# cucibala/FaceRecognizeOnnx

Hardware: AMD Instinct MI355X
Metric: faces/sec end-to-end (detect+align+embed), batch=128 640x640 (higher is better)
Workload: dtype f32; 1 GPU; C-headline: 128 frames 640x640 per GPU, SCRFD det_500m + decode + NMS, first 1 face(s)/frame aligned to 112x112, IResNet-50 (w600k_r50) embed, L2-norm; frames_per_gpu=128, faces_per_frame=1, weights=synthetic seeded (det seed 100, rec seed 200), input_residency=HBM-resident before the timed region, gallery_rows=0, topk=0, parallelism=frame-sharded x1, no data-path collective

## Files before the change

facerecognizeonnx_amd/_lib.py:

```python
from __future__ import annotations

import ctypes as C
import os
import subprocess

import numpy as np

_HERE = os.path.dirname(os.path.abspath(__file__))
LIB_PATH = os.path.join(_HERE, "libfacehip.so")
CSRC = os.path.join(_HERE, "csrc")

FACE_DTYPE = np.dtype([("x", "<i4"), ("y", "<i4"), ("w", "<i4"), ("h", "<i4"),
                       ("score", "<f4"), ("lm", "<f4", (10,))])
assert FACE_DTYPE.itemsize == 60


class FhFace(C.Structure):
    _fields_ = [("x", C.c_int32), ("y", C.c_int32), ("w", C.c_int32), ("h", C.c_int32),
                ("score", C.c_float), ("lm", C.c_float * 10)]


def build(force: bool = False) -> str:
    srcs = [os.path.join(CSRC, f) for f in os.listdir(CSRC)] + [os.path.join(_HERE, "..", "include", "facehip.h")]
    stale = (not os.path.exists(LIB_PATH)) or any(os.path.getmtime(s) > os.path.getmtime(LIB_PATH) for s in srcs)
    if force or stale:
        subprocess.check_call(["make", "-C", CSRC, "-j8", "-s"])
    return LIB_PATH


def csrc_fingerprint() -> str:
    import hashlib
    h = hashlib.sha256()
    host_only = {"image_io.cpp", "onnx_reader.cpp", "onnx_reader.h", "comm.cpp"}
    for f in sorted(os.listdir(CSRC)):
        if f.endswith((".hip", ".cpp", ".h")) and f not in host_only:
            h.update(f.encode()); h.update(open(os.path.join(CSRC, f), "rb").read())
    return h.hexdigest()[:16]


_vp, _i, _f, _ll, _d = C.c_void_p, C.c_int, C.c_float, C.c_longlong, C.c_double
_ip = C.POINTER(C.c_int)

PROTOTYPES = {
    "fh_version": (C.c_char_p, []),
    "fh_last_error": (C.c_char_p, []),
    "fh_init": (_i, [_i]),
    "fh_plan_describe": (_i, [C.c_char_p, _i, _i, C.c_char_p, _i]),
    "fh_onnx_dump": (_i, [C.c_char_p, C.c_char_p, _i]),
    "fh_det_create": (_vp, [C.c_char_p]),
    "fh_det_destroy": (None, [_vp]),
    "fh_det_input_size": (_i, [_vp, _ip, _ip]),
    "fh_det_num_anchors": (_i, [_vp]),
    "fh_det_macs_per_frame": (_d, [_vp]),
    "fh_det_act_bytes_per_frame": (_d, [_vp]),
    "fh_det_detect": (_i, [_vp, _vp, _i, _i, _i, _f, _f, _vp, _i]),
    "fh_det_detect_batch_dev": (_i, [_vp, _vp, _i, _i, _i, _i, _ll, _f, _f, _vp, _i, _vp, _vp]),
    "fh_det_run_network_dev": (_i, [_vp, _vp, _i, _i, _i, _i, _ll, _vp]),
    "fh_det_num_outputs": (_i, [_vp]),
    "fh_det_output_dev": (_vp, [_vp, _i, _ip, _ip]),
    "fh_det_input_dev": (_vp, [_vp]),
    "fh_det_postprocess_dev": (_i, [_vp, _i, _f, _f, _vp, _i, _vp, _vp]),
    "fh_postprocess_rows_dev": (_i, [_vp, _i, _i, _i, _f, _f, _f, _vp, _i, _vp, _vp]),
    "fh_rec_create": (_vp, [C.c_char_p]),
    "fh_rec_destroy": (None, [_vp]),
    "fh_rec_input_size": (_i, [_vp, _ip, _ip]),
    "fh_rec_feature_dim": (_i, [_vp]),
    "fh_rec_macs_per_face": (_d, [_vp]),
    "fh_rec_act_bytes_per_face": (_d, [_vp]),
    "fh_rec_set_chunk": (_i, [_vp, _i]),
    "fh_rec_extract": (_i, [_vp, _vp, _i, _i, _i, _vp, _vp, _i]),
    "fh_rec_extract_simple": (_i, [_vp, _vp, _i, _i, _i, _vp, _i]),
    "fh_compare": (_f, [_vp, _i, _vp, _i]),
    "fh_rec_embed_aligned_dev": (_i, [_vp, _vp, _i, _vp, _vp, _vp]),
    "fh_rec_align_dev": (_i, [_vp, _vp, _i, _i, _i, _ll, _vp, _vp, _i, _vp, _vp, _vp]),
    "fh_rec_input_dev": (_vp, [_vp]),
    "fh_rec_embed_faces_dev": (_i, [_vp, _vp, _i, _i, _i, _ll, _vp, _vp, _i, _vp, _vp, _vp]),
    "fh_pipeline_run_dev": (_i, [_vp, _vp, _vp, _i, _i, _i, _i, _ll, _f, _f, _i, _vp, _vp, _vp, _vp]),
    "fh_pipeline_submit_dev": (_i, [_vp, _vp, _vp, _i, _i, _i, _i, _ll, _f, _f, _i, _vp, _vp, _vp, _vp, _vp, _vp]),
    "fh_stream_create": (_vp, [_vp, _vp, _i, _i, _i, _i]),
    "fh_stream_destroy": (None, [_vp]),
    "fh_stream_submit": (_i, [_vp, _vp, _i, _f, _f]),
    "fh_stream_collect": (_i, [_vp, _vp, _vp, _vp, _i]),
    "fh_gallery_create": (_vp, [_i]),
    "fh_gallery_destroy": (None, [_vp]),
    "fh_gallery_upload": (_i, [_vp, _vp, _ll, _i, _ll]),
    "fh_gallery_enroll": (_ll, [_vp, _vp, _ll, _i]),
    "fh_gallery_size": (_ll, [_vp]),
    "fh_gallery_label_dev": (_i, [_vp, _vp, _i, _f, _vp, _vp, _vp]),
    "fh_gallery_topk_dev": (_i, [_vp, _vp, _i, _i, _vp, _vp, _vp]),
    "fh_gallery_set_scan": (_i, [_vp, _i]),
    "fh_gallery_get_scan": (_i, [_vp]),
    "fh_gallery_scan_stats": (_i, [_vp, C.POINTER(_ll), C.POINTER(_ll)]),
    "fh_topk_merge_dev": (_i, [_vp, _vp, _i, _i, _i, _vp, _vp, _vp]),
    "fh_comm_unique_id": (_i, [_vp]),
    "fh_comm_create": (_vp, [_i, _i, _vp, _i]),
    "fh_comm_destroy": (None, [_vp]),
    "fh_comm_rank": (_i, [_vp]),
    "fh_comm_world": (_i, [_vp]),
    "fh_comm_allgather_f32_dev": (_i, [_vp, _vp, _vp, _ll, _vp]),
    "fh_gallery_topk_sharded_dev": (_i, [_vp, _vp, _vp, _i, _i, _vp, _vp, _vp]),
    "fh_timing_enable": (_i, [_i]),
    "fh_timing_num_tags": (_i, []),
    "fh_timing_collect": (_i, [_vp, _vp, _vp, _vp, _i]),
    "fh_timing_collect_ops": (_i, [_vp, _vp, _vp, _i]),
    "fh_det_set_conv_cfg": (_i, [_vp, _i, _i]),
    "fh_rec_set_conv_cfg": (_i, [_vp, _i, _i]),
    "fh_memcpy_d2h": (_i, [_vp, _vp, C.c_size_t]),
    "fh_det_sync": (_i, [_vp, _vp]),
    "fh_rec_sync": (_i, [_vp, _vp]),
    "fh_imread": (_i, [C.c_char_p, C.POINTER(_vp), C.POINTER(_i), C.POINTER(_i)]),
    "fh_image_decode": (_i, [_vp, C.c_size_t, C.POINTER(_vp), C.POINTER(_i), C.POINTER(_i)]),
    "fh_image_free": (None, [_vp]),
    "fh_det_set_winograd": (_i, [_vp, _i]),
    "fh_rec_set_winograd": (_i, [_vp, _i]),
    "fh_rec_set_wino_fusion": (_i, [_vp, _i]),
    "fh_rec_set_shortcut_fold": (_i, [_vp, _i]),
    "fh_rec_set_precision": (_i, [_vp, _i, C.POINTER(C.c_float)]),
    "fh_rec_get_precision": (_i, [_vp]),
    "fh_det_set_cus": (_i, [_vp, _i]),
    "fh_rec_set_cus": (_i, [_vp, _i]),
    "fh_debug_streamk": (_i, [_i, _i]),
    "fh_debug_wino_slots": (_i, [_i]),
    "fh_debug_topk_merge_strided_dev": (_i, [_vp, _vp, _i, _i, _i, _ll, _vp, _vp, _vp]),
    "fh_set_graph_replay": (_i, [_i]),
    "fh_det_workspace_dev": (_vp, [_vp]),
    "fh_det_graph_stats": (_i, [_vp, _vp]),
    "fh_rec_graph_stats": (_i, [_vp, _vp]),
    "fh_det_set_fused_stem": (_i, [_vp, _i]),
    "fh_rec_set_fused_stem": (_i, [_vp, _i]),
    "fh_det_set_fused_front": (_i, [_vp, _i]),
    "fh_det_set_halo_conv": (_i, [_vp, _i]),
    "fh_resize_u8c3_dev": (_i, [_vp, _i, _i, _i, _vp, _i, _i, _i, _vp]),
    "fh_conv_forward_dev": (_i, [_vp, _vp, _vp, _vp, _i, _i, _i, _i, _i, _i, _i, _i, _i, _vp]),
    "fh_conv_winograd_dev": (_i, [_vp, _vp, _vp, _vp, _i, _i, _i, _i, _i, _vp]),
    "fh_debug_wino2_clock_mhz": (_d, []),
    "fh_conv_wino2_dev": (_i, [_vp, _vp, _vp, _vp, _vp, _vp, _i, _i, _i, _i, _i, _i, _i, _vp]),
    "fh_conv_wino2_ex_dev": (_i, [_vp, _vp, _vp, _vp, _vp, _vp, _vp, _vp, _vp, _i, _vp, _vp, _vp, _i, _i, _i, _i, _i, _i, _i, _vp]),
    "fh_conv_wt_rows": (_i, [_i]),
    "fh_conv_pack_weights": (_i, [_vp, _i, _i, _i, _vp]),
    "fh_conv_kpad": (_i, [_i]),
}

_LIB = None


def lib() -> C.CDLL:
    global _LIB
    if _LIB is None:
        path = build()
        path = os.environ.get("FACEHIP_LIB") or path
        try:
            import torch
        except ImportError:
            pass
        L = C.CDLL(path)
        for name, (res, args) in PROTOTYPES.items():
            fn = getattr(L, name)
            fn.restype = res
            fn.argtypes = args
        _LIB = L
    return _LIB


def last_error() -> str:
    return lib().fh_last_error().decode(errors="replace")


class FaceHipError(RuntimeError):
    pass


def check(rc: int, what: str) -> int:
    if rc < 0:
        raise FaceHipError(f"{what} failed ({rc}): {last_error()}")
    return rc
```

facerecognizeonnx_amd/csrc/api.cpp:

```cpp
#include <algorithm>
#include <cstdio>
#include <cstring>
#include <memory>
#include <string>
#include <vector>

#include "../../include/facehip.h"
#include "engine.h"

static_assert(sizeof(fh_face) == 60 && sizeof(fh::FaceRec) == 60, "FaceBox mirror must stay 60 bytes");

namespace {
thread_local std::string g_err;

struct CallOwners { const fh::Net* net[2] = {nullptr, nullptr}; bool shared = false; };
thread_local CallOwners t_owners;
struct Owns {
    explicit Owns(const fh::Net* a, const fh::Net* b = nullptr) { t_owners.net[0] = a; t_owners.net[1] = b; t_owners.shared = !a && !b; }
    ~Owns() { t_owners = CallOwners{}; }
    Owns(const Owns&) = delete;
    Owns& operator=(const Owns&) = delete;
};
template <class F>
int guarded(F&& f) {
    try {
        const int rc = f();
        for (const fh::Net* n : t_owners.net)
            if (n && fh::conv_take_error(g_err, n->error_record())) return FH_ERR_DEVICE;
        if (t_owners.shared && fh::conv_take_error(g_err, fh::conv_error_words())) return FH_ERR_DEVICE;
        return rc;
    } catch (const std::exception& e) {
        g_err = e.what();
        const bool dev = g_err.rfind("HIP error", 0) == 0;
        return dev ? FH_ERR_DEVICE : (g_err.rfind("onnx", 0) == 0 || g_err.rfind("plan", 0) == 0) ? FH_ERR_MODEL : FH_ERR_STATE;
    } catch (...) {
        g_err = "unknown exception";
        return FH_ERR_STATE;
    }
}
int arg_error(const char* msg) { g_err = msg; return FH_ERR_ARG; }
size_t host_image_bytes(int rows, int cols, int step) { return (size_t)(rows - 1) * step + (size_t)cols * 3; }
hipStream_t S(void* s) { return reinterpret_cast<hipStream_t>(s); }
}

namespace fh {
void set_error(const std::string& msg) { g_err = msg; }
}

struct PinnedBuf {
    void* p = nullptr; size_t bytes = 0;
    bool ensure(size_t n) {
        if (n <= bytes) return false;
        if (p) (void)hipHostFree(p);
        p = nullptr; bytes = 0;
        FH_HIP(hipHostMalloc(&p, n, hipHostMallocDefault));
        bytes = n;
        return true;
    }
    ~PinnedBuf() { if (p) (void)hipHostFree(p); }
};
bool g_graph_replay = [] { const char* e = getenv("FACEHIP_GRAPH"); return !e || atoi(e) != 0; }();
struct GraphCall {
    hipGraph_t g = nullptr; hipGraphExec_t x = nullptr;
    std::vector<long long> key;
    int seen = 0;
    size_t nodes = 0;
    long replays = 0;
    void reset() {
        if (x) (void)hipGraphExecDestroy(x);
        if (g) (void)hipGraphDestroy(g);
        x = nullptr; g = nullptr; seen = 0; nodes = 0;
    }
    ~GraphCall() { reset(); }
    template <class F>
    void run(const std::vector<long long>& k, hipStream_t s, F&& body) {
        const bool allow = g_graph_replay && !fh::KernelTimer::get().enabled && !getenv("FACEHIP_DEBUG_SYNC");
        if (!allow) { reset(); key.clear(); body(s); return; }
        if (k != key) { reset(); key = k; }
        if (x) { FH_HIP(hipGraphLaunch(x, s)); ++replays; return; }
        if (seen++ == 0) { body(s); return; }
        FH_HIP(hipStreamBeginCapture(s, hipStreamCaptureModeThreadLocal));
        try {
            body(s);
        } catch (...) {
            hipGraph_t dead = nullptr;
            (void)hipStreamEndCapture(s, &dead);
            if (dead) (void)hipGraphDestroy(dead);
            seen = 0;
            throw;
        }
        FH_HIP(hipStreamEndCapture(s, &g));
        FH_HIP(hipGraphInstantiate(&x, g, nullptr, nullptr, 0));
        (void)hipGraphGetNodes(g, nullptr, &nodes);
        FH_HIP(hipGraphLaunch(x, s));
        ++replays;
    }
};
struct CallStream {
    hipStream_t s = nullptr;
    hipStream_t get() { if (!s) FH_HIP(hipStreamCreateWithFlags(&s, hipStreamNonBlocking)); return s; }
    ~CallStream() { if (s) (void)hipStreamDestroy(s); }
};
static void graph_env_key(std::vector<long long>& key, const fh::Net& net) {
    key.push_back((long long)fh::layout_epoch());
    key.push_back(net.config_word());
    key.push_back((long long)fh::conv_error_generation() << 32 | fh::conv_debug_generation());
}
constexpr int kGraphFaces = 256;

struct fh_det {
    explicit fh_det(const char* p) : det(p) {}
    fh::Detector det;
    fh::DevBuf img, out, cnt;
    PinnedBuf h_img, h_res;
    GraphCall gcall;
    CallStream cs;
    fh::DevBuf p_det, p_cnt, p_total;
    hipEvent_t ev_sel = nullptr;
    int* h_total = nullptr;
    ~fh_det() { if (ev_sel) (void)hipEventDestroy(ev_sel); if (h_total) (void)hipHostFree(h_total); }
};
struct fh_rec {
    explicit fh_rec(const char* p) : rec(p) {}
    fh::Recognizer rec;
    fh::DevBuf img, face, emb;
    PinnedBuf h_img, h_io;
    GraphCall gcall, gcall_simple;
    CallStream cs;
};
struct fh_gallery {
    explicit fh_gallery(int dim) : g(dim) {}
    fh::Gallery g;
};

extern "C" {

const char* fh_version(void) { return "facehip 0.1 (gfx950)"; }
const char* fh_last_error(void) { return g_err.c_str(); }

int fh_init(int device) {
    return guarded([&] {
        int n = 0;
        FH_HIP(hipGetDeviceCount(&n));
        if (device < 0 || device >= n) throw std::runtime_error("HIP error: no such device");
        FH_HIP(hipSetDevice(device));
        return n;
    });
}

int fh_plan_describe(const char* onnx_path, int default_h, int default_w, char* buf, int cap) {
    if (!onnx_path || !buf || cap <= 0) return arg_error("fh_plan_describe: null argument");
    return guarded([&] {
        fh::OnnxModel m = fh::load_onnx(onnx_path);
        int H = default_h, W = default_w;
        const auto& shp = m.inputs[0].shape;
        if (shp.size() == 4) { if (shp[2] > 0) H = (int)shp[2]; if (shp[3] > 0) W = (int)shp[3]; }
        fh::Plan p = fh::build_plan(m, H, W);
        std::string s = p.describe();
        snprintf(buf, (size_t)cap, "%s", s.c_str());
        return (int)s.size();
    });
}

int fh_onnx_dump(const char* onnx_path, char* buf, int cap) {
    if (!onnx_path || !buf || cap <= 0) return arg_error("fh_onnx_dump: null argument");
    return guarded([&] {
        const fh::OnnxModel m = fh::load_onnx(onnx_path);
        std::string s;
        char tmp[256];
        auto dims = [&](const std::vector<int64_t>& d) { std::string o; for (size_t i = 0; i < d.size(); ++i) { o += (i ? "," : ""); o += std::to_string(d[i]); } return o; };
        for (const auto& v : m.inputs) s += "input " + v.name + " [" + dims(v.shape) + "]\n";
        for (const auto& v : m.outputs) s += "output " + v.name + " [" + dims(v.shape) + "]\n";
        for (const auto& kv : m.inits) {
            const fh::OnnxTensor& t = kv.second;
            double sum = 0, first = 0, last = 0;
            size_t n = 0;
            if (!t.f.empty()) { n = t.f.size(); for (float x : t.f) sum += x; first = t.f.front(); last = t.f.back(); }
            else if (!t.i.empty()) { n = t.i.size(); for (int64_t x : t.i) sum += (double)x; first = (double)t.i.front(); last = (double)t.i.back(); }
            snprintf(tmp, sizeof tmp, " n=%zu sum=%.9g first=%.9g last=%.9g\n", n, sum, first, last);
            s += "init " + kv.first + " dtype=" + std::to_string(t.dtype) + " [" + dims(t.dims) + "]" + tmp;
        }
        for (const auto& nd : m.nodes) {
            s += "node " + nd.op + " in=";
            for (size_t i = 0; i < nd.inputs.size(); ++i) s += (i ? "," : "") + nd.inputs[i];
            s += " out=";
            for (size_t i = 0; i < nd.outputs.size(); ++i) s += (i ? "," : "") + nd.outputs[i];
            for (const auto& av : nd.attrs) {
                const fh::OnnxAttr& a = av.second;
                s += " " + av.first + "=";
                if (!a.ints.empty()) s += "ints:" + dims(a.ints);
                else if (!a.floats.empty()) { s += "floats:"; for (size_t i = 0; i < a.floats.size(); ++i) { snprintf(tmp, sizeof tmp, "%s%.9g", i ? "," : "", a.floats[i]); s += tmp; } }
                else if (!a.s.empty()) s += "s:" + a.s;
                else if (!a.t.dims.empty() || !a.t.f.empty() || !a.t.i.empty()) s += "t:[" + dims(a.t.dims) + "]";
                else if (a.f != 0.f) { snprintf(tmp, sizeof tmp, "f:%.9g", a.f); s += tmp; }
                else s += "i:" + std::to_string(a.i);
            }
            s += "\n";
        }
        snprintf(buf, (size_t)cap, "%s", s.c_str());
        return (int)std::min<size_t>(s.size(), (size_t)cap - 1);
    });
}

fh_det* fh_det_create(const char* onnx_path) {
    if (!onnx_path) { g_err = "fh_det_create: null path"; return nullptr; }
    fh_det* h = nullptr;
    int rc = guarded([&] { h = new fh_det(onnx_path); return 0; });
    return rc == 0 ? h : nullptr;
}
void fh_det_destroy(fh_det* d) { delete d; }
int fh_det_input_size(const fh_det* d, int* w, int* h) {
    if (!d) return arg_error("null handle");
    if (w) *w = const_cast<fh_det*>(d)->det.net().in_w();
    if (h) *h = const_cast<fh_det*>(d)->det.net().in_h();
    return FH_OK;
}
int fh_det_num_anchors(const fh_det* d) { return d ? d->det.num_anchors() : arg_error("null handle"); }
double fh_det_macs_per_frame(const fh_det* d) { return d ? const_cast<fh_det*>(d)->det.net().plan().macs : 0.0; }
double fh_det_act_bytes_per_frame(const fh_det* d) { return d ? const_cast<fh_det*>(d)->det.net().plan().act_bytes : 0.0; }

int fh_det_detect_batch_dev(fh_det* d, const uint8_t* frames, int n, int rows, int cols, int step, long long stride,
                            float score_thr, float nms_thr, fh_face* out, int max_pf, int* counts, void* stream) {
    if (!d || !frames || !out || !counts) return arg_error("fh_det_detect_batch_dev: null argument");
    if (n <= 0 || rows <= 0 || cols <= 0 || step < cols * 3 || max_pf <= 0) return arg_error("fh_det_detect_batch_dev: bad size");
    Owns owns(&d->det.net());
    return guarded([&] {
        d->det.detect_dev(frames, n, rows, cols, step, (long)stride, score_thr, nms_thr, reinterpret_cast<fh::FaceRec*>(out), max_pf,
                          counts, S(stream));
        return n;
    });
}

int fh_det_detect(fh_det* d, const uint8_t* bgr, int rows, int cols, int step, float score_thr, float nms_thr, fh_face* out,
                  int max_out) {
    if (!d) return arg_error("Model not loaded!");
    if (!bgr || rows <= 0 || cols <= 0) return 0;
    if (!out || max_out <= 0 || step < cols * 3) return arg_error("fh_det_detect: bad output buffer / step");
    Owns owns(&d->det.net());
    return guarded([&] {
        const size_t bytes = (size_t)rows * step, used = host_image_bytes(rows, cols, step);
        const int in_graph = max_out < kGraphFaces ? max_out : kGraphFaces;
        d->img.ensure(bytes);
        d->out.ensure((size_t)max_out * sizeof(fh_face));
        d->cnt.ensure(sizeof(int));
        const bool m1 = d->h_img.ensure(bytes), m2 = d->h_res.ensure(64 + (size_t)kGraphFaces * sizeof(fh_face));
        const bool moved = m1 || m2;
        if (moved) d->gcall.reset();
        memcpy(d->h_img.p, bgr, used);
        hipStream_t s = d->cs.get();
        int* const h_cnt = static_cast<int*>(d->h_res.p);
        fh_face* const h_faces = reinterpret_cast<fh_face*>(static_cast<char*>(d->h_res.p) + 64);
        long long kthr, knms;
        { float f = score_thr; int v; memcpy(&v, &f, 4); kthr = v; f = nms_thr; memcpy(&v, &f, 4); knms = v; }
        std::vector<long long> key{rows, cols, step, kthr, knms, max_out, (long long)(size_t)d->img.p, (long long)(size_t)d->out.p};
        graph_env_key(key, d->det.net());
        try {
            d->gcall.run(key, s, [&](hipStream_t st) {
                FH_HIP(hipMemcpyAsync(d->img.p, d->h_img.p, used, hipMemcpyHostToDevice, st));
                d->det.detect_dev(d->img.as<uint8_t>(), 1, rows, cols, step, (long)bytes, score_thr, nms_thr, d->out.as<fh::FaceRec>(),
                                  max_out, d->cnt.as<int>(), st);
                FH_HIP(hipMemcpyAsync(h_cnt, d->cnt.p, sizeof(int), hipMemcpyDeviceToHost, st));
                FH_HIP(hipMemcpyAsync(h_faces, d->out.p, (size_t)in_graph * sizeof(fh_face), hipMemcpyDeviceToHost, st));
            });
        } catch (const std::runtime_error& e) {
            if (std::string(e.what()) == "Invalid resize dimensions") return 0;
            throw;
        }
        FH_HIP(hipStreamSynchronize(s));
        int c = *h_cnt;
        c = c < max_out ? c : max_out;
        const int first = c < in_graph ? c : in_graph;
        if (first > 0) memcpy(out, h_faces, (size_t)first * sizeof(fh_face));
        if (c > first)
            FH_HIP(hipMemcpy(out + first, d->out.as<fh_face>() + first, (size_t)(c - first) * sizeof(fh_face), hipMemcpyDeviceToHost));
        return c;
    });
}

int fh_det_sync(fh_det* d, void* stream) {
    if (!d) return arg_error("fh_det_sync: null handle");
    Owns owns(&d->det.net());
    return guarded([&] { FH_HIP(hipStreamSynchronize(S(stream))); return (int)FH_OK; });
}
int fh_det_run_network_dev(fh_det* d, const uint8_t* frames, int n, int rows, int cols, int step, long long stride, void* stream) {
    if (!d || !frames || n <= 0) return arg_error("fh_det_run_network_dev: bad argument");
    Owns owns(&d->det.net());
    return guarded([&] { d->det.run_network_dev(frames, n, rows, cols, step, (long)stride, S(stream)); return n; });
}
int fh_det_num_outputs(const fh_det* d) { return d ? (int)const_cast<fh_det*>(d)->det.net().plan().outputs.size() : arg_error("null handle"); }
const float* fh_det_output_dev(fh_det* d, int index, int* rows, int* cols) {
    if (!d || index < 0 || index >= (int)d->det.net().plan().outputs.size()) { g_err = "bad output index"; return nullptr; }
    const auto& o = d->det.net().plan().outputs[index];
    if (rows) *rows = o.rows;
    if (cols) *cols = o.cols;
    return d->det.net().capacity() > 0 ? d->det.net().output(index) : nullptr;
}
const float* fh_det_input_dev(fh_det* d) { return d && d->det.net().capacity() > 0 ? d->det.net().input() : nullptr; }
int fh_det_postprocess_dev(fh_det* d, int n, float score_thr, float nms_thr, fh_face* out, int max_pf, int* counts, void* stream) {
    if (!d || !out || !counts || n <= 0) return arg_error("fh_det_postprocess_dev: bad argument");
    Owns owns(&d->det.net());
    return guarded([&] { d->det.postprocess_dev(n, score_thr, nms_thr, reinterpret_cast<fh::FaceRec*>(out), max_pf, counts, S(stream)); return n; });
}

int fh_postprocess_rows_dev(const float* rows, int n, int rows_per_frame, int feat, float scale, float score_thr, float nms_thr,
                            fh_face* out, int max_pf, int* counts, void* stream) {
    if (!rows || !out || !counts) return arg_error("fh_postprocess_rows_dev: null argument");
    if (n <= 0 || rows_per_frame <= 0 || max_pf <= 0 || !(scale > 0.f)) return arg_error("fh_postprocess_rows_dev: bad size");
    if ((long)n * rows_per_frame >= (1L << 31) / 16) return arg_error("fh_postprocess_rows_dev: too many rows");
    return guarded([&] {
        hipStream_t s = S(stream);
        if (feat < 15) {
            FH_HIP(hipMemsetAsync(counts, 0, (size_t)n * sizeof(int), s));
            return n;
        }
        struct Scratch { fh::DevBuf cand, keys, ws, count; hipEvent_t done = nullptr; hipStream_t last = nullptr; bool used = false; };
        thread_local Scratch* scp = new Scratch();
        Scratch& sc = *scp;
        if (!sc.done) FH_HIP(hipEventCreateWithFlags(&sc.done, hipEventDisableTiming));
        if (sc.used && sc.last != s) FH_HIP(hipStreamWaitEvent(s, sc.done, 0));
        fh::DevBuf &cand = sc.cand, &keys = sc.keys, &ws = sc.ws, &count = sc.count;
        int cap = 1;
        while (cap < rows_per_frame) cap <<= 1;
        cand.ensure((size_t)n * cap * sizeof(fh::FaceRec));
        keys.ensure((size_t)n * cap * sizeof(unsigned long long));
        ws.ensure((size_t)n * cap * sizeof(int));
        count.ensure((size_t)n * sizeof(int));
        FH_HIP(hipMemsetAsync(count.p, 0, (size_t)n * sizeof(int), s));
        fh::launch_rows_threshold(rows, n, rows_per_frame, feat, scale, score_thr, cand.as<fh::FaceRec>(), keys.as<unsigned long long>(),
                                  count.as<int>(), cap, s);
        fh::launch_sort_nms(cand.as<fh::FaceRec>(), keys.as<unsigned long long>(), count.as<int>(), cap, n, nms_thr,
                            reinterpret_cast<fh::FaceRec*>(out), counts, max_pf, ws.as<int>(), s);
        FH_HIP(hipGetLastError());
        FH_HIP(hipEventRecord(sc.done, s));
        sc.last = s; sc.used = true;
        return n;
    });
}

fh_rec* fh_rec_create(const char* onnx_path) {
    if (!onnx_path) { g_err = "fh_rec_create: null path"; return nullptr; }
    fh_rec* h = nullptr;
    int rc = guarded([&] { h = new fh_rec(onnx_path); return 0; });
    return rc == 0 ? h : nullptr;
}
void fh_rec_destroy(fh_rec* r) { delete r; }
int fh_rec_input_size(const fh_rec* r, int* w, int* h) {
    if (!r) return arg_error("null handle");
    if (w) *w = const_cast<fh_rec*>(r)->rec.net().in_w();
    if (h) *h = const_cast<fh_rec*>(r)->rec.net().in_h();
    return FH_OK;
}
int fh_rec_feature_dim(const fh_rec* r) { return r ? r->rec.dim() : arg_error("null handle"); }
double fh_rec_macs_per_face(const fh_rec* r) { return r ? const_cast<fh_rec*>(r)->rec.net().plan().macs : 0.0; }
double fh_rec_act_bytes_per_face(const fh_rec* r) { return r ? const_cast<fh_rec*>(r)->rec.net().plan().act_bytes : 0.0; }
int fh_rec_set_chunk(fh_rec* r, int n) {
    if (!r || n <= 0) return arg_error("fh_rec_set_chunk: bad argument");
    size_t biggest = 1;
    for (const auto& t : r->rec.net().plan().tensors) biggest = std::max(biggest, t.elems());
    const long limit = (long)(((1UL << 31) - 1) / biggest);
    if (n > limit) return arg_error("fh_rec_set_chunk: chunk too large for the 32-bit tensor offsets of one pass");
    r->rec.max_chunk = n;
    return FH_OK;
}
const float* fh_rec_input_dev(fh_rec* r) { return r && r->rec.net().capacity() > 0 ? r->rec.net().input() : nullptr; }

int fh_rec_embed_aligned_dev(fh_rec* r, const uint8_t* crops, int n, float* out, float* raw, void* stream) {
    if (!r || !crops || !out || n <= 0) return arg_error("fh_rec_embed_aligned_dev: bad argument");
    Owns owns(&r->rec.net());
    return guarded([&] { r->rec.embed_aligned_dev(crops, n, out, S(stream), raw); return n; });
}
int fh_rec_sync(fh_rec* r, void* stream) {
    if (!r) return arg_error("fh_rec_sync: null handle");
    Owns owns(&r->rec.net());
    return guarded([&] { FH_HIP(hipStreamSynchronize(S(stream))); return (int)FH_OK; });
}
int fh_rec_align_dev(fh_rec* r, const uint8_t* frames, int rows, int cols, int step, long long stride, const fh_face* faces,
                     const int* frame_of, int n, uint8_t* crops, int* ok, void* stream) {
    if (!r || !frames || !faces || !crops || !ok || n <= 0 || rows <= 0 || cols <= 0) return arg_error("fh_rec_align_dev: bad argument");
    Owns owns(&r->rec.net());
    return guarded([&] {
        r->rec.align_dev(frames, rows, cols, step, (long)stride, reinterpret_cast<const fh::FaceRec*>(faces), frame_of, n, crops, ok, S(stream));
        return n;
    });
}
int fh_rec_embed_faces_dev(fh_rec* r, const uint8_t* frames, int rows, int cols, int step, long long stride, const fh_face* faces,
                           const int* frame_of, int n, float* out, int* ok, void* stream) {
    if (!r || !frames || !faces || !out || n <= 0 || rows <= 0 || cols <= 0) return arg_error("fh_rec_embed_faces_dev: bad argument");
    Owns owns(&r->rec.net());
    return guarded([&] {
        r->rec.embed_faces_dev(frames, rows, cols, step, (long)stride, reinterpret_cast<const fh::FaceRec*>(faces), frame_of, n, out, ok, S(stream));
        return n;
    });
}

int fh_rec_extract(fh_rec* r, const uint8_t* bgr, int rows, int cols, int step, const fh_face* face, float* out, int out_cap) {
    if (!r) return arg_error("Model not loaded!");
    if (!bgr || rows <= 0 || cols <= 0) return 0;
    if (!face || !out || step < cols * 3) return arg_error("fh_rec_extract: bad argument");
    if (out_cap < r->rec.dim()) return arg_error("fh_rec_extract: output buffer too small");
    Owns owns(&r->rec.net());
    return guarded([&] {
        const size_t bytes = (size_t)rows * step, used = host_image_bytes(rows, cols, step);
        const size_t dimb = (size_t)r->rec.dim() * sizeof(float);
        r->img.ensure(bytes);
        r->face.ensure(sizeof(fh_face) + sizeof(int));
        r->emb.ensure(dimb);
        const bool m1 = r->h_img.ensure(bytes), m2 = r->h_io.ensure(128 + dimb);
        const bool moved = m1 || m2;
        if (moved) { r->gcall.reset(); r->gcall_simple.reset(); }
// ... 44 lines not shown
        });
        FH_HIP(hipStreamSynchronize(s));
        memcpy(out, io + 128, dimb);
        return r->rec.dim();
    });
}

float fh_compare(const float* f1, int n1, const float* f2, int n2) {
    if (n1 != n2 || n1 <= 0 || !f1 || !f2) return 0.0f;
    float dot = 0.0f;
    for (int i = 0; i < n1; ++i) dot += f1[i] * f2[i];
    return (dot + 1.0f) / 2.0f;
}

namespace {
int detect_select_count(fh_det* d, const uint8_t* frames, int n, int rows, int cols, int step, long stride, float score_thr, float nms_thr,
                        int F, fh_face* faces, int* frame_of, int* d_total, hipStream_t sd) {
    d->p_det.ensure((size_t)n * F * sizeof(fh_face));
    d->p_cnt.ensure((size_t)n * sizeof(int));
    d->p_total.ensure(sizeof(int));
    if (!d->ev_sel) FH_HIP(hipEventCreateWithFlags(&d->ev_sel, hipEventDisableTiming));
    if (!d->h_total) FH_HIP(hipHostMalloc(reinterpret_cast<void**>(&d->h_total), sizeof(int), hipHostMallocDefault));
    int* dt = d_total ? d_total : d->p_total.as<int>();
    d->det.detect_dev(frames, n, rows, cols, step, stride, score_thr, nms_thr, d->p_det.as<fh::FaceRec>(), F, d->p_cnt.as<int>(), sd);
    fh::launch_select_faces(d->p_det.as<fh::FaceRec>(), d->p_cnt.as<int>(), n, F, F, reinterpret_cast<fh::FaceRec*>(faces), frame_of, dt, sd);
    FH_HIP(hipMemcpyAsync(d->h_total, dt, sizeof(int), hipMemcpyDeviceToHost, sd));
    FH_HIP(hipEventRecord(d->ev_sel, sd));
    FH_HIP(hipEventSynchronize(d->ev_sel));
    return *d->h_total;
}
}

int fh_pipeline_run_dev(fh_det* d, fh_rec* r, const uint8_t* frames, int n, int rows, int cols, int step, long long stride,
                        float score_thr, float nms_thr, int F, fh_face* faces, int* frame_of, float* emb, void* stream) {
    if (!d || !r || !frames || !faces || !frame_of || !emb) return arg_error("fh_pipeline_run_dev: null argument");
    if (n <= 0 || n > 4096 || rows <= 0 || cols <= 0 || F <= 0) return arg_error("fh_pipeline_run_dev: bad size");
    Owns owns(&d->det.net(), &r->rec.net());
    return guarded([&] {
        hipStream_t s = S(stream);
        const int total = detect_select_count(d, frames, n, rows, cols, step, (long)stride, score_thr, nms_thr, F, faces, frame_of, nullptr, s);
        r->rec.embed_faces_dev(frames, rows, cols, step, (long)stride, reinterpret_cast<const fh::FaceRec*>(faces), frame_of, total, emb, nullptr, s);
        return total;
    });
}

int fh_pipeline_submit_dev(fh_det* d, fh_rec* r, const uint8_t* frames, int n, int rows, int cols, int step, long long stride,
                           float score_thr, float nms_thr, int F, fh_face* faces, int* frame_of, float* emb, int* d_total,
                           void* stream_det, void* stream_rec) {
    if (!d || !r || !frames || !faces || !frame_of || !emb || !d_total) return arg_error("fh_pipeline_submit_dev: null argument");
    if (n <= 0 || n > 4096 || rows <= 0 || cols <= 0 || F <= 0) return arg_error("fh_pipeline_submit_dev: bad size");
    Owns owns(&d->det.net(), &r->rec.net());
    return guarded([&] {
        hipStream_t sd = S(stream_det), sr = S(stream_rec);
        const int total = detect_select_count(d, frames, n, rows, cols, step, (long)stride, score_thr, nms_thr, F, faces, frame_of, d_total, sd);
        if (sd != sr) FH_HIP(hipStreamWaitEvent(sr, d->ev_sel, 0));
        r->rec.embed_faces_dev(frames, rows, cols, step, (long)stride, reinterpret_cast<const fh::FaceRec*>(faces), frame_of, total, emb, nullptr, sr);
        return total;
    });
}

struct fh_stream {
    static constexpr int kSlots = 2;
    fh_det* det; fh_rec* rec;
    int n, rows, cols, F, dim;
    size_t frame_bytes;
    hipStream_t copy_s = nullptr, comp_s = nullptr;
    struct Slot {
        fh::DevBuf frames, faces, frame_of, emb;
        hipEvent_t uploaded = nullptr, done = nullptr;
        int total = -1;
        int frames_in = 0;
    } slot[kSlots];
    long submitted = 0, collected = 0;
    fh_stream(fh_det* d, fh_rec* r, int n_, int rows_, int cols_, int F_) : det(d), rec(r), n(n_), rows(rows_), cols(cols_), F(F_) {
        dim = r->rec.dim();
        frame_bytes = (size_t)rows * cols * 3;
        FH_HIP(hipStreamCreateWithFlags(&copy_s, hipStreamNonBlocking));
        FH_HIP(hipStreamCreateWithFlags(&comp_s, hipStreamNonBlocking));
        for (auto& sl : slot) {
            sl.frames.ensure((size_t)n * frame_bytes);
            sl.faces.ensure((size_t)n * F * sizeof(fh_face));
            sl.frame_of.ensure((size_t)n * F * sizeof(int));
            sl.emb.ensure((size_t)n * F * dim * sizeof(float));
            FH_HIP(hipEventCreateWithFlags(&sl.uploaded, hipEventDisableTiming));
            FH_HIP(hipEventCreateWithFlags(&sl.done, hipEventDisableTiming));
        }
    }
    ~fh_stream() {
        (void)hipDeviceSynchronize();
        for (auto& sl : slot) { if (sl.uploaded) (void)hipEventDestroy(sl.uploaded); if (sl.done) (void)hipEventDestroy(sl.done); }
        if (copy_s) (void)hipStreamDestroy(copy_s);
        if (comp_s) (void)hipStreamDestroy(comp_s);
    }
};

fh_stream* fh_stream_create(fh_det* d, fh_rec* r, int frames_per_batch, int rows, int cols, int faces_per_frame) {
    if (!d || !r || frames_per_batch <= 0 || frames_per_batch > 4096 || rows <= 0 || cols <= 0 || faces_per_frame <= 0) {
        g_err = "fh_stream_create: bad argument";
        return nullptr;
    }
    fh_stream* h = nullptr;
    const int rc = guarded([&] { h = new fh_stream(d, r, frames_per_batch, rows, cols, faces_per_frame); return 0; });
    return rc == 0 ? h : nullptr;
}
void fh_stream_destroy(fh_stream* s) { delete s; }

int fh_stream_submit(fh_stream* st, const uint8_t* host_frames, int n_frames, float score_thr, float nms_thr) {
    if (!st || !host_frames) return arg_error("fh_stream_submit: null argument");
    if (n_frames <= 0 || n_frames > st->n) return arg_error("fh_stream_submit: batch larger than the stream was created for");
    if (st->submitted - st->collected >= fh_stream::kSlots) { g_err = "fh_stream_submit: ring full, collect a batch first"; return FH_ERR_STATE; }
    Owns owns(&st->det->det.net(), &st->rec->rec.net());
    return guarded([&] {
        fh_stream::Slot& sl = st->slot[st->submitted % fh_stream::kSlots];
        FH_HIP(hipMemcpyAsync(sl.frames.p, host_frames, (size_t)n_frames * st->frame_bytes, hipMemcpyHostToDevice, st->copy_s));
        FH_HIP(hipEventRecord(sl.uploaded, st->copy_s));
        FH_HIP(hipStreamWaitEvent(st->comp_s, sl.uploaded, 0));
        const int step = st->cols * 3;
        const int total = detect_select_count(st->det, sl.frames.as<uint8_t>(), n_frames, st->rows, st->cols, step, (long)st->frame_bytes, score_thr, nms_thr,
                                              st->F, sl.faces.as<fh_face>(), sl.frame_of.as<int>(), nullptr, st->comp_s);
        st->rec->rec.embed_faces_dev(sl.frames.as<uint8_t>(), st->rows, st->cols, step, (long)st->frame_bytes, sl.faces.as<fh::FaceRec>(),
                                     sl.frame_of.as<int>(), total, sl.emb.as<float>(), nullptr, st->comp_s);
        FH_HIP(hipEventRecord(sl.done, st->comp_s));
        sl.total = total; sl.frames_in = n_frames;
        ++st->submitted;
        return total;
    });
}

int fh_stream_collect(fh_stream* st, fh_face* faces, int* frame_of, float* emb, int cap) {
    if (!st) return arg_error("fh_stream_collect: null handle");
    if (st->collected >= st->submitted) { g_err = "fh_stream_collect: nothing in flight"; return FH_ERR_STATE; }
    Owns owns(&st->det->det.net(), &st->rec->rec.net());
    return guarded([&] {
        fh_stream::Slot& sl = st->slot[st->collected % fh_stream::kSlots];
        FH_HIP(hipEventSynchronize(sl.done));
        const int m = sl.total < cap ? sl.total : cap;
        if (m > 0) {
            if (faces) FH_HIP(hipMemcpy(faces, sl.faces.p, (size_t)m * sizeof(fh_face), hipMemcpyDeviceToHost));
            if (frame_of) FH_HIP(hipMemcpy(frame_of, sl.frame_of.p, (size_t)m * sizeof(int), hipMemcpyDeviceToHost));
            if (emb) FH_HIP(hipMemcpy(emb, sl.emb.p, (size_t)m * st->dim * sizeof(float), hipMemcpyDeviceToHost));
        }
        const int total = sl.total;
        sl.total = -1;
        ++st->collected;
        return total;
    });
}

fh_gallery* fh_gallery_create(int dim) {
    if (dim <= 0) { g_err = "fh_gallery_create: bad dim"; return nullptr; }
    return new fh_gallery(dim);
}
void fh_gallery_destroy(fh_gallery* g) { delete g; }
int fh_gallery_upload(fh_gallery* g, const float* rows, long long n, int on_device, long long index_base) {
    if (!g || !rows || n <= 0) return arg_error("fh_gallery_upload: bad argument");
    return guarded([&] { g->g.upload(rows, (long)n, on_device != 0, (long)index_base); return 0; });
}
long long fh_gallery_enroll(fh_gallery* g, const float* rows, long long n, int on_device) {
    if (!g || !rows || n <= 0) return arg_error("fh_gallery_enroll: bad argument");
    long long first = -1;
    const int rc = guarded([&] { first = g->g.enroll(rows, (long)n, on_device != 0); return 0; });
    return rc < 0 ? rc : first;
}
long long fh_gallery_size(fh_gallery* g) { return g ? (long long)g->g.size() : (long long)arg_error("fh_gallery_size: null handle"); }
int fh_gallery_label_dev(fh_gallery* g, const float* q, int nq, float threshold, int* labels, float* scores, void* stream) {
    if (!g || !q || !labels || !scores) return arg_error("fh_gallery_label_dev: null argument");
    return guarded([&] { g->g.label_dev(q, nq, threshold, labels, scores, S(stream)); return nq; });
}
int fh_gallery_topk_dev(fh_gallery* g, const float* q, int nq, int k, float* scores, int* indices, void* stream) {
    if (!g || !q || !scores || !indices) return arg_error("fh_gallery_topk_dev: null argument");
    return guarded([&] { g->g.topk_dev(q, nq, k, scores, indices, S(stream)); return nq; });
}

int fh_gallery_set_scan(fh_gallery* g, int mode) {
    if (!g) return arg_error("fh_gallery_set_scan: null handle");
    if (mode != FH_GAL_SCAN_FP32 && mode != FH_GAL_SCAN_F16_RERANK) return arg_error("fh_gallery_set_scan: unknown mode");
    return guarded([&] { g->g.set_scan(mode); return 0; });
}
int fh_gallery_get_scan(const fh_gallery* g) { return g ? g->g.scan() : arg_error("fh_gallery_get_scan: null handle"); }
int fh_gallery_scan_stats(fh_gallery* g, long long* certified, long long* fallback) {
    if (!g) return arg_error("fh_gallery_scan_stats: null handle");
    return guarded([&] { g->g.scan_stats(certified, fallback); return 0; });
}

int fh_topk_merge_dev(const float* ps, const int* pi, int nparts, int nq, int k, float* scores, int* indices, void* stream) {
    if (!ps || !pi || !scores || !indices) return arg_error("fh_topk_merge_dev: null argument");
    if (nparts <= 0 || nq <= 0 || k <= 0 || k > 16 || (long)nparts * k > 65536) return arg_error("fh_topk_merge_dev: bad size");
    return guarded([&] {
        fh::launch_topk_merge(ps, pi, nparts, nq, k, scores, indices, S(stream));
        FH_HIP(hipGetLastError());
        return nq;
    });
}

int fh_debug_topk_merge_strided_dev(const float* ps, const int* pi, int nparts, int nq, int k, long long part_stride, float* scores, int* indices,
                                    void* stream) {
    if (!ps || !pi || !scores || !indices) return arg_error("fh_debug_topk_merge_strided_dev: null argument");
    if (nparts <= 0 || nq <= 0 || k <= 0 || k > 16 || (long)nparts * k > 65536 || part_stride < (long long)nq * k)
        return arg_error("fh_debug_topk_merge_strided_dev: bad size");
    return guarded([&] {
        fh::launch_topk_merge_strided(ps, pi, nparts, nq, k, (long)part_stride, scores, indices, S(stream));
        FH_HIP(hipGetLastError());
        return nq;
    });
}

int fh_timing_enable(int on) { fh::KernelTimer::get().enabled = on != 0; return FH_OK; }
int fh_timing_num_tags(void) { return fh::KernelTimer::kTags; }
int fh_timing_collect(double* ms, double* flops, double* bytes, long long* launches, int n) {
    if (!ms || !flops || !bytes || !launches || n < fh::KernelTimer::kTags) return arg_error("fh_timing_collect: need fh_timing_num_tags()-entry arrays");
    return guarded([&] { fh::KernelTimer::get().collect(ms, flops, bytes, launches); return fh::KernelTimer::kTags; });
}
int fh_timing_collect_ops(double* ms, double* flops, int* tag, int cap) {
    if (!ms || !flops || !tag || cap <= 0) return arg_error("fh_timing_collect_ops: bad argument");
    return guarded([&] { return fh::KernelTimer::get().collect_ops(ms, flops, tag, cap); });
}
int fh_det_set_conv_cfg(fh_det* d, int cfg, int stream_k) {
    if (!d) return arg_error("null handle");
    d->det.net().force_cfg = cfg; d->det.net().sk_enable = stream_k != 0;
    return FH_OK;
}
int fh_det_set_winograd(fh_det* d, int on) { if (!d) return arg_error("null handle"); d->det.net().winograd = on != 0; return FH_OK; }
int fh_rec_set_winograd(fh_rec* r, int on) { if (!r) return arg_error("null handle"); r->rec.net().winograd = on != 0; return FH_OK; }
int fh_rec_set_wino_fusion(fh_rec* r, int on) { if (!r) return arg_error("null handle"); r->rec.net().fuse_wino = on != 0; return FH_OK; }
int fh_rec_set_precision(fh_rec* r, int mode, float* worst_out) {
    if (!r || (mode != FH_PREC_FP32 && mode != FH_PREC_BF16X2)) return arg_error("fh_rec_set_precision: bad argument");
    if (worst_out) *worst_out = 0.f;
    Owns owns(&r->rec.net());
    if (mode == FH_PREC_FP32) return guarded([&] { r->rec.net().set_bf16x2(false, nullptr); return (int)FH_OK; });
    return guarded([&] {
        fh::Net& net = r->rec.net();
        const int n = 64, dim = r->rec.dim();
        const size_t crop = (size_t)net.in_h() * net.in_w() * 3;
        std::vector<uint8_t> h((size_t)n * crop);
        uint32_t st = 0x9E3779B9u;
        for (int i = 0; i < n; ++i) {
            const int amp = 16 + 3 * i;
            for (size_t e = 0; e < crop; ++e) {
                st = st * 1664525u + 1013904223u;
                const int px = (int)(e / 3) % net.in_w(), py = (int)(e / 3) / net.in_w();
                const int v = 128 + ((px * (i + 1) + py * (n - i)) % 97 - 48) + (int)((st >> 24) % (2 * amp + 1)) - amp;
                h[(size_t)i * crop + e] = (uint8_t)std::min(255, std::max(0, v));
            }
        }
        fh::DevBuf dc, de;
        dc.ensure(h.size()); de.ensure((size_t)2 * n * dim * sizeof(float));
        FH_HIP(hipMemcpy(dc.p, h.data(), h.size(), hipMemcpyHostToDevice));
        const bool was = net.bf16x2();
        net.set_bf16x2(false, nullptr);
        r->rec.embed_aligned_dev(dc.as<uint8_t>(), n, de.as<float>(), nullptr);
        const int layers = net.set_bf16x2(true, nullptr);
        if (layers == 0) { net.set_bf16x2(was, nullptr); throw std::runtime_error("fh_rec_set_precision: this model has no layer with a split-bf16 form"); }
        struct Rollback { fh::Net& n; bool armed = true; ~Rollback() { if (armed) { try { n.set_bf16x2(false, nullptr); } catch (...) {} } } } rollback{net};
        r->rec.embed_aligned_dev(dc.as<uint8_t>(), n, de.as<float>() + (size_t)n * dim, nullptr);
        std::vector<float> e((size_t)2 * n * dim);
        FH_HIP(hipDeviceSynchronize());
        FH_HIP(hipMemcpy(e.data(), de.p, e.size() * sizeof(float), hipMemcpyDeviceToHost));
        double worst = 0;
        for (int i = 0; i < n; ++i) {
            double dot = 0, na = 0, nb = 0;
            for (int c = 0; c < dim; ++c) {
                const double a = e[(size_t)i * dim + c], b = e[(size_t)(n + i) * dim + c];
                dot += a * b; na += a * a; nb += b * b;
            }
            const double err = (na > 0 && nb > 0) ? 1.0 - dot / std::sqrt(na * nb) : 1.0;
            worst = std::max(worst, std::isfinite(err) ? err : 1.0);
        }
        if (worst_out) *worst_out = (float)worst;
        double gate = 1e-3;
        if (const char* g = getenv("FACEHIP_PRECISION_GATE")) gate = std::min(gate, atof(g));
        if (!(worst < gate))
            throw std::runtime_error("fh_rec_set_precision: split-bf16 embeddings differ from fp32 by 1 - cos = " + std::to_string(worst) +
                                 " (gate " + std::to_string(gate) + "): staying fp32");
        rollback.armed = false;
        return layers;
    });
}
int fh_rec_get_precision(fh_rec* r) { return r && r->rec.net().bf16x2() ? FH_PREC_BF16X2 : FH_PREC_FP32; }
int fh_rec_set_shortcut_fold(fh_rec* r, int on) { if (!r) return arg_error("null handle"); r->rec.net().fold_shortcut = on != 0; return FH_OK; }
int fh_det_set_halo_conv(fh_det* d, int on) { if (!d) return arg_error("null handle"); d->det.net().halo_conv = on != 0; return FH_OK; }
int fh_det_set_cus(fh_det* d, int cus) { if (!d || cus < 0) return arg_error("bad argument"); d->det.net().cus = cus; return FH_OK; }
int fh_rec_set_cus(fh_rec* r, int cus) { if (!r || cus < 0) return arg_error("bad argument"); r->rec.net().cus = cus; return FH_OK; }
int fh_det_set_fused_stem(fh_det* d, int on) { if (!d) return arg_error("null handle"); d->det.net().fuse_stem = on != 0; return FH_OK; }
int fh_det_set_fused_front(fh_det* d, int on) { if (!d) return arg_error("null handle"); d->det.net().fuse_front = on != 0; return FH_OK; }
int fh_rec_set_fused_stem(fh_rec* r, int on) { if (!r) return arg_error("null handle"); r->rec.net().fuse_stem = on != 0; return FH_OK; }
int fh_rec_set_conv_cfg(fh_rec* r, int cfg, int stream_k) {
    if (!r) return arg_error("null handle");
    r->rec.net().force_cfg = cfg; r->rec.net().sk_enable = stream_k != 0;
    return FH_OK;
}

int fh_memcpy_d2h(void* dst, const void* src, size_t bytes) {
    if (!dst || !src) return arg_error("fh_memcpy_d2h: null argument");
    return guarded([&] { FH_HIP(hipDeviceSynchronize()); FH_HIP(hipMemcpy(dst, src, bytes, hipMemcpyDeviceToHost)); return 0; });
}
int fh_resize_u8c3_dev(const uint8_t* src, int sh, int sw, int sstep, uint8_t* dst, int dh, int dw, int dstep, void* stream) {
    if (!src || !dst || sh <= 0 || sw <= 0 || dh <= 0 || dw <= 0) return arg_error("fh_resize_u8c3_dev: bad argument");
    return guarded([&] {
        fh::launch_resize_u8c3(src, (long)sh * sstep, sh, sw, sstep, dst, (long)dh * dstep, dh, dw, dstep, 1, S(stream));
        FH_HIP(hipGetLastError());
        return 0;
    });
}
int fh_conv_winograd_dev(const float* d_in, const float* w_ohwi, const float* d_bias, float* d_out, int batch, int h, int w, int cin,
                         int cout, void* stream) {
    if (!d_in || !w_ohwi || !d_out || cin % 32 || cout % 4) return arg_error("fh_conv_winograd_dev: bad argument");
    Owns owns(nullptr);
    return guarded([&] {
        const int rows = fh::conv_wt_rows(cout);
        std::vector<float> u36((size_t)36 * rows * cin, 0.f), uf((size_t)cout * cin);
        std::vector<double> uall((size_t)cout * cin * 36);
        for (int co = 0; co < cout; ++co)
            for (int ci = 0; ci < cin; ++ci) {
                double g[9];
                for (int t = 0; t < 9; ++t) g[t] = w_ohwi[((size_t)co * 9 + t) * cin + ci];
                fh::wino_filter_transform(g, &uall[((size_t)co * cin + ci) * 36]);
            }
        for (int f = 0; f < 36; ++f) {
            for (size_t e = 0; e < uf.size(); ++e) uf[e] = (float)uall[e * 36 + f];
            fh::conv_pack_weights(uf.data(), cout, cin, 1, u36.data() + (size_t)f * rows * cin);
        }
        const size_t tiles = (size_t)batch * ((h + 3) / 4) * ((w + 3) / 4);
        fh::DevBuf dU, dV, dM;
        dU.ensure(u36.size() * sizeof(float));
        dV.ensure((36 * (size_t)fh::wino_rows((long)tiles) + 100 * 128) * cin * sizeof(float));
        dM.ensure((36 * (size_t)fh::wino_rows((long)tiles) + 100 * 128) * cout * sizeof(float));
        FH_HIP(hipMemcpy(dU.p, u36.data(), u36.size() * sizeof(float), hipMemcpyHostToDevice));
        static fh::DevBuf slabs;
        static unsigned slabs_gen = 0;
        if (!slabs.p) { slabs.ensure(fh::conv_slab_floats() * sizeof(float)); fh::conv_workspace_init(slabs.as<float>()); slabs_gen = fh::conv_error_generation(); }
        if (slabs_gen != fh::conv_error_generation()) { fh::conv_workspace_reset_async(slabs.as<float>(), S(stream)); slabs_gen = fh::conv_error_generation(); }
        fh::ConvArgs a{};
        a.in = d_in; a.bias = d_bias; a.out1 = d_out; a.slabs = slabs.as<float>(); a.sk_enable = 1;
        a.B = batch; a.H = h; a.W = w; a.Ho = h; a.Wo = w; a.Cin = cin; a.Cout = cout; a.ks = 3; a.stride = 1; a.pad = 1;
        a.act = (int)fh::Act::NONE; a.res_mode = (int)fh::ResMode::NONE;
        fh::launch_conv_winograd(a, dU.as<float>(), dV.as<float>(), dM.as<float>(), 2, nullptr, nullptr, S(stream));
        FH_HIP(hipStreamSynchronize(S(stream)));
        return 0;
    });
}
int fh_conv_wino2_ex_dev(const float* d_in, const float* w_ohwi, const float* d_bias, const float* d_slope, const float* d_res, float* d_out,
                         float* d_out2, const float* d_s2, const float* d_t2, int n_outs, float* const* d_outs, const int* oc0, const int* oact,
                         int batch, int h, int w, int cin, int cout, int act, int bias_cls, void* stream) {
    if (!d_in || !w_ohwi || batch <= 0 || h <= 0 || w <= 0 || cin != 64 || cout <= 0) return arg_error("fh_conv_wino2_dev: bad argument (cin = 64, positive sizes)");
    if (n_outs < 0 || n_outs > 3 || (n_outs > 0 && (!d_outs || !oc0 || !oact))) return arg_error("fh_conv_wino2_dev: bad merged-output description");
    if (n_outs == 0 && ((!d_out && !d_out2) || cout % 64)) return arg_error("fh_conv_wino2_dev: plain layers need an output and cout % 64 == 0");
    if (d_out2 && (!d_s2 || !d_t2)) return arg_error("fh_conv_wino2_dev: a second output needs its scale and shift");
    Owns owns(nullptr);
    return guarded([&] {
        fh::ConvArgs a{};
        a.in = d_in; a.bias = d_bias; a.slope = d_slope; a.res = d_res; a.out1 = d_out; a.out2 = d_out2; a.s2 = d_s2; a.t2 = d_t2;
        a.B = batch; a.H = h; a.W = w; a.Ho = h; a.Wo = w; a.Cin = cin; a.Cout = cout; a.ks = 3; a.stride = 1; a.pad = 1;
        a.act = act; a.bias_cls = bias_cls; a.res_mode = d_res ? (int)fh::ResMode::SAME : (int)fh::ResMode::NONE;
        a.n_outs = n_outs;
        for (int g = 0; g < n_outs; ++g) { a.outs[g] = d_outs[g]; a.oact[g] = oact[g]; a.oc0[g] = oc0[g]; }
        if (n_outs > 0) a.oc0[n_outs] = oc0[n_outs];
        if (!fh::wino2_ok(a)) throw std::runtime_error("fh_conv_wino2_dev: layer shape not supported by the fused F(2x2) kernel");
        std::vector<float> u(fh::wino2_weight_floats(cin, cout));
        fh::wino2_pack_weights(w_ohwi, cout, cin, u.data());
        fh::DevBuf dU;
        dU.ensure(u.size() * sizeof(float));
        FH_HIP(hipMemcpy(dU.p, u.data(), u.size() * sizeof(float), hipMemcpyHostToDevice));
        a.wt = dU.as<float>();
        fh::launch_wino2(a, S(stream));
        FH_HIP(hipGetLastError());
        FH_HIP(hipStreamSynchronize(S(stream)));
        return 0;
    });
}
int fh_conv_wino2_dev(const float* d_in, const float* w_ohwi, const float* d_bias, const float* d_slope, const float* d_res, float* d_out,
                      int batch, int h, int w, int cin, int cout, int act, int bias_cls, void* stream) {
    return fh_conv_wino2_ex_dev(d_in, w_ohwi, d_bias, d_slope, d_res, d_out, nullptr, nullptr, nullptr, 0, nullptr, nullptr, nullptr, batch, h, w,
                                cin, cout, act, bias_cls, stream);
}
double fh_debug_wino2_clock_mhz(void) { return fh::wino2_debug_clock_mhz(); }
int fh_conv_wt_rows(int cout) { return fh::conv_wt_rows(cout); }
int fh_conv_pack_weights(const float* w_ohwi, int cout, int cin, int ksize, float* dst_packed) {
    if (!w_ohwi || !dst_packed || cout <= 0 || cin <= 0) return arg_error("fh_conv_pack_weights: bad argument");
    memset(dst_packed, 0, (size_t)fh::conv_wt_rows(cout) * fh::conv_kpad(ksize * ksize * cin) * sizeof(float));
    fh::conv_pack_weights(w_ohwi, cout, cin, ksize, dst_packed);
    return 0;
}
int fh_conv_kpad(int ktot) { return fh::conv_kpad(ktot); }
const float* fh_det_workspace_dev(fh_det* d) { return d ? d->det.net().workspace() : nullptr; }
int fh_set_graph_replay(int on) { g_graph_replay = on != 0; return FH_OK; }
int fh_det_graph_stats(fh_det* d, long long* replays) {
    if (!d) return arg_error("null handle");
    if (replays) *replays = d->gcall.replays;
    return (int)d->gcall.nodes;
}
int fh_rec_graph_stats(fh_rec* r, long long* replays) {
    if (!r) return arg_error("null handle");
    if (replays) *replays = r->gcall.replays + r->gcall_simple.replays;
    return (int)(r->gcall.nodes ? r->gcall.nodes : r->gcall_simple.nodes);
}
int fh_debug_wino_slots(int slots) { fh::wino_debug_slots(slots); return 0; }
int fh_debug_streamk(int drop_publish, int timeout_ms) { fh::conv_debug_streamk(drop_publish, timeout_ms); return 0; }
int fh_conv_forward_dev(const float* in, const float* wt, const float* bias, float* out, int batch, int h, int w, int cin, int cout,
                        int ks, int stride, int kpad, int cfg, void* stream) {
    if (!in || !wt || !out || batch <= 0 || (ks != 1 && ks != 3) || cin % 4) return arg_error("fh_conv_forward_dev: bad argument");
    Owns owns(nullptr);
    return guarded([&] {
        fh::ConvArgs a{};
        const int pad = ks / 2;
        a.in = in; a.wt = wt; a.bias = bias; a.out1 = out;
        a.B = batch; a.H = h; a.W = w; a.Cin = cin; a.Cout = cout; a.ks = ks; a.stride = stride; a.pad = pad;
        a.Ho = (h + 2 * pad - ks) / stride + 1; a.Wo = (w + 2 * pad - ks) / stride + 1;
        a.Kpad = kpad;
        static fh::DevBuf slabs;
        static unsigned slabs_gen = 0;
        if (!slabs.p) { slabs.ensure(fh::conv_slab_floats() * sizeof(float)); fh::conv_workspace_init(slabs.as<float>()); slabs_gen = fh::conv_error_generation(); }
        if (slabs_gen != fh::conv_error_generation()) { fh::conv_workspace_reset_async(slabs.as<float>(), S(stream)); slabs_gen = fh::conv_error_generation(); }
        a.slabs = slabs.as<float>(); a.sk_enable = 1;
        fh::launch_conv(a, cfg, S(stream));
        FH_HIP(hipGetLastError());
        return 0;
    });
}

}

namespace fh {
Gallery& gallery_of(fh_gallery* g) { return g->g; }
}
```

facerecognizeonnx_amd/csrc/engine.cpp:

```cpp
#include "engine.h"

#include <atomic>
#include <cstdio>
#include <cstdlib>
#include <algorithm>
#include <cmath>
#include <cstring>

namespace fh {

void hip_check(hipError_t e, const char* what) {
    if (e != hipSuccess) throw std::runtime_error(std::string("HIP error: ") + hipGetErrorString(e) + " in " + what);
}

static std::atomic<unsigned long long> g_layout_epoch{1};
unsigned long long layout_epoch() { return g_layout_epoch.load(std::memory_order_relaxed); }

DevBuf::~DevBuf() {
    if (p) { (void)hipFree(p); g_layout_epoch.fetch_add(1, std::memory_order_relaxed); }
}
void DevBuf::ensure(size_t n) {
    if (n <= bytes) return;
    g_layout_epoch.fetch_add(1, std::memory_order_relaxed);
    if (p) { FH_HIP(hipDeviceSynchronize()); FH_HIP(hipFree(p)); p = nullptr; bytes = 0; }
    FH_HIP(hipMalloc(&p, n));
    bytes = n;
}

KernelTimer& KernelTimer::get() { static KernelTimer t; return t; }
hipEvent_t KernelTimer::take() {
    if (!pool_.empty()) { hipEvent_t e = pool_.back(); pool_.pop_back(); return e; }
    hipEvent_t e; FH_HIP(hipEventCreate(&e)); return e;
}
void KernelTimer::begin(hipStream_t s) {
    if (!enabled) return;
    cur_ = take();
    FH_HIP(hipEventRecord(cur_, s));
}
void KernelTimer::end(hipStream_t s, int tag, double flops, double bytes) {
    if (!enabled || !cur_) return;
    hipEvent_t b = take();
    FH_HIP(hipEventRecord(b, s));
    recs_.push_back(Rec{cur_, b, tag, flops, bytes});
    cur_ = nullptr;
}
void KernelTimer::collect(double* ms, double* flops, double* bytes, long long* launches) {
    for (int i = 0; i < kTags; ++i) { ms[i] = 0; flops[i] = 0; bytes[i] = 0; launches[i] = 0; }
    for (auto& r : recs_) {
        FH_HIP(hipEventSynchronize(r.b));
        float t = 0.f;
        FH_HIP(hipEventElapsedTime(&t, r.a, r.b));
        ms[r.tag] += t; flops[r.tag] += r.flops; bytes[r.tag] += r.bytes; launches[r.tag] += 1;
        pool_.push_back(r.a); pool_.push_back(r.b);
    }
    recs_.clear();
}

int KernelTimer::collect_ops(double* ms, double* flops, int* tag, int cap) {
    int n = 0;
    for (auto& r : recs_) {
        FH_HIP(hipEventSynchronize(r.b));
        float t = 0.f;
        FH_HIP(hipEventElapsedTime(&t, r.a, r.b));
        if (n < cap) { ms[n] = t; flops[n] = r.flops; tag[n] = r.tag; ++n; }
        pool_.push_back(r.a); pool_.push_back(r.b);
    }
    recs_.clear();
    return n;
}

static bool debug_sync() {
    static int v = -1;
    if (v < 0) { const char* e = getenv("FACEHIP_DEBUG_SYNC"); v = e ? atoi(e) : 0; }
    return v != 0;
}


static constexpr int kWinoMinCin = 128;
static constexpr long kWinoMinTiles = 256;
static long wino2_min_blocks() {
    static long v = -1;
    if (v < 0) {
        const char* e = getenv("FACEHIP_WINO2");
        const char* m = getenv("FACEHIP_WINO2_MIN");
        v = e && atoi(e) == 0 ? (1L << 60) : m ? atol(m) : 64;
    }
    return v;
}

Net::Net(const std::string& onnx_path, int default_h, int default_w) {
    OnnxModel m = load_onnx(onnx_path);
    int H = default_h, W = default_w;
    const auto& shp = m.inputs[0].shape;
    if (shp.size() == 4) {
        if (shp[2] > 0) H = (int)shp[2];
        if (shp[3] > 0) W = (int)shp[3];
    }
    plan_ = build_plan(m, H, W);

    std::vector<float> host;
    auto push = [&](const float* src, size_t n) {
        size_t off = (host.size() + 63) / 64 * 64;
        host.resize(off + n, 0.f);
        if (n) memcpy(host.data() + off, src, n * sizeof(float));
        return off;
    };
    dev_.resize(plan_.ops.size());
    for (size_t i = 0; i < plan_.ops.size(); ++i) {
        POp& c = plan_.ops[i];
        if (c.bn_src < 0 || c.kind != OpKind::CONV || c.ks != 3 || c.stride != 1 || c.pad != 1 || c.H < 2 || c.W < 2) continue;
        const bool wino_ok = c.Cin >= kWinoMinCin && c.Cin % 32 == 0 && c.Cout % 4 == 0 && c.outs.empty() && c.res_mode != ResMode::UP2X;
        const POp& pr = plan_.ops[c.bn_src];
        if (wino_ok || !c.outs.empty() || (int)pr.s2.size() < c.Cin || pr.out < 0) continue;
        std::vector<float> b9((size_t)9 * c.Cout);
        for (int co = 0; co < c.Cout; ++co) {
            double tap_shift[9];
            for (int t = 0; t < 9; ++t) {
                double acc = 0;
                for (int ci = 0; ci < c.Cin; ++ci) acc += (double)c.weight[((size_t)co * 9 + t) * c.Cin + ci] * pr.t2[ci];
                tap_shift[t] = acc;
            }
            for (int ry = 0; ry < 3; ++ry)
                for (int rx = 0; rx < 3; ++rx) {
                    double b = c.bias[co];
                    for (int ky = 0; ky < 3; ++ky)
                        for (int kx = 0; kx < 3; ++kx) {
                            const bool in_y = !(ry == 0 && ky == 0) && !(ry == 2 && ky == 2);
                            const bool in_x = !(rx == 0 && kx == 0) && !(rx == 2 && kx == 2);
                            if (in_y && in_x) b += tap_shift[ky * 3 + kx];
                        }
                    b9[(size_t)(ry * 3 + rx) * c.Cout + co] = (float)b;
                }
            for (int t = 0; t < 9; ++t)
                for (int ci = 0; ci < c.Cin; ++ci) c.weight[((size_t)co * 9 + t) * c.Cin + ci] *= pr.s2[ci];
        }
        c.bias = b9;
        dev_[i].bn_fold_src = c.bn_src;
        dev_[c.bn_src].bn_fold_dst = true;
    }
    for (size_t i = 0; i < plan_.ops.size(); ++i) {
        const POp& op = plan_.ops[i];
        DevOp& d = dev_[i];
        if (op.kind == OpKind::DWPW) {
            d.dww = push(op.dw_weight.data(), op.dw_weight.size());
            d.dwb = push(op.dw_bias.data(), op.dw_bias.size());
        }
        if (op.kind == OpKind::CONV || op.kind == OpKind::GEMM || op.kind == OpKind::DWPW) {
            const int Ktot = op.ks * op.ks * op.Cin;
            d.Kpad = conv_kpad(Ktot);
            const int rows = conv_wt_rows(op.Cout);
            std::vector<float> packed((size_t)rows * d.Kpad, 0.f);
            conv_pack_weights(op.weight.data(), op.Cout, op.Cin, op.ks, packed.data());
            d.wt = push(packed.data(), packed.size());
            if (op.kind == OpKind::CONV) {
                ConvArgs probe{};
                probe.ks = op.ks; probe.stride = op.stride; probe.pad = op.pad; probe.Cin = op.Cin; probe.Cout = op.Cout; probe.act = (int)op.act;
                probe.res_mode = (int)op.res_mode; probe.H = op.H; probe.W = op.W;
                float dummy = 0.f;
                probe.out2 = op.out2 >= 0 ? &dummy : nullptr;
                probe.bias_cls = dev_[i].bn_fold_src >= 0 ? 1 : 0;
                if (conv_halo_ok(probe) && op.Ho * op.Wo >= 400) {
                    std::vector<float> wf(conv_halo_wfrag_floats(op.Cin, op.Cout));
                    conv_halo_pack_weights(op.weight.data(), op.Cout, op.Cin, wf.data());
                    d.wfrag = push(wf.data(), wf.size());
                    d.halo = true;
                }
            }
            if (op.kind == OpKind::CONV && op.Cin < kWinoMinCin) {
                ConvArgs probe{};
                probe.ks = op.ks; probe.stride = op.stride; probe.pad = op.pad; probe.Cin = op.Cin; probe.Cout = op.Cout; probe.act = (int)op.act;
                probe.res_mode = (int)op.res_mode; probe.H = op.H; probe.W = op.W; probe.Ho = op.Ho; probe.Wo = op.Wo;
                probe.n_outs = (int)op.outs.size(); probe.bias_cls = dev_[i].bn_fold_src >= 0 ? 1 : 0;
                float dummy2 = 0.f;
                probe.out2 = op.out2 >= 0 ? &dummy2 : nullptr;
                if (wino2_ok(probe)) {
                    std::vector<float> u(wino2_weight_floats(op.Cin, op.Cout));
                    wino2_pack_weights(op.weight.data(), op.Cout, op.Cin, u.data());
                    d.w2 = push(u.data(), u.size());
                    d.w2ok = true;
                }
            }
            if (op.kind == OpKind::CONV && op.ks == 3 && op.stride == 1 && op.pad == 1 && op.Cin >= kWinoMinCin && op.Cin % 32 == 0 &&
                op.Cout % 4 == 0 && op.outs.empty() && op.res_mode != ResMode::UP2X) {
                std::vector<float> u36((size_t)36 * rows * op.Cin, 0.f), uf((size_t)op.Cout * op.Cin);
                std::vector<double> uall((size_t)op.Cout * op.Cin * 36);
                for (int co = 0; co < op.Cout; ++co)
                    for (int ci = 0; ci < op.Cin; ++ci) {
                        double g[9];
                        for (int t = 0; t < 9; ++t) g[t] = op.weight[((size_t)co * 9 + t) * op.Cin + ci];
                        wino_filter_transform(g, &uall[((size_t)co * op.Cin + ci) * 36]);
                    }
                for (int f = 0; f < 36; ++f) {
                    for (size_t e = 0; e < uf.size(); ++e) uf[e] = (float)uall[e * 36 + f];
                    conv_pack_weights(uf.data(), op.Cout, op.Cin, 1, u36.data() + (size_t)f * rows * op.Cin);
                }
                d.w36 = push(u36.data(), u36.size());
                d.w36n = u36.size();
                d.wino = true;
                d.bf2 = wino_gemm_ok_bf16x2(op.Cin, op.Cout);
                const size_t tiles = (size_t)((op.H + 3) / 4) * ((op.W + 3) / 4);
                wino_elems_ = std::max(wino_elems_, 36 * tiles * (size_t)std::max(op.Cin, op.Cout));
                wino_maxc_ = std::max(wino_maxc_, (size_t)std::max(op.Cin, op.Cout));
            }
        } else if (op.kind == OpKind::DWCONV || op.kind == OpKind::DWGLOBAL || op.kind == OpKind::GCONV) {
            d.wt = push(op.weight.data(), op.weight.size());
        }
        if (!op.bias.empty()) d.bias = push(op.bias.data(), op.bias.size());
        if (!op.slope.empty()) { d.slope = push(op.slope.data(), op.slope.size()); d.has_slope = true; }
        if (!op.s2.empty()) { d.s2 = push(op.s2.data(), op.s2.size()); d.t2 = push(op.t2.data(), op.t2.size()); d.has_aff = true; }
    }
    for (size_t i = 0; i < plan_.ops.size(); ++i) {
        const POp& c = plan_.ops[i];
        if (c.sc_src < 0 || dev_[i].bn_fold_src >= 0 || c.bias.size() != (size_t)c.Cout) continue;
        if (dev_[i].wino || dev_[i].halo) continue;
        const POp& x = plan_.ops[c.sc_src];
        const int K9 = 9 * c.Cin, K = K9 + x.Cin, rows = conv_wt_rows(c.Cout);
        std::vector<float> w((size_t)rows * K, 0.f), b((size_t)c.Cout);
        for (int co = 0; co < c.Cout; ++co) {
            std::copy_n(&c.weight[(size_t)co * K9], K9, &w[(size_t)co * K]);
            std::copy_n(&x.weight[(size_t)co * x.Cin], x.Cin, &w[(size_t)co * K + K9]);
            b[co] = c.bias[co] + (x.bias.empty() ? 0.f : x.bias[co]);
        }
        dev_[i].wt_sc = push(w.data(), w.size());
        dev_[i].bias_sc = push(b.data(), b.size());
        dev_[i].Kpad_sc = K;
        dev_[i].sc_src = c.sc_src;
        dev_[c.sc_src].sc_dst = true;
    }
    for (size_t i = 0; i < plan_.ops.size(); ++i) {
        const int prod = plan_.ops[i].bn_src;
        if (!dev_[i].wino || prod <= 0 || !dev_[prod].has_aff) continue;
        dev_[i].aff_src = prod; dev_[prod].aff_dst = (int)i;
    }
    for (size_t i = 0; i + 1 < plan_.ops.size(); ++i) {
        const POp& a = plan_.ops[i];
        const POp& b = plan_.ops[i + 1];
        if (!dev_[i].wino || !dev_[i + 1].wino || a.H != b.H || a.W != b.W || a.Cout != b.Cin || !wino_can_fuse(a.H, a.W, a.Cout, false)) continue;
        int feed = -1;
        if (dev_[i + 1].aff_src == (int)i) feed = 1;
        else if (a.out >= 0 && b.in == a.out) feed = 0;
        else if (a.out2 >= 0 && b.in == a.out2) feed = 1;
        if (feed < 0) continue;
        int other_uses = 0;
        if (a.out >= 0) {
            for (const POp& o : plan_.ops)
                for (int x : {o.in, o.in2, o.res}) if (x == a.out) ++other_uses;
            for (const auto& o : plan_.outputs) if (o.tensor == a.out) ++other_uses;
            if (b.in == a.out) --other_uses;
        }
        const bool writes_out2 = a.out2 >= 0 && dev_[i + 1].aff_src != (int)i;
        if (!wino_can_fuse(a.H, a.W, a.Cout, other_uses > 0 || a.res >= 0 || writes_out2)) continue;
        dev_[i].fuse_next = true; dev_[i].fuse_feed_aff = feed == 1; dev_[i].fuse_keep_out1 = other_uses > 0;
    }
    {
        const POp& op = plan_.ops[0];
        stem_ok_ = op.kind == OpKind::CONV && op.in == plan_.input && op.ks == 3 && op.Cin == 4 && op.res < 0 && op.outs.empty() &&
                   op.Cout % 4 == 0 && op.Cout <= 64 && (op.stride == 1 || op.stride == 2);
        if (stem_ok_) {
            std::vector<float> w27((size_t)27 * op.Cout);
            for (int co = 0; co < op.Cout; ++co)
                for (int t = 0; t < 9; ++t)
                    for (int ci = 0; ci < 3; ++ci) w27[(size_t)(t * 3 + ci) * op.Cout + co] = op.weight[((size_t)co * 9 + t) * 4 + ci];
            dev_[0].w27 = push(w27.data(), w27.size());
            std::vector<float> wf((size_t)27 * op.Cout), bf((size_t)op.Cout);
            for (int co = 0; co < op.Cout; ++co) {
                double sum = 0;
                for (int t = 0; t < 9; ++t)
                    for (int j = 0; j < 3; ++j) {
                        const float w = op.weight[((size_t)co * 9 + t) * 4 + (2 - j)];
                        wf[(size_t)(t * 3 + j) * op.Cout + co] = w / 128.0f;
                        sum += w;
                    }
                bf[co] = (float)((double)op.bias[co] - 127.5 / 128.0 * sum);
            }
            dev_[0].wf = push(wf.data(), wf.size());
            dev_[0].bf = push(bf.data(), bf.size());
            if (op.Cout % 16 == 0) {
                std::vector<unsigned> fr((size_t)(op.Cout / 16) * 3 * 64 * 4, 0u);
                stem_pack_wfrag(wf.data(), op.Cout, fr.data());
                std::vector<float> asf(fr.size());
                memcpy(asf.data(), fr.data(), fr.size() * 4);
                dev_[0].wfr = push(asf.data(), asf.size());
            }
        }
    }
    if (stem_ok_ && plan_.ops.size() > 1) {
        const POp& st = plan_.ops[0];
        const POp& nx = plan_.ops[1];
        int uses = 0;
        for (const auto& o : plan_.ops) for (int x : {o.in, o.in2, o.res}) if (x == st.out) ++uses;
        for (const auto& o : plan_.outputs) if (o.tensor == st.out) ++uses;
        front_ok_ = st.Cout == 16 && st.out >= 0 && st.out2 < 0 && (st.act == Act::NONE || st.act == Act::RELU) && nx.kind == OpKind::DWPW &&
                    nx.in == st.out && uses == 1 && front_fused_ok(nx.Cin, nx.Cout, nx.dw_stride);
    }
    params_.ensure(std::max<size_t>(host.size(), 64) * sizeof(float));
    FH_HIP(hipMemcpy(params_.p, host.data(), host.size() * sizeof(float), hipMemcpyHostToDevice));
    for (auto& op : plan_.ops) { std::vector<float>().swap(op.weight); }
}

Net::SkRecord::~SkRecord() {
    if (!p) return;
    int cur = -1;
    (void)hipGetDevice(&cur);
    if (device >= 0 && device != cur) (void)hipSetDevice(device);
    (void)hipDeviceSynchronize();
    if (device >= 0 && device != cur && cur >= 0) (void)hipSetDevice(cur);
    conv_error_record_release(p);
}

void Net::reserve(int max_batch) {
    if (max_batch <= cap_) return;
    cap_ = max_batch;
    arena_.ensure(plan_.arena_elems * (size_t)cap_ * sizeof(float));
    if (partial_.bytes < conv_slab_floats() * sizeof(float)) {
        partial_.ensure(conv_slab_floats() * sizeof(float));
        conv_workspace_init(partial_.as<float>());
        if (!sk_rec_.p) { sk_rec_.p = conv_error_record_new(); (void)hipGetDevice(&sk_rec_.device); }
        if (!sk_rec_.p) throw std::runtime_error("HIP error: cannot allocate the stream-K watchdog record");
        sk_gen_ = conv_error_generation();
    }
    if (wino_elems_) {
        const size_t pad = 36 * 256 * wino_maxc_;
        wino_v_.ensure((wino_elems_ * (size_t)cap_ + pad) * sizeof(float));
        wino_m_.ensure((wino_elems_ * (size_t)cap_ + pad) * sizeof(float));
    }
    FH_HIP(hipMemset(arena_.p, 0, arena_.bytes));
}

void Net::run_u8(const uint8_t* src, long img_stride, int srcH, int srcW, int step, int batch, hipStream_t s) {
    if (batch <= 0) return;
    if (batch > cap_) throw std::runtime_error("Net::run_u8: batch exceeds reserved capacity");
    if (stem_ok_ && fuse_stem && front_ok_ && fuse_front && srcW >= 2) {
        const POp& st = plan_.ops[0];
        const POp& op = plan_.ops[1];
        const DevOp& d0 = dev_[0];
        const DevOp& d = dev_[1];
        const float* P = params_.as<float>();
        ConvArgs a{};
        a.wt = P + d.wt; a.bias = P + d.bias;
        a.out1 = tensor_ptr(op.out);
        a.dw_w = P + d.dww; a.dw_b = P + d.dwb; a.dw_act = (int)op.dw_act; a.dw_stride = op.dw_stride;
        a.B = batch; a.H = op.H; a.W = op.W; a.Cin = op.Cin; a.Ho = op.Ho; a.Wo = op.Wo; a.Cout = op.Cout;
        a.ks = 1; a.stride = 1; a.pad = 0; a.Kpad = d.Kpad; a.act = (int)op.act;
        a.u8_src = src; a.u8_img_stride = img_stride; a.u8_step = step; a.u8_srcH = srcH; a.u8_srcW = srcW; a.u8_inH = plan_.inH; a.u8_inW = plan_.inW;
        a.slabs = partial_.as<float>();
        a.u8_stride = st.stride; a.stem_act = (int)st.act; a.stem_wf = P + d0.wf; a.stem_bf = P + d0.bf;
        a.stem_wfrag = reinterpret_cast<const unsigned*>(P + d0.wfr);
        a.cus = cus;
        a.t_flops = 2.0 * (st.macs + op.macs) * batch;
        a.t_bytes = ((double)srcH * srcW * 3 + (double)op.Ho * op.Wo * op.Cout * 4) * batch;
        launch_dwpw(a, s);
        run(batch, s, 2);
        return;
    }
    if (stem_ok_ && fuse_stem) {
        const POp& op = plan_.ops[0];
        const DevOp& d = dev_[0];
        const float* P = params_.as<float>();
        KernelTimer& timer = KernelTimer::get();
        timer.begin(s);
        launch_stem_conv_u8(src, img_stride, srcH, srcW, step, batch, plan_.inH, plan_.inW, op.stride, op.Cout, P + d.w27, P + d.bias, P + d.wf,
                            P + d.bf, d.has_slope ? P + d.slope : nullptr, (int)op.act, op.out >= 0 ? tensor_ptr(op.out) : nullptr,
                            op.out2 >= 0 && !d.bn_fold_dst ? tensor_ptr(op.out2) : nullptr, d.has_aff ? P + d.s2 : nullptr,
                            d.has_aff ? P + d.t2 : nullptr, s, d.wfr ? reinterpret_cast<const unsigned*>(P + d.wfr) : nullptr);
        timer.end(s, 5, 2.0 * op.macs * batch, op.bytes * batch);
        run(batch, s, 1);
        return;
    }
    launch_det_preprocess(src, img_stride, srcH, srcW, step, batch, plan_.inH, plan_.inW, srcH, srcW, input(), s);
    run(batch, s, 0);
}

int Net::set_bf16x2(bool on, hipStream_t s) {
    int layers = 0;
    size_t total = 0;
    for (auto& d : dev_) if (d.wino && d.bf2) { d.w36p = total; total += d.w36n; ++layers; }
    if (on && layers > 0 && w36_bf_.bytes < total * sizeof(float)) {
        w36_bf_.ensure(total * sizeof(float));
        for (const auto& d : dev_)
            if (d.wino && d.bf2) launch_pack_bf16x2(params_.as<float>() + d.w36, w36_bf_.as<float>() + d.w36p, (long)d.w36n, s);
        FH_HIP(hipStreamSynchronize(s));
    }
    bf16x2_ = on && layers > 0;
    return on ? layers : 0;
}

void Net::run(int batch, hipStream_t s, int first_op) {
    if (batch <= 0) return;
    if ((sk_gen_ != conv_error_generation() || conv_error_pending(sk_rec_.p)) && partial_.p) {
        conv_workspace_reset_async(partial_.as<float>(), s);
        sk_gen_ = conv_error_generation();
    }
    if (batch > cap_) throw std::runtime_error("Net::run: batch exceeds reserved capacity");
    const float* P = params_.as<float>();
    KernelTimer& timer = KernelTimer::get();
    bool v_ready = false;
    for (size_t i = (size_t)first_op; i < plan_.ops.size(); ++i) {
        const POp& op = plan_.ops[i];
        const DevOp& d = dev_[i];
        int tag = 5;
        const bool dense = op.kind == OpKind::CONV || op.kind == OpKind::GEMM || op.kind == OpKind::DWPW;
        if (!dense) timer.begin(s);
        switch (op.kind) {
            case OpKind::CONV:
            case OpKind::GEMM: {
                if (d.sc_dst && fold_shortcut && force_cfg < 0) break;
                ConvArgs a{};
                a.in = tensor_ptr(op.in);
                a.wt = P + d.wt;
                a.bias = P + d.bias;
                a.slope = d.has_slope ? P + d.slope : nullptr;
                a.res = op.res >= 0 ? tensor_ptr(op.res) : nullptr;
                a.out1 = op.out >= 0 ? tensor_ptr(op.out) : nullptr;
                a.out2 = op.out2 >= 0 ? tensor_ptr(op.out2) : nullptr;
                if (d.bn_fold_dst) a.out2 = nullptr;
                if (d.bn_fold_src >= 0) { a.in = tensor_ptr(plan_.ops[d.bn_fold_src].out); a.bias_cls = 1; }
                if (d.aff_dst >= 0 && winograd) {
                    const POp& c = plan_.ops[d.aff_dst];
                    if ((long)batch * ((c.H + 3) / 4) * ((c.W + 3) / 4) >= kWinoMinTiles) a.out2 = nullptr;
                }
                a.s2 = d.has_aff ? P + d.s2 : nullptr;
                a.t2 = d.has_aff ? P + d.t2 : nullptr;
                a.slabs = partial_.as<float>();
                a.sk_err = sk_rec_.p;
                a.sk_enable = sk_enable ? 1 : 0;
                a.cus = cus;
                a.no_pw = force_cfg >= 0 ? 1 : 0;
                a.B = batch; a.H = op.H; a.W = op.W; a.Cin = op.Cin; a.Ho = op.Ho; a.Wo = op.Wo; a.Cout = op.Cout;
                a.ks = op.ks; a.stride = op.stride; a.pad = op.pad; a.Kpad = d.Kpad;
                a.act = (int)op.act; a.res_mode = (int)op.res_mode;
                a.n_outs = (int)op.outs.size();
                for (int g = 0; g < a.n_outs && g < 3; ++g) { a.outs[g] = tensor_ptr(op.outs[g]); a.oact[g] = op.out_act[g]; a.oc0[g] = op.out_c0[g]; }
                if (a.n_outs > 0) a.oc0[a.n_outs] = op.out_c0[a.n_outs];
                const long M = (long)batch * op.Ho * op.Wo;
                int cfg = force_cfg >= 0 ? force_cfg : conv_pick_cfg(M, op.Cout);
                if (force_cfg < 0 && cfg == 0 && ((M + 127) / 128) * ((op.Cout + 127) / 128) < 128) cfg = 3;
                a.t_flops = 2.0 * op.macs * batch; a.t_bytes = op.bytes * batch;
                if (d.sc_src >= 0 && fold_shortcut && force_cfg < 0) {
                    const POp& x = plan_.ops[d.sc_src];
                    a.wt = P + d.wt_sc; a.bias = P + d.bias_sc; a.Kpad = d.Kpad_sc;
                    a.res = nullptr; a.res_mode = (int)ResMode::NONE;
                    a.sc_in = tensor_ptr(x.in); a.sc_H = x.H; a.sc_W = x.W; a.sc_C = x.Cin; a.sc_stride = x.stride;
                    a.t_flops += 2.0 * x.macs * batch;
                }
                if (d.halo && halo_conv && force_cfg < 0) {
                    launch_conv_halo(a, P + d.wfrag, s);
                    tag = 9;
                    break;
                }
                if (d.w2ok && winograd && force_cfg < 0 && d.sc_src < 0 && wino2_blocks(a) >= wino2_min_blocks()) {
                    a.wt = P + d.w2;
                    launch_wino2(a, s);
                    break;
                }
                const bool use_wino = d.wino && winograd && (long)batch * ((op.H + 3) / 4) * ((op.W + 3) / 4) >= kWinoMinTiles;
                if (use_wino) {
                    const int wcfg = force_cfg >= 0 ? force_cfg : 2;
                    const bool bf2 = bf16x2_ && d.bf2 && force_cfg < 0;
                    WinoPlanes pl;
                    const bool mix = wcfg == 2 && wino_mix_layout(batch, op.H, op.W, op.Cin, op.Cout, &pl);
                    if (!v_ready) {
                        const float* in_s = nullptr; const float* in_t = nullptr;
                        if (d.aff_src >= 0) {
                            a.in = tensor_ptr(plan_.ops[d.aff_src].out);
                            in_s = P + dev_[d.aff_src].s2; in_t = P + dev_[d.aff_src].t2;
                        }
                        if (mix) launch_wino_mix(a, pl, nullptr, wino_v_.as<float>(), 0, in_s, in_t, bf2, s);
                        else launch_wino_input(a, wino_v_.as<float>(), in_s, in_t, bf2, s);
                    }
                    launch_wino_gemm(a, bf2 ? w36_bf_.as<float>() + d.w36p : P + d.w36, wino_v_.as<float>(), wino_m_.as<float>(), wcfg, bf2, s,
                                     mix ? &pl : nullptr);
                    v_ready = false;
                    if (d.fuse_next && fuse_wino && i + 1 < plan_.ops.size()) {
                        const POp& nx = plan_.ops[i + 1];
                        const bool next_wino = dev_[i + 1].wino && (long)batch * ((nx.H + 3) / 4) * ((nx.W + 3) / 4) >= kWinoMinTiles;
                        const bool next_mix = next_wino && wcfg == 2 && wino_mix_layout(batch, nx.H, nx.W, nx.Cin, nx.Cout, nullptr);
                        if (next_wino && mix == next_mix) {
                            ConvArgs e = a;
                            if (!d.fuse_keep_out1) e.out1 = nullptr;
                            const bool pack_next = bf16x2_ && dev_[i + 1].bf2 && force_cfg < 0;
                            if (mix) launch_wino_mix(e, pl, wino_m_.as<float>(), wino_v_.as<float>(), d.fuse_feed_aff ? 1 : 0, nullptr, nullptr, pack_next, s);
                            else launch_wino_fused(e, wino_m_.as<float>(), wino_v_.as<float>(), d.fuse_feed_aff ? 1 : 0, pack_next, s);
                            v_ready = true;
                        }
                    }
                    if (!v_ready) {
                        if (mix) launch_wino_mix(a, pl, wino_m_.as<float>(), nullptr, 0, nullptr, nullptr, false, s);
                        else launch_wino_output(a, wino_m_.as<float>(), s);
                    }
                    tag = 7;
                    break;
                }
                launch_conv(a, cfg, s);
                tag = cfg;
                break;
            }
            case OpKind::DWPW: {
                ConvArgs a{};
                a.in = tensor_ptr(op.in);
                a.wt = P + d.wt; a.bias = P + d.bias;
                a.out1 = tensor_ptr(op.out);
                a.dw_w = P + d.dww; a.dw_b = P + d.dwb; a.dw_act = (int)op.dw_act; a.dw_stride = op.dw_stride;
                a.B = batch; a.H = op.H; a.W = op.W; a.Cin = op.Cin; a.Ho = op.Ho; a.Wo = op.Wo; a.Cout = op.Cout;
                a.ks = 1; a.stride = 1; a.pad = 0; a.Kpad = d.Kpad; a.act = (int)op.act;
                a.t_flops = 2.0 * op.macs * batch; a.t_bytes = op.bytes * batch;
                a.slabs = partial_.as<float>();
                launch_dwpw(a, s);
                break;
            }
            case OpKind::DWCONV:
                launch_dwconv3x3(tensor_ptr(op.in), P + d.wt, P + d.bias, tensor_ptr(op.out), batch, op.H, op.W, op.Cin, op.stride,
                                 (int)op.act, d.has_slope ? P + d.slope : nullptr, s);
                tag = 4;
                break;
            case OpKind::DWGLOBAL:
                launch_dwglobal(tensor_ptr(op.in), P + d.wt, P + d.bias, tensor_ptr(op.out), batch, op.ks * op.ks, op.Cin, (int)op.act,
                                d.has_slope ? P + d.slope : nullptr, s);
                break;
            case OpKind::GCONV:
                launch_gconv3x3(tensor_ptr(op.in), P + d.wt, P + d.bias, tensor_ptr(op.out), batch, op.H, op.W, op.Cin,
                                (int)(op.weight_group), op.stride, (int)op.act, d.has_slope ? P + d.slope : nullptr, s);
                tag = 4;
                break;
            case OpKind::AFFINE:
                launch_affine(tensor_ptr(op.in), P + d.s2, P + d.t2, tensor_ptr(op.out), (long)batch * op.H * op.W, op.Cin, s);
                break;
            case OpKind::ACT:
                launch_act(tensor_ptr(op.in), d.has_slope ? P + d.slope : nullptr, tensor_ptr(op.out), (long)batch * op.H * op.W,
                           op.Cin, (int)op.act, s);
                break;
            case OpKind::ADD:
                launch_add(tensor_ptr(op.in), tensor_ptr(op.in2), tensor_ptr(op.out), (long)batch * op.H * op.W * op.Cin, s);
                break;
            case OpKind::UPSAMPLE:
                launch_upsample2x(tensor_ptr(op.in), tensor_ptr(op.out), batch, op.H, op.W, op.Cin, s);
                break;
        }
        if (!dense) timer.end(s, tag, 2.0 * op.macs * batch, op.bytes * batch);
        if (debug_sync()) {
            fprintf(stderr, "[facehip] op %zu %s batch %d done-launch\n", i, op.name.c_str(), batch); fflush(stderr);
            const hipError_t e1 = hipGetLastError(), e2 = hipStreamSynchronize(s);
            if (e1 != hipSuccess || e2 != hipSuccess)
                throw std::runtime_error("HIP error after op " + std::to_string(i) + " (" + op.name + "): " + hipGetErrorString(e1 != hipSuccess ? e1 : e2));
        }
    }
    FH_HIP(hipGetLastError());
}

Detector::Detector(const std::string& onnx_path) : net_(onnx_path, 640, 640) {
    const auto& outs = net_.plan().outputs;
    const int H = net_.in_h(), W = net_.in_w();
    if (outs.size() == 9) {
        static const int cols[9] = {1, 1, 1, 4, 4, 4, 10, 10, 10};
        static const int strides[3] = {8, 16, 32};
        bool ok = true;
        for (int i = 0; i < 9; ++i) {
            const int s = strides[i % 3];
            ok = ok && outs[i].cols == cols[i] && outs[i].rows == (H / s) * (W / s) * 2;
        }
        if (ok) anchors_ = ((H / 8) * (W / 8) + (H / 16) * (W / 16) + (H / 32) * (W / 32)) * 2;
    } else if (outs.size() >= 1 && outs[0].cols >= 15) {
        predecoded_ = true;
        anchors_ = outs[0].rows;
        feat_ = outs[0].cols;
    }
    cap_ = 1;
    while (cap_ < std::max(anchors_, 1)) cap_ <<= 1;
}

void Detector::reserve(int n, int rows, int cols) {
    (void)rows; (void)cols;
    net_.reserve(n);
    if (n > nb_) {
        nb_ = n;
        cand_.ensure((size_t)n * cap_ * sizeof(FaceRec));
        keys_.ensure((size_t)n * cap_ * sizeof(unsigned long long));
        ws_.ensure((size_t)n * cap_ * sizeof(int));
        count_.ensure((size_t)n * sizeof(int));
    }
}

void Detector::run_network_dev(const uint8_t* frames, int n, int rows, int cols, int step, long stride, hipStream_t s) {
    reserve(n, rows, cols);
    const int inW = net_.in_w(), inH = net_.in_h();
    const float scaleW = (float)inW / (float)cols, scaleH = (float)inH / (float)rows;
    scale_ = std::min(scaleW, scaleH);
    const int newW = (int)((float)cols * scale_), newH = (int)((float)rows * scale_);
    if (newW <= 0 || newH <= 0) throw std::runtime_error("Invalid resize dimensions");
    const uint8_t* src = frames;
    long sstride = stride;
    int sstep = step;
    if (newW != cols || newH != rows) {
        resized_.ensure((size_t)n * newH * newW * 3);
        launch_resize_u8c3(frames, stride, rows, cols, step, resized_.as<uint8_t>(), (long)newH * newW * 3, newH, newW, newW * 3, n, s);
        src = resized_.as<uint8_t>(); sstride = (long)newH * newW * 3; sstep = newW * 3;
    }
    net_.run_u8(src, sstride, newH, newW, sstep, n, s);
}

void Detector::postprocess_dev(int n, float score_thr, float nms_thr, FaceRec* out, int max_out, int* counts, hipStream_t s) {
    if (anchors_ <= 0) { FH_HIP(hipMemsetAsync(counts, 0, (size_t)n * sizeof(int), s)); return; }
    FH_HIP(hipMemsetAsync(count_.p, 0, (size_t)n * sizeof(int), s));
    if (predecoded_) {
        launch_rows_threshold(net_.output(0), n, anchors_, feat_, scale_, score_thr, cand_.as<FaceRec>(),
                              keys_.as<unsigned long long>(), count_.as<int>(), cap_, s);
    } else {
        DecodeArgs a{};
        for (int i = 0; i < 3; ++i) { a.score[i] = net_.output(i); a.bbox[i] = net_.output(3 + i); a.kps[i] = net_.output(6 + i); }
        a.inH = net_.in_h(); a.inW = net_.in_w(); a.B = n; a.scale = scale_; a.thr = score_thr;
        a.cand = cand_.as<FaceRec>(); a.keys = keys_.as<unsigned long long>(); a.count = count_.as<int>(); a.cap = cap_;
        launch_scrfd_decode(a, s);
    }
    launch_sort_nms(cand_.as<FaceRec>(), keys_.as<unsigned long long>(), count_.as<int>(), cap_, n, nms_thr, out, counts, max_out,
                    ws_.as<int>(), s);
    FH_HIP(hipGetLastError());
}

void Detector::detect_dev(const uint8_t* frames, int n, int rows, int cols, int step, long stride, float score_thr, float nms_thr,
                          FaceRec* out, int max_out, int* counts, hipStream_t s) {
    if (n <= 0) return;
    run_network_dev(frames, n, rows, cols, step, stride, s);
    postprocess_dev(n, score_thr, nms_thr, out, max_out, counts, s);
}

Recognizer::Recognizer(const std::string& onnx_path) : net_(onnx_path, 112, 112) {
    const auto& o = net_.plan().outputs.at(0);
    dim_ = o.rows * o.cols;
}

void Recognizer::embed_aligned_dev(const uint8_t* crops, int n, float* out, hipStream_t s, float* raw_out) {
    const int H = net_.in_h(), W = net_.in_w();
    net_.reserve(std::min(n, max_chunk));
    for (int off = 0; off < n; off += max_chunk) {
        const int c = std::min(max_chunk, n - off);
        net_.run_u8(crops + (size_t)off * H * W * 3, (long)H * W * 3, H, W, W * 3, c, s);
        if (raw_out) FH_HIP(hipMemcpyAsync(raw_out + (size_t)off * dim_, net_.output(0), (size_t)c * dim_ * sizeof(float), hipMemcpyDeviceToDevice, s));
        launch_l2_normalize(net_.output(0), out + (size_t)off * dim_, c, dim_, s);
    }
    FH_HIP(hipGetLastError());
}

void Recognizer::align_dev(const uint8_t* frames, int rows, int cols, int step, long stride, const FaceRec* faces,
                           const int* frame_of, int n, uint8_t* crops, int* ok, hipStream_t s) {
    launch_align(frames, stride, rows, cols, step, faces, frame_of, n, net_.in_h(), net_.in_w(), crops, ok, s);
    FH_HIP(hipGetLastError());
}

void Recognizer::embed_faces_dev(const uint8_t* frames, int rows, int cols, int step, long stride, const FaceRec* faces,
                                 const int* frame_of, int n, float* out, int* ok, hipStream_t s) {
    if (n <= 0) return;
    const size_t crop = (size_t)net_.in_h() * net_.in_w() * 3;
    crops_.ensure((size_t)n * crop);
    ok_.ensure((size_t)n * sizeof(int));
    int* okp = ok ? ok : ok_.as<int>();
    align_dev(frames, rows, cols, step, stride, faces, frame_of, n, crops_.as<uint8_t>(), okp, s);
    embed_aligned_dev(crops_.as<uint8_t>(), n, out, s);
}

void Recognizer::resize_embed_dev(const uint8_t* frames, int n, int rows, int cols, int step, long stride, float* out, hipStream_t s) {
    const int H = net_.in_h(), W = net_.in_w();
    crops_.ensure((size_t)n * H * W * 3);
    launch_resize_u8c3(frames, stride, rows, cols, step, crops_.as<uint8_t>(), (long)H * W * 3, H, W, W * 3, n, s);
    embed_aligned_dev(crops_.as<uint8_t>(), n, out, s);
}

void Gallery::upload(const float* rows, long n, bool device_src, long index_base) {
    if (dim_ % 64) throw std::runtime_error("gallery: dim must be a multiple of 64");
    rows_.ensure((size_t)n * dim_ * sizeof(float));
    FH_HIP(hipMemcpy(rows_.p, rows, (size_t)n * dim_ * sizeof(float), device_src ? hipMemcpyDeviceToDevice : hipMemcpyHostToDevice));
    n_ = n; base_ = index_base;
    if (scan_ == 1) {
        rows16_.ensure((size_t)n * dim_ * sizeof(uint16_t));
        convert16(0, n);
    }
}

void Gallery::convert16(long first, long n) {
    gstat_.ensure(4 * sizeof(unsigned));
    if (first == 0) FH_HIP(hipMemset(gstat_.p, 0, 4 * sizeof(unsigned)));
    launch_gallery16_convert(rows_.as<float>() + (size_t)first * dim_, rows16_.as<uint16_t>() + (size_t)first * dim_, n, dim_,
                             gstat_.as<unsigned>(), nullptr);
    FH_HIP(hipGetLastError());
    unsigned h[4];
    FH_HIP(hipMemcpy(h, gstat_.p, sizeof(h), hipMemcpyDeviceToHost));
    for (int i = 0; i < 3; ++i) memcpy(&gbound_[i], &h[i], sizeof(float));
    f16_bad_ = h[3] != 0;
}

void Gallery::set_scan(int mode) {
    if (mode != 0 && mode != 1) throw std::invalid_argument("gallery: unknown scan mode");
    if (mode == 0) {
        DevBuf none;
        std::swap(none.p, rows16_.p);
        std::swap(none.bytes, rows16_.bytes);
        scan_ = 0;
        return;
    }
    if (scan_ != 1) {
        ctr_.ensure(2 * sizeof(unsigned long long));
        FH_HIP(hipMemset(ctr_.p, 0, 2 * sizeof(unsigned long long)));
        if (n_ > 0) {
            rows16_.ensure((size_t)n_ * dim_ * sizeof(uint16_t));
            convert16(0, n_);
        }
        scan_ = 1;
    }
}

void Gallery::scan_stats(long long* certified, long long* fallback) {
    unsigned long long h[2] = {0, 0};
    FH_HIP(hipDeviceSynchronize());
    if (ctr_.p) {
        FH_HIP(hipMemcpy(h, ctr_.p, sizeof(h), hipMemcpyDeviceToHost));
        FH_HIP(hipMemset(ctr_.p, 0, sizeof(h)));
    }
    if (certified) *certified = (long long)h[0];
    if (fallback) *fallback = (long long)h[1] + host_fallback_;
    host_fallback_ = 0;
}

long Gallery::enroll(const float* rows, long n, bool device_src) {
    if (dim_ % 64) throw std::runtime_error("gallery: dim must be a multiple of 64");
    const size_t row_bytes = (size_t)dim_ * sizeof(float);
    const size_t need = (size_t)(n_ + n) * row_bytes;
    if (need > rows_.bytes) {
        DevBuf bigger;
        bigger.ensure(std::max(need, rows_.bytes * 2));
        if (n_ > 0) FH_HIP(hipMemcpy(bigger.p, rows_.p, (size_t)n_ * row_bytes, hipMemcpyDeviceToDevice));
        std::swap(bigger.p, rows_.p);
        std::swap(bigger.bytes, rows_.bytes);
    }
    FH_HIP(hipMemcpy(static_cast<char*>(rows_.p) + (size_t)n_ * row_bytes, rows, (size_t)n * row_bytes,
                     device_src ? hipMemcpyDeviceToDevice : hipMemcpyHostToDevice));
    if (scan_ == 1) {
        const size_t row16 = (size_t)dim_ * sizeof(uint16_t), cap16 = rows_.bytes / row_bytes * row16;
        if (cap16 > rows16_.bytes) {
            DevBuf bigger;
            bigger.ensure(cap16);
            if (n_ > 0) FH_HIP(hipMemcpy(bigger.p, rows16_.p, (size_t)n_ * row16, hipMemcpyDeviceToDevice));
            std::swap(bigger.p, rows16_.p);
            std::swap(bigger.bytes, rows16_.bytes);
        }
        convert16(n_, n);
    }
    const long first = base_ + n_;
    n_ += n;
    return first;
}

void Gallery::label_dev(const float* q, int Q, float thr, int* out_label, float* out_score, hipStream_t s) {
    best_i_.ensure((size_t)std::max(Q, 1) * sizeof(int));
    topk_dev(q, Q, 1, out_score, best_i_.as<int>(), s);
    launch_label(out_score, best_i_.as<int>(), Q, thr, out_label, s);
}

void Gallery::topk_dev(const float* q, int Q, int k, float* out_score, int* out_idx, hipStream_t s) {
    if (Q <= 0 || Q > 256 || k <= 0 || k > 16) throw std::runtime_error("gallery: need 0 < Q <= 256 and 0 < k <= 16");
    if (dim_ % 64) throw std::runtime_error("gallery: dim must be a multiple of 64");
    if (scan_ == 1) {
        if (!f16_bad_ && n_ > 0 && dim_ % 128 == 0) {
            topk_f16(q, Q, k, out_score, out_idx, s);
            return;
        }
// ... 52 lines not shown
```

facerecognizeonnx_amd/csrc/kernels.h:

```cpp
#pragma once
#include <hip/hip_runtime.h>

#include <cstdint>
#include <string>

#include <vector>

namespace fh {

void hip_check(hipError_t e, const char* what);
#define FH_HIP(x) ::fh::hip_check((x), #x)

#if defined(__HIPCC__)
__device__ __forceinline__ void wave_lds_order() {
#if defined(__HIP_DEVICE_COMPILE__)
    __builtin_amdgcn_fence(__ATOMIC_ACQ_REL, "wavefront");
    __builtin_amdgcn_wave_barrier();
#endif
}
#endif

struct KernelTimer {
    static constexpr int kTags = 13;
    bool enabled = false;
    void begin(hipStream_t s);
    void end(hipStream_t s, int tag, double flops, double bytes);
    void collect(double* ms, double* flops, double* bytes, long long* launches);
    int collect_ops(double* ms, double* flops, int* tag, int cap);
    static KernelTimer& get();

  private:
    struct Rec { hipEvent_t a, b; int tag; double flops, bytes; };
    std::vector<Rec> recs_;
    std::vector<hipEvent_t> pool_;
    hipEvent_t cur_ = nullptr;
    hipEvent_t take();
};


struct ConvArgs {
    const float* in;
    const float* wt;
    const float* bias;
    const float* slope;
    const float* res;
    float* out1;
    float* out2;
    const float* s2;
    const float* t2;
    float* slabs;
    const float* zeros;
    int B, H, W, Cin, Ho, Wo, Cout;
    int ks, stride, pad;
    int Kpad;
    int bias_cls;
    const float* sc_in;
    int sc_H, sc_W, sc_C, sc_stride;
    int act;
    int res_mode;
    const float* dw_w;
    const float* dw_b;
    int dw_act;
    int dw_stride;
    const uint8_t* u8_src;
    long u8_img_stride;
    int u8_step, u8_srcH, u8_srcW, u8_inH, u8_inW, u8_stride, stem_act;
    const float* stem_wf;
    const float* stem_bf;
    const unsigned* stem_wfrag;
    int no_prio;
    int no_pw;
    int n_outs;
    float* outs[3];
    int oc0[4];
    int oact[3];
    int sk_enable;
    int cus;
    int wt_group_rows;
    long wt_gs;
    double t_flops, t_bytes;
    int sk_full, sk_units, sk_q, sk_helpers, sk_rem, sk_owner_chunks, sk_maxp;
    unsigned* sk_err;
    int ep_direct;
    unsigned sk_timeout;
    int sk_test_drop;
    int tile0;
};

void launch_conv(const ConvArgs& a, int cfg, hipStream_t s);
int conv_pick_cfg(long M, int Cout);
void conv_workspace_init(float* ws);
void conv_workspace_reset_async(float* ws, hipStream_t s);
unsigned* conv_error_words();
unsigned* conv_error_record_new();
void conv_error_record_release(unsigned* r);
bool conv_take_error(std::string& msg, unsigned* rec);
bool conv_error_pending(const unsigned* rec);
unsigned conv_error_generation();
void conv_debug_streamk(int drop_publish, int timeout_ms);
unsigned conv_debug_generation();
size_t wino2_weight_floats(int Cin, int Cout);
void wino2_pack_weights(const float* w_ohwi, int Cout, int Cin, float* dst);
bool wino2_ok(const ConvArgs& a);
void launch_wino2(const ConvArgs& a, hipStream_t s);
long wino2_blocks(const ConvArgs& a);
double wino2_debug_clock_mhz();
const float* conv_zero_line();
int conv_num_cus();
bool conv_halo_ok(const ConvArgs& a);
size_t conv_halo_wfrag_floats(int Cin, int Cout);
void conv_halo_pack_weights(const float* w_ohwi, int Cout, int Cin, float* dst);
void launch_conv_halo(const ConvArgs& a, const float* wfrag, hipStream_t s);
void stem_pack_wfrag(const float* wf, int Cout, unsigned* out);
bool front_fused_ok(int Cin, int Cout, int dw_stride);
void launch_dwpw(const ConvArgs& a, hipStream_t s);
void launch_conv_winograd(const ConvArgs& a, const float* wt36, float* V, float* M, int cfg, const float* in_scale, const float* in_shift,
                          hipStream_t s);
struct WinoPlanes;
void launch_wino_input(const ConvArgs& a, float* V, const float* in_scale, const float* in_shift, bool pack, hipStream_t s);
void launch_wino_gemm(const ConvArgs& a, const float* wt36, const float* V, float* M, int cfg, bool bf16x2, hipStream_t s,
                      const WinoPlanes* mix = nullptr);
bool wino_gemm_ok_bf16x2(int Cin, int Cout);
void launch_wino_output(const ConvArgs& a, const float* M, hipStream_t s);
bool wino_can_fuse(int H, int W, int C, bool touches_memory);
void launch_wino_fused(const ConvArgs& a, const float* M, float* Vnext, int feed_aff, bool pack_next, hipStream_t s);
void launch_pack_bf16x2(const float* in, float* out, long n, hipStream_t s);
struct WinoPlanes {
    int e[4];
    int t[4];
    int nfc[4];
    int f2[4];
    int n[4];
    int rows[4];
    int base[4];
    int total_tiles;
    int planes;
};
bool wino_mix_layout(int B, int H, int W, int Cin, int Cout, WinoPlanes* out);
void launch_wino_mix(const ConvArgs& a, const WinoPlanes& pl, const float* M, float* Vnext, int feed_aff, const float* in_scale,
                     const float* in_shift, bool pack_next, hipStream_t s);
void wino_filter_transform(const double g[9], double u[36]);
void wino_debug_slots(int slots);
long wino_rows(long tiles);
int conv_wt_rows(int Cout);
size_t conv_slab_floats();
void conv_pack_weights(const float* w, int Cout, int Cin, int ks, float* dst);
inline int conv_kpad(int Ktot) { return (Ktot + 31) / 32 * 32; }

void launch_dwconv3x3(const float* in, const float* w9c, const float* bias, float* out, int B, int H, int W,
                      int C, int stride, int act, const float* slope, hipStream_t s);
void launch_dwglobal(const float* in, const float* w, const float* bias, float* out, int B, int taps, int C, int act, const float* slope,
                     hipStream_t s);
void launch_gconv3x3(const float* in, const float* w, const float* bias, float* out, int B, int H, int W, int C, int G, int stride, int act,
                     const float* slope, hipStream_t s);
void launch_affine(const float* in, const float* sc, const float* sh, float* out, long pixels, int C, hipStream_t s);
void launch_act(const float* in, const float* slope, float* out, long pixels, int C, int act, hipStream_t s);
void launch_add(const float* a, const float* b, float* out, long n, hipStream_t s);
void launch_upsample2x(const float* in, float* out, int B, int H, int W, int C, hipStream_t s);

struct FaceRec {
    int32_t x, y, w, h;
    float score;
    float lm[10];
};

void launch_det_preprocess(const uint8_t* frames, long img_stride, int rows, int cols, int step, int B,
                           int inH, int inW, int newH, int newW, float* out, hipStream_t s);
void launch_rec_preprocess(const uint8_t* crops, int n, int H, int W, float* out, hipStream_t s);
void launch_stem_conv_u8(const uint8_t* src, long img_stride, int srcH, int srcW, int step, int B, int inH, int inW, int stride,
                         int Cout, const float* w27, const float* bias, const float* wf, const float* biasf, const float* slope, int act,
                         float* out1, float* out2, const float* s2, const float* t2, hipStream_t s, const unsigned* wfrag = nullptr);

struct DecodeArgs {
    const float* score[3];
    const float* bbox[3];
    const float* kps[3];
    int inH, inW, B;
    float scale, thr;
    FaceRec* cand;
    unsigned long long* keys;
    int* count;
    int cap;
};
void launch_scrfd_decode(const DecodeArgs& a, hipStream_t s);
void launch_rows_threshold(const float* rows, int B, int n, int feat, float scale, float thr, FaceRec* cand,
                           unsigned long long* keys, int* count, int cap, hipStream_t s);
void launch_sort_nms(const FaceRec* cand, unsigned long long* keys, const int* count, int cap, int B, float nms_thr,
                     FaceRec* out, int* out_count, int max_out, int* order_ws, hipStream_t s);

void launch_align(const uint8_t* frames, long img_stride, int rows, int cols, int step, const FaceRec* faces,
                  const int* frame_of, int n, int outH, int outW, uint8_t* crops, int* ok, hipStream_t s);
void launch_resize_u8c3(const uint8_t* src, long src_stride, int sh, int sw, int sstep, uint8_t* dst, long dst_stride,
                        int dh, int dw, int dstep, int n, hipStream_t s);

void launch_l2_normalize(const float* in, float* out, int n, int dim, hipStream_t s);

int gallery_parts(long G, int Q, int* tiles_per_part);
void launch_gallery_topk(const float* gal, long G, int dim, const float* qpacked, int Q, int k, long idx_base, float* part_score, int* part_idx,
                         float* seed_score, int* seed_idx, hipStream_t s,
                         const int* qcount = nullptr);
void launch_label(const float* best_score, const int* best_idx, int n, float thr, int* labels, hipStream_t s);
void launch_topk_merge(const float* part_score, const int* part_idx, int nparts, int Q, int k, float* out_score,
                       int* out_idx, hipStream_t s, const int* qcount = nullptr);
void launch_topk_merge_strided(const float* part_score, const int* part_idx, int nparts, int Q, int k, long part_stride, float* out_score,
                               int* out_idx, hipStream_t s, const int* qcount = nullptr);

constexpr int GAL16_KC = 32;
void launch_gallery16_convert(const float* rows, uint16_t* rows16, long n, int dim, unsigned* stats, hipStream_t s);
int gallery16_parts(long G, int Q, int* tiles_per_part);
void launch_gallery16_candidates(const uint16_t* rows16, long G, int dim, const float* q, uint16_t* q16, int Q, long idx_base, float* part_score,
                                 int* part_idx, float* seed_score, int* seed_idx, float* cand_score, int* cand_idx, hipStream_t s);
void launch_gallery16_rescore(const float* rows, long G, int dim, const float* q, int Q, int k, long idx_base, const float* cand_score,
                              const int* cand_idx, float gn, float ghn, float dn, float* out_score, int* out_idx, int* fb_count, int* fb_idx,
                              unsigned long long* counters, hipStream_t s);
void launch_gallery16_gather(const float* q, int Q, int dim, const int* fb_count, const int* fb_idx, float* qpacked, hipStream_t s);
void launch_gallery16_scatter(const float* fb_score, const int* fb_idx_out, int Q, int k, const int* fb_count, const int* fb_idx, float* out_score,
                              int* out_idx, hipStream_t s);

void launch_select_faces(const FaceRec* det, const int* counts, int n, int per_frame, int F, FaceRec* faces, int* frame_of,
                         int* total, hipStream_t s);

}
```

facerecognizeonnx_amd/csrc/winograd.hip:

```cpp
#include <hip/hip_runtime.h>

#include <algorithm>
#include <cstdlib>
#include <stdexcept>

#include "kernels.h"
#include "plan.h"

namespace fh {

typedef float v4f __attribute__((ext_vector_type(4)));
typedef float v16f __attribute__((ext_vector_type(16)));
typedef float v2f __attribute__((ext_vector_type(2)));
typedef unsigned v4u __attribute__((ext_vector_type(4)));
typedef __bf16 bf16x2 __attribute__((ext_vector_type(2)));
typedef __bf16 bf16x8 __attribute__((ext_vector_type(8)));

__device__ __forceinline__ v4f wino_pack_bf16x2(const v4f x) {
    v4u out;
#pragma unroll
    for (int p = 0; p < 2; ++p) {
        const v2f a = {x[2 * p], x[2 * p + 1]};
        const unsigned hb = __builtin_bit_cast(unsigned, __builtin_convertvector(a, bf16x2));
        const v2f r = {a[0] - __builtin_bit_cast(float, hb << 16), a[1] - __builtin_bit_cast(float, hb & 0xffff0000u)};
        const unsigned mb = __builtin_bit_cast(unsigned, __builtin_convertvector(r, bf16x2));
        out[2 * p] = (hb & 0xffffu) | (mb << 16);
        out[2 * p + 1] = (hb >> 16) | (mb & 0xffff0000u);
    }
    return __builtin_bit_cast(v4f, out);
}

__global__ __launch_bounds__(256) void pack_bf16x2_kernel(const float* __restrict__ in, float* __restrict__ out, long n4) {
    for (long i = (long)blockIdx.x * blockDim.x + threadIdx.x; i < n4; i += (long)gridDim.x * blockDim.x)
        *reinterpret_cast<v4f*>(out + 4 * i) = wino_pack_bf16x2(*reinterpret_cast<const v4f*>(in + 4 * i));
}
void launch_pack_bf16x2(const float* in, float* out, long n, hipStream_t s) {
    const long n4 = n / 4;
    if (n4 > 0) hipLaunchKernelGGL(pack_bf16x2_kernel, dim3((unsigned)std::min<long>((n4 + 255) / 256, 256 * 64)), dim3(256), 0, s, in, out, n4);
}

__device__ __forceinline__ void wino_bt(const v4f (&d)[6], v4f (&t)[6]) {
    t[0] = 4.f * d[0] - 5.f * d[2] + d[4];
    t[1] = -4.f * d[1] - 4.f * d[2] + d[3] + d[4];
    t[2] = 4.f * d[1] - 4.f * d[2] - d[3] + d[4];
    t[3] = -2.f * d[1] - d[2] + 2.f * d[3] + d[4];
    t[4] = 2.f * d[1] - d[2] - 2.f * d[3] + d[4];
    t[5] = 4.f * d[1] - 5.f * d[3] + d[5];
}
__device__ __forceinline__ void wino_at(const v4f (&m)[6], v4f (&y)[4]) {
    y[0] = m[0] + m[1] + m[2] + m[3] + m[4];
    y[1] = m[1] - m[2] + 2.f * m[3] - 2.f * m[4];
    y[2] = m[1] + m[2] + 4.f * m[3] + 4.f * m[4];
    y[3] = m[1] - m[2] + 8.f * m[3] - 8.f * m[4] + m[5];
}

__global__ __launch_bounds__(256, 2) void wino_input_kernel(const float* __restrict__ in, float* __restrict__ V, int B, int H, int W,
                                                            int C, int TY, int TX, long NTp, const float* __restrict__ aff_s,
                                                            const float* __restrict__ aff_t, const int pack) {
    const int C4 = C >> 2;
    const int NT = B * TY * TX;
    const int total = NT * C4;
    for (int idx = blockIdx.x * blockDim.x + threadIdx.x; idx < total; idx += gridDim.x * blockDim.x) {
        const int c4 = idx % C4;
        const int tile = idx / C4;
        const int tx = tile % TX, ty = (tile / TX) % TY, b = tile / (TX * TY);
        const int iy0 = 4 * ty - 1, ix0 = 4 * tx - 1;
        const float* img = in + (size_t)b * H * W * C + c4 * 4;
        v4f as4 = {1.f, 1.f, 1.f, 1.f}, at4 = {0.f, 0.f, 0.f, 0.f};
        if (aff_s) { as4 = *reinterpret_cast<const v4f*>(aff_s + c4 * 4); at4 = *reinterpret_cast<const v4f*>(aff_t + c4 * 4); }
        v4f t[6][6];
#pragma unroll
        for (int c = 0; c < 6; ++c) {
            const int ix = ix0 + c;
            v4f d[6];
#pragma unroll
            for (int r = 0; r < 6; ++r) {
                const int iy = iy0 + r;
                const bool ok = (unsigned)iy < (unsigned)H && (unsigned)ix < (unsigned)W;
                const v4f raw = *reinterpret_cast<const v4f*>(img + (ok ? ((size_t)iy * W + ix) * C : (size_t)0));
                const float okf = ok ? 1.f : 0.f;
                d[r] = raw * (as4 * okf) + at4 * okf;
            }
            v4f tc[6];
            wino_bt(d, tc);
#pragma unroll
            for (int i = 0; i < 6; ++i) t[i][c] = tc[i];
        }
        float* dst = V + (size_t)tile * C + c4 * 4;
        const size_t fs = (size_t)NTp * C;
#pragma unroll
        for (int i = 0; i < 6; ++i) {
            v4f o[6];
            wino_bt(t[i], o);
#pragma unroll
            for (int j = 0; j < 6; ++j) *reinterpret_cast<v4f*>(dst + (size_t)(i * 6 + j) * fs) = pack ? wino_pack_bf16x2(o[j]) : o[j];
        }
    }
}

struct WinoOutArgs {
    const float* M; const float* bias; const float* slope; const float* res; float* out1; float* out2; const float* s2; const float* t2;
    int B, H, W, C, TY, TX, act;
    long NTp;
};

__global__ __launch_bounds__(256, 2) void wino_output_kernel(const WinoOutArgs p) {
    const int C = p.C, C4 = C >> 2;
    const int NT = p.B * p.TY * p.TX;
    const int total = NT * C4;
    const size_t fs = (size_t)p.NTp * C;
    for (int idx = blockIdx.x * blockDim.x + threadIdx.x; idx < total; idx += gridDim.x * blockDim.x) {
        const int c4 = idx % C4;
        const int tile = idx / C4;
        const int tx = tile % p.TX, ty = (tile / p.TX) % p.TY, b = tile / (p.TX * p.TY);
        const float* src = p.M + (size_t)tile * C + c4 * 4;
        v4f t[4][6];
#pragma unroll
        for (int j = 0; j < 6; ++j) {
            v4f m[6];
#pragma unroll
            for (int i = 0; i < 6; ++i) m[i] = *reinterpret_cast<const v4f*>(src + (size_t)(i * 6 + j) * fs);
            v4f y[4];
            wino_at(m, y);
#pragma unroll
            for (int r = 0; r < 4; ++r) t[r][j] = y[r];
        }
        const v4f b4 = p.bias ? *reinterpret_cast<const v4f*>(p.bias + c4 * 4) : v4f{0.f, 0.f, 0.f, 0.f};
        v4f sl = {0.f, 0.f, 0.f, 0.f}, s2 = sl, t2 = sl;
        if (p.act == (int)Act::PRELU) sl = *reinterpret_cast<const v4f*>(p.slope + c4 * 4);
        if (p.out2) { s2 = *reinterpret_cast<const v4f*>(p.s2 + c4 * 4); t2 = *reinterpret_cast<const v4f*>(p.t2 + c4 * 4); }
#pragma unroll
        for (int r = 0; r < 4; ++r) {
            const int oy = 4 * ty + r;
            if (oy >= p.H) continue;
            v4f y[4];
            wino_at(t[r], y);
            v4f rs[4];
            if (p.res) {
#pragma unroll
                for (int x = 0; x < 4; ++x)
                    rs[x] = *reinterpret_cast<const v4f*>(p.res + (((size_t)b * p.H + oy) * p.W + min(4 * tx + x, p.W - 1)) * C + c4 * 4);
            }
#pragma unroll
            for (int x = 0; x < 4; ++x) {
                const int ox = 4 * tx + x;
                if (ox >= p.W) continue;
                v4f v = y[x] + b4;
#pragma unroll
                for (int e = 0; e < 4; ++e) {
                    float u = v[e];
                    if (p.act == (int)Act::RELU) u = u > 0.f ? u : 0.f;
                    else if (p.act == (int)Act::PRELU) u = u >= 0.f ? u : u * sl[e];
                    else if (p.act == (int)Act::SIGMOID) u = 1.0f / (1.0f + expf(-u));
                    v[e] = u;
                }
                const size_t o = (((size_t)b * p.H + oy) * p.W + ox) * C + c4 * 4;
                if (p.res) v += rs[x];
                if (p.out1) *reinterpret_cast<v4f*>(p.out1 + o) = v;
                if (p.out2) *reinterpret_cast<v4f*>(p.out2 + o) = v * s2 + t2;
            }
        }
    }
}

struct WinoFuseArgs {
    WinoOutArgs o;
    float* V;
    int feed_aff;
    int csl4, pitch, img;
    int pack;
};

__global__ __launch_bounds__(256, 2) void wino_fused_kernel(const WinoFuseArgs a) {
    const WinoOutArgs& p = a.o;
    extern __shared__ v4f act[];
    const int C = p.C, TPI = p.TY * p.TX, IMG = a.img, HW = p.H * p.W, PITCH = a.pitch;
    const int tid = threadIdx.x, c4l = tid % a.csl4, slot = tid / a.csl4;
    const int cslices = C / (4 * a.csl4);
    const int cs = blockIdx.x % cslices, b0 = (blockIdx.x / cslices) * IMG;
    const int il = slot / TPI, tile = slot - il * TPI;
    const int ty = tile / p.TX, tx = tile - ty * p.TX;
    const int b = b0 + il;
    const bool live = il < IMG && b < p.B;
    const int c4 = cs * a.csl4 + c4l;
    const size_t fs = (size_t)p.NTp * C;
    const size_t tg = ((size_t)b * p.TY + ty) * p.TX + tx;
    if (live) {
        const float* src = p.M + tg * C + c4 * 4;
        v4f t[4][6];
#pragma unroll
        for (int j = 0; j < 6; ++j) {
            v4f m[6];
#pragma unroll
            for (int i = 0; i < 6; ++i) m[i] = *reinterpret_cast<const v4f*>(src + (size_t)(i * 6 + j) * fs);
            v4f y[4];
            wino_at(m, y);
#pragma unroll
            for (int r = 0; r < 4; ++r) t[r][j] = y[r];
        }
        const v4f b4 = p.bias ? *reinterpret_cast<const v4f*>(p.bias + c4 * 4) : v4f{0.f, 0.f, 0.f, 0.f};
        v4f rs[4][4];
        if (p.res) {
#pragma unroll
            for (int r = 0; r < 4; ++r)
#pragma unroll
                for (int x = 0; x < 4; ++x) {
                    const int oy = 4 * ty + r, ox = 4 * tx + x;
                    rs[r][x] = *reinterpret_cast<const v4f*>(p.res + (((size_t)b * p.H + min(oy, p.H - 1)) * p.W + min(ox, p.W - 1)) * C + c4 * 4);
                }
        }
        v4f sl = {0.f, 0.f, 0.f, 0.f}, s2 = {1.f, 1.f, 1.f, 1.f}, t2 = {0.f, 0.f, 0.f, 0.f};
        if (p.act == (int)Act::PRELU) sl = *reinterpret_cast<const v4f*>(p.slope + c4 * 4);
        if (p.s2) { s2 = *reinterpret_cast<const v4f*>(p.s2 + c4 * 4); t2 = *reinterpret_cast<const v4f*>(p.t2 + c4 * 4); }
#pragma unroll
        for (int r = 0; r < 4; ++r) {
            const int oy = 4 * ty + r;
            if (oy >= p.H) continue;
            v4f y[4];
            wino_at(t[r], y);
#pragma unroll
            for (int x = 0; x < 4; ++x) {
                const int ox = 4 * tx + x;
                if (ox >= p.W) continue;
                v4f v = y[x] + b4;
#pragma unroll
                for (int e = 0; e < 4; ++e) {
                    float u = v[e];
                    if (p.act == (int)Act::RELU) u = u > 0.f ? u : 0.f;
                    else if (p.act == (int)Act::PRELU) u = u >= 0.f ? u : u * sl[e];
                    else if (p.act == (int)Act::SIGMOID) u = 1.0f / (1.0f + expf(-u));
                    v[e] = u;
                }
                const size_t o = (((size_t)b * p.H + oy) * p.W + ox) * C + c4 * 4;
                if (p.res) v += rs[r][x];
                if (p.out1) *reinterpret_cast<v4f*>(p.out1 + o) = v;
                const v4f vb = v * s2 + t2;
                if (p.out2) *reinterpret_cast<v4f*>(p.out2 + o) = vb;
                act[(il * HW + oy * p.W + ox) * PITCH + c4l] = a.feed_aff ? vb : v;
            }
        }
    }
    __syncthreads();
    if (!live) return;
    const v4f* img = act + (size_t)il * HW * PITCH + c4l;
    const int iy0 = 4 * ty - 1, ix0 = 4 * tx - 1;
    v4f tt[6][6];
#pragma unroll
    for (int c = 0; c < 6; ++c) {
        const int ix = ix0 + c;
        v4f d[6];
#pragma unroll
        for (int r = 0; r < 6; ++r) {
            const int iy = iy0 + r;
            const bool ok = (unsigned)iy < (unsigned)p.H && (unsigned)ix < (unsigned)p.W;
            d[r] = ok ? img[(iy * p.W + ix) * PITCH] : v4f{0.f, 0.f, 0.f, 0.f};
        }
        v4f tc[6];
        wino_bt(d, tc);
#pragma unroll
        for (int i = 0; i < 6; ++i) tt[i][c] = tc[i];
    }
    float* dst = a.V + tg * C + c4 * 4;
#pragma unroll
    for (int i = 0; i < 6; ++i) {
        v4f o6[6];
        wino_bt(tt[i], o6);
#pragma unroll
        for (int j = 0; j < 6; ++j) *reinterpret_cast<v4f*>(dst + (size_t)(i * 6 + j) * fs) = a.pack ? wino_pack_bf16x2(o6[j]) : o6[j];
    }
}

constexpr int kSliceThreads = 448, kSliceTiles = kSliceThreads / 8;
__device__ __forceinline__ int wino_slice_slot(int x) { return (x & ~5) | ((x >> 2) & 1) | ((x & 1) << 2); }

__global__ __launch_bounds__(kSliceThreads) void wino_slice_kernel(const WinoFuseArgs a) {
    const WinoOutArgs& p = a.o;
    extern __shared__ v4f act[];
    const int C = p.C, TPI = p.TY * p.TX;
    const int tid = threadIdx.x, c4l = tid & 7, tile = tid >> 3;
    const int cslices = C >> 5;
    int blk = blockIdx.x;
    if ((p.B & 7) == 0) { const int x = blk & 7, j = blk >> 3; blk = ((j / cslices) * 8 + x) * cslices + j % cslices; }
    const int cs = blk % cslices, b = blk / cslices;
    const int ty = tile / p.TX, tx = tile - ty * p.TX;
    const bool live = tile < TPI;
    const int c4 = cs * 8 + c4l;
    const size_t fs = (size_t)p.NTp * C;
    const bool slice_nt = a.img == 2;
    const size_t tg = ((size_t)b * p.TY + ty) * p.TX + tx;
    if (live) {
        const float* src = p.M + tg * C + c4 * 4;
        v4f t[4][6];
#pragma unroll
        for (int j = 0; j < 6; ++j) {
            v4f m[6];
#pragma unroll
            for (int i = 0; i < 6; ++i) m[i] = slice_nt ? __builtin_nontemporal_load(reinterpret_cast<const v4f*>(src + (size_t)(i * 6 + j) * fs)) : *reinterpret_cast<const v4f*>(src + (size_t)(i * 6 + j) * fs);
            v4f y[4];
            wino_at(m, y);
#pragma unroll
            for (int r = 0; r < 4; ++r) t[r][j] = y[r];
        }
        const v4f b4 = p.bias ? *reinterpret_cast<const v4f*>(p.bias + c4 * 4) : v4f{0.f, 0.f, 0.f, 0.f};
        v4f rs[4][4];
        if (p.res) {
#pragma unroll
            for (int r = 0; r < 4; ++r)
#pragma unroll
                for (int x = 0; x < 4; ++x) {
                    const int oy = 4 * ty + r, ox = 4 * tx + x;
                    rs[r][x] = *reinterpret_cast<const v4f*>(p.res + (((size_t)b * p.H + min(oy, p.H - 1)) * p.W + min(ox, p.W - 1)) * C + c4 * 4);
                }
        }
        v4f sl = {0.f, 0.f, 0.f, 0.f}, s2 = {1.f, 1.f, 1.f, 1.f}, t2 = {0.f, 0.f, 0.f, 0.f};
        if (p.act == (int)Act::PRELU) sl = *reinterpret_cast<const v4f*>(p.slope + c4 * 4);
        if (p.s2) { s2 = *reinterpret_cast<const v4f*>(p.s2 + c4 * 4); t2 = *reinterpret_cast<const v4f*>(p.t2 + c4 * 4); }
#pragma unroll
        for (int r = 0; r < 4; ++r) {
            const int oy = 4 * ty + r;
            if (oy >= p.H) continue;
            v4f y[4];
            wino_at(t[r], y);
#pragma unroll
            for (int x = 0; x < 4; ++x) {
                const int ox = 4 * tx + x;
                if (ox >= p.W) continue;
                v4f v = y[x] + b4;
#pragma unroll
                for (int e = 0; e < 4; ++e) {
                    float u = v[e];
                    if (p.act == (int)Act::RELU) u = u > 0.f ? u : 0.f;
                    else if (p.act == (int)Act::PRELU) u = u >= 0.f ? u : u * sl[e];
                    else if (p.act == (int)Act::SIGMOID) u = 1.0f / (1.0f + expf(-u));
                    v[e] = u;
                }
                const size_t o = (((size_t)b * p.H + oy) * p.W + ox) * C + c4 * 4;
                if (p.res) v += rs[r][x];
                if (p.out1) *reinterpret_cast<v4f*>(p.out1 + o) = v;
                const v4f vb = v * s2 + t2;
                if (p.out2) *reinterpret_cast<v4f*>(p.out2 + o) = vb;
                act[(oy * 32 + wino_slice_slot(ox)) * 8 + c4l] = a.feed_aff ? vb : v;
            }
        }
    }
    __syncthreads();
    if (!live) return;
    const v4f* img = act + c4l;
    const int iy0 = 4 * ty - 1, ix0 = 4 * tx - 1;
    v4f tt[6][6];
#pragma unroll
    for (int c = 0; c < 6; ++c) {
        const int ix = ix0 + c;
        const int sx = wino_slice_slot(ix & 31);
        v4f d[6];
#pragma unroll
        for (int r = 0; r < 6; ++r) {
            const int iy = iy0 + r;
            const bool ok = (unsigned)iy < (unsigned)p.H && (unsigned)ix < (unsigned)p.W;
            d[r] = ok ? img[(iy * 32 + sx) * 8] : v4f{0.f, 0.f, 0.f, 0.f};
        }
        v4f tc[6];
        wino_bt(d, tc);
#pragma unroll
        for (int i = 0; i < 6; ++i) tt[i][c] = tc[i];
    }
    float* dst = a.V + tg * C + c4 * 4;
#pragma unroll
    for (int i = 0; i < 6; ++i) {
        v4f o6[6];
        wino_bt(tt[i], o6);
#pragma unroll
        for (int j = 0; j < 6; ++j) *reinterpret_cast<v4f*>(dst + (size_t)(i * 6 + j) * fs) = a.pack ? wino_pack_bf16x2(o6[j]) : o6[j];
    }
}

static int wino_slice_enabled() {
    static int v = -1;
    if (v < 0) { const char* e = getenv("FACEHIP_WINO_SLICE"); v = e ? atoi(e) : 1; }
    return v;
}
static bool wino_slice_shape(int H, int W, int C) {
    const int tpi = ((H + 3) / 4) * ((W + 3) / 4);
    return wino_slice_enabled() && C % 32 == 0 && tpi > 16 && tpi <= kSliceTiles && W <= 32 && (size_t)H * 32 * 8 * sizeof(v4f) <= 160 * 1024;
}

__device__ __forceinline__ void wino_dma16(const float* src, v4f* dst) {
#if defined(__HIP_DEVICE_COMPILE__)
    __builtin_amdgcn_global_load_lds(src, (__attribute__((address_space(3))) void*)dst, 16, 0, 0);
#else
    (void)src; (void)dst;
#endif
}

__device__ __forceinline__ int wino_plane_freq(const WinoPlanes& pl, const int tile_m) {
    const int c = tile_m >= pl.e[3] ? 3 : tile_m >= pl.e[2] ? 2 : tile_m >= pl.e[1] ? 1 : 0;
    const int pln = (tile_m - pl.e[c]) / pl.t[c];
    const int nfc = pl.nfc[c], f2 = pl.f2[c];
    int i = pln / nfc, j = pln - i * nfc;
    if ((f2 & 2) && i == 3) i = 5;
    if ((f2 & 1) && j == 3) j = 5;
    return 6 * i + j;
}

template <int TN>
__device__ __forceinline__ void wino_store_lines(const v16f (&acc)[TN], float* scratch, size_t scratch_bytes, float* __restrict__ M, int N,
                                                 int m0, int n0, int wid, int lane) {
    constexpr int JB = TN >= 2 ? 2 : 1, W = JB * 32;
    constexpr int PITCH = W + 4, RPI = 64 / (W / 4);
    static_assert(TN % JB == 0, "store scratch");
    (void)scratch_bytes;
    const int fr = lane & 31, fh2 = lane >> 5;
    float* const blk = scratch + wid * 32 * PITCH;
    const int rr = lane / (W / 4), cq = lane % (W / 4);
#pragma unroll
    for (int h = 0; h < TN / JB; ++h) {
        wave_lds_order();
#pragma unroll
        for (int jj = 0; jj < JB; ++jj)
#pragma unroll
            for (int g = 0; g < 4; ++g) {
                const int j = h * JB + jj;
                *reinterpret_cast<v4f*>(blk + fr * PITCH + jj * 32 + 8 * g + 4 * fh2) = v4f{acc[j][4 * g], acc[j][4 * g + 1], acc[j][4 * g + 2], acc[j][4 * g + 3]};
            }
        wave_lds_order();
        float* const obase = M + (size_t)(m0 + wid * 32 + rr) * N + n0 + h * W + 4 * cq;
#pragma unroll
        for (int i = 0; i < 32 / RPI; ++i)
            *reinterpret_cast<v4f*>(obase + (size_t)i * RPI * N) = *reinterpret_cast<const v4f*>(blk + (rr + i * RPI) * PITCH + 4 * cq);
    }
}

#ifdef FACEHIP_WINO_STAMP
__device__ unsigned long long g_wino_stamp[8 * 4096];
extern "C" __attribute__((visibility("default"))) int fh_debug_wino_stamps(unsigned long long* host, int n) {
    return hipMemcpyFromSymbol(host, HIP_SYMBOL(g_wino_stamp), sizeof(unsigned long long) * (size_t)(n < 8 * 4096 ? n : 8 * 4096)) == hipSuccess ? 0 : -1;
}
#define WINO_STAMP(i) if (tid == 0 && blockIdx.x < 4096) g_wino_stamp[blockIdx.x * 8 + (i)] = __builtin_amdgcn_s_memrealtime()
#else
#define WINO_STAMP(i)
#endif
template <int BN, int OCC, int ABL = 0>
__global__ __launch_bounds__(256, OCC) void wino_gemm_kernel(const float* __restrict__ V, const float* __restrict__ U, float* __restrict__ M,
                                                            const int K, const int N, const WinoPlanes pl, const long wt_gs,
                                                            const int tiles_n, const int chunks) {
    constexpr int BM = 128, TN = BN / 32, AL = BM / 32, BL = BN / 32;
    __shared__ v4f lds[2][(BM + BN) * 8];
    const int tid = threadIdx.x, lane = tid & 63;
    WINO_STAMP(0);
    const int wid = __builtin_amdgcn_readfirstlane(tid >> 6);
    const int fr = lane & 31, fh2 = lane >> 5, fsw = (fr >> 1) & 7;
    const int nb = gridDim.x, q = nb >> 3, r8 = nb & 7, x = blockIdx.x & 7;
    const int tile = x * q + min(x, r8) + (blockIdx.x >> 3);
    const int tile_n = tile % tiles_n, tile_m = tile / tiles_n;
    const int m0 = tile_m * BM, n0 = tile_n * BN;
    const float* Ug = U + (size_t)wino_plane_freq(pl, tile_m) * wt_gs;

    const int lrow = tid >> 3;
    const int lqs = (tid & 7) ^ ((lrow >> 1) & 7);
    const float* a_src = V + (size_t)(m0 + lrow) * K + lqs * 4;
    const float* b_src = Ug + (size_t)(n0 + lrow) * K + lqs * 4;
    const size_t row32 = (size_t)32 * K;
    v4f* const dstA = &lds[0][wid * 64];
    v4f* const dstB = &lds[0][BM * 8 + wid * 64];
    auto load_chunk = [&](int buf) {
        v4f* const dA = dstA + buf * ((BM + BN) * 8);
        v4f* const dB = dstB + buf * ((BM + BN) * 8);
#pragma unroll
        for (int i = 0; i < AL; ++i) wino_dma16(a_src + i * row32, dA + i * 32 * 8);
#pragma unroll
        for (int i = 0; i < BL; ++i) wino_dma16(b_src + i * row32, dB + i * 32 * 8);
        a_src += 32; b_src += 32;
    };
    v16f acc[TN];
#pragma unroll
    for (int j = 0; j < TN; ++j)
#pragma unroll
        for (int e = 0; e < 16; ++e) acc[j][e] = 0.f;
    load_chunk(0);
    __syncthreads();
    WINO_STAMP(1);
    v4f xk = v4f{0.f, 0.f, 0.f, 0.f}, wk[TN];
    if constexpr ((ABL & 2) != 0) {
        xk = lds[0][(wid * 32 + fr) * 8 + (fh2 ^ fsw)];
#pragma unroll
        for (int j = 0; j < TN; ++j) wk[j] = lds[0][BM * 8 + fr * 8 + j * 32 * 8 + (fh2 ^ fsw)];
    }
    for (int kc = 0; kc < chunks; ++kc) {
        const int buf = (ABL & 1) ? 0 : (kc & 1);
        if ((ABL & 1) == 0 && kc + 1 < chunks) load_chunk(buf ^ 1);
        const v4f* X = lds[buf] + (wid * 32 + fr) * 8;
        const v4f* Wt = lds[buf] + BM * 8 + fr * 8;
#pragma unroll
        for (int s = 0; s < 4; ++s) {
            const int col = (2 * s + fh2) ^ fsw;
            v4f xv;
            v4f w[TN];
            if constexpr ((ABL & 2) != 0) {
                xv = xk;
#pragma unroll
                for (int j = 0; j < TN; ++j) w[j] = wk[j];
#if defined(__HIP_DEVICE_COMPILE__)
                asm volatile("" : "+v"(xv));
#endif
            } else {
                xv = X[col];
#pragma unroll
                for (int j = 0; j < TN; ++j) w[j] = Wt[j * 32 * 8 + col];
            }
#pragma unroll
            for (int e = 0; e < 4; ++e)
#pragma unroll
                for (int j = 0; j < TN; ++j) acc[j] = __builtin_amdgcn_mfma_f32_32x32x2f32(w[j][e], xv[e], acc[j], 0, 0, 0);
        }
        if constexpr ((ABL & 4) == 0) __syncthreads();
    }
    WINO_STAMP(2);
    if constexpr ((ABL & 8) != 0) { if (acc[0][0] != 123.456f) return; }
    if constexpr ((ABL & 16) == 0) {
        static_assert(4 * 32 * ((TN >= 2 ? 64 : 32) + 4) * sizeof(float) <= sizeof(lds), "store scratch");
        wino_store_lines<TN>(acc, reinterpret_cast<float*>(&lds[0][0]), sizeof(lds), M, N, m0, n0, wid, lane);
        WINO_STAMP(3);
#ifdef FACEHIP_WINO_STAMP
        asm volatile("s_waitcnt vmcnt(0)" ::: "memory");
        WINO_STAMP(4);
        if (tid == 0 && blockIdx.x < 4096) { g_wino_stamp[blockIdx.x * 8 + 5] = (unsigned long long)tile; g_wino_stamp[blockIdx.x * 8 + 6] = __builtin_amdgcn_s_getreg((3 << 11) | 20); }
#endif
        return;
    }
    float* orow = M + (size_t)(m0 + wid * 32 + fr) * N + n0 + 4 * fh2;
#pragma unroll
    for (int j = 0; j < TN; ++j)
#pragma unroll
        for (int g = 0; g < 4; ++g)
            *reinterpret_cast<v4f*>(orow + j * 32 + 8 * g) = v4f{acc[j][4 * g], acc[j][4 * g + 1], acc[j][4 * g + 2], acc[j][4 * g + 3]};
}

template <int BN, int OCC>
__global__ __launch_bounds__(256, OCC) void wino_gemm_pers_kernel(const float* __restrict__ V, const float* __restrict__ U, float* __restrict__ M,
                                                                 const int K, const int N, const WinoPlanes pl, const long wt_gs,
                                                                 const int tiles_n, const int chunks, const int ntiles) {
    constexpr int BM = 128, TN = BN / 32, AL = BM / 32, BL = BN / 32;
    constexpr int BUF = (BM + BN) * 8;
    __shared__ v4f lds[2][BUF];
    const int tid = threadIdx.x, lane = tid & 63;
    const int wid = __builtin_amdgcn_readfirstlane(tid >> 6);
    const int fr = lane & 31, fh2 = lane >> 5, fsw = (fr >> 1) & 7;
    const int lrow = tid >> 3;
    const int lqs = (tid & 7) ^ ((lrow >> 1) & 7);
    const size_t row32 = (size_t)32 * K;
    const int q = ntiles >> 3, r8 = ntiles & 7;
    auto tile_of = [&](int vb) { const int x = vb & 7; return x * q + min(x, r8) + (vb >> 3); };
    const float* a_src; const float* b_src;
    auto point_at = [&](int tile) {
        const int tile_n = tile % tiles_n, tile_m = tile / tiles_n;
        const float* Ug = U + (size_t)wino_plane_freq(pl, tile_m) * wt_gs;
        a_src = V + (size_t)(tile_m * BM + lrow) * K + lqs * 4;
        b_src = Ug + (size_t)(tile_n * BN + lrow) * K + lqs * 4;
    };
    auto load_chunk = [&](int buf) {
        v4f* const dA = &lds[0][wid * 64] + buf * BUF;
        v4f* const dB = &lds[0][BM * 8 + wid * 64] + buf * BUF;
#pragma unroll
        for (int i = 0; i < AL; ++i) wino_dma16(a_src + i * row32, dA + i * 32 * 8);
#pragma unroll
        for (int i = 0; i < BL; ++i) wino_dma16(b_src + i * row32, dB + i * 32 * 8);
        a_src += 32; b_src += 32;
    };
    constexpr int JB = 1, W = JB * 32, PITCH = W + 4, RPI = 64 / (W / 4);
    static_assert(4 * 32 * PITCH * sizeof(float) <= BUF * sizeof(v4f), "store scratch must fit ONE tile buffer");
    constexpr int NSTORE = TN * (32 / RPI);
    int base = 0;
    int vb = blockIdx.x;
    point_at(tile_of(vb));
    load_chunk(0);
    __syncthreads();
    for (;;) {
        const int tile = tile_of(vb);
        const int m0 = (tile / tiles_n) * BM, n0 = (tile % tiles_n) * BN;
        v16f acc[TN];
#pragma unroll
        for (int j = 0; j < TN; ++j)
#pragma unroll
            for (int e = 0; e < 16; ++e) acc[j][e] = 0.f;
        for (int kc = 0; kc < chunks; ++kc) {
            const int buf = (base + kc) & 1;
            if (kc + 1 < chunks) load_chunk(buf ^ 1);
            const v4f* X = lds[buf] + (wid * 32 + fr) * 8;
            const v4f* Wt = lds[buf] + BM * 8 + fr * 8;
#pragma unroll
            for (int s4 = 0; s4 < 4; ++s4) {
                const int col = (2 * s4 + fh2) ^ fsw;
                const v4f xv = X[col];
                v4f w[TN];
#pragma unroll
                for (int j = 0; j < TN; ++j) w[j] = Wt[j * 32 * 8 + col];
#pragma unroll
                for (int e = 0; e < 4; ++e)
#pragma unroll
                    for (int j = 0; j < TN; ++j) acc[j] = __builtin_amdgcn_mfma_f32_32x32x2f32(w[j][e], xv[e], acc[j], 0, 0, 0);
            }
            __syncthreads();
        }
        const int last = (base + chunks - 1) & 1;
        const int nvb = vb + gridDim.x;
        const bool more = nvb < ntiles;
        if (more) {
            point_at(tile_of(nvb));
            load_chunk(last ^ 1);
#if defined(__HIP_DEVICE_COMPILE__)
            __builtin_amdgcn_sched_barrier(0);
#endif
        }
        {
            float* const blk = reinterpret_cast<float*>(&lds[last][0]) + wid * 32 * PITCH;
            const int rr = lane / (W / 4), cq = lane % (W / 4);
#pragma unroll
            for (int j = 0; j < TN; ++j) {
                wave_lds_order();
#pragma unroll
                for (int g = 0; g < 4; ++g)
                    *reinterpret_cast<v4f*>(blk + fr * PITCH + 8 * g + 4 * fh2) = v4f{acc[j][4 * g], acc[j][4 * g + 1], acc[j][4 * g + 2], acc[j][4 * g + 3]};
                wave_lds_order();
                float* const obase = M + (size_t)(m0 + wid * 32 + rr) * N + n0 + j * W + 4 * cq;
#pragma unroll
                for (int i = 0; i < 32 / RPI; ++i)
                    *reinterpret_cast<v4f*>(obase + (size_t)i * RPI * N) = *reinterpret_cast<const v4f*>(blk + (rr + i * RPI) * PITCH + 4 * cq);
            }
        }
        if (!more) break;
        vb = nvb; base = last ^ 1;
#if defined(__HIP_DEVICE_COMPILE__)
        asm volatile("s_waitcnt vmcnt(%0) lgkmcnt(0)" ::"n"(NSTORE) : "memory");
        __builtin_amdgcn_s_barrier();
        __builtin_amdgcn_sched_barrier(0);
#endif
    }
}

template <int BN, int OCC>
__global__ __launch_bounds__(256, OCC) void wino_gemm_bf16x2_kernel(const float* __restrict__ V, const float* __restrict__ U, float* __restrict__ M,
                                                                   const int K, const int N, const WinoPlanes pl, const long wt_gs,
                                                                   const int tiles_n, const int chunks) {
    constexpr int BM = 128, TN = BN / 32, AL = BM / 32, BL = BN / 32;
    __shared__ v4f lds[2][(BM + BN) * 8];
    const int tid = threadIdx.x, lane = tid & 63;
    const int wid = __builtin_amdgcn_readfirstlane(tid >> 6);
    const int fr = lane & 31, fh2 = lane >> 5, fsw = (fr >> 1) & 7;
    const int nb = gridDim.x, q = nb >> 3, r8 = nb & 7, x = blockIdx.x & 7;
    const int tile = x * q + min(x, r8) + (blockIdx.x >> 3);
    const int tile_n = tile % tiles_n, tile_m = tile / tiles_n;
    const int m0 = tile_m * BM, n0 = tile_n * BN;
    const float* Ug = U + (size_t)wino_plane_freq(pl, tile_m) * wt_gs;
    const int lrow = tid >> 3;
    const int lqs = (tid & 7) ^ ((lrow >> 1) & 7);
    const float* a_src = V + (size_t)(m0 + lrow) * K + lqs * 4;
    const float* b_src = Ug + (size_t)(n0 + lrow) * K + lqs * 4;
    const size_t row32 = (size_t)32 * K;
    v4f* const dstA = &lds[0][wid * 64];
    v4f* const dstB = &lds[0][BM * 8 + wid * 64];
    auto load_chunk = [&](int buf) {
        v4f* const dA = dstA + buf * ((BM + BN) * 8);
        v4f* const dB = dstB + buf * ((BM + BN) * 8);
#pragma unroll
        for (int i = 0; i < AL; ++i) wino_dma16(a_src + i * row32, dA + i * 32 * 8);
#pragma unroll
        for (int i = 0; i < BL; ++i) wino_dma16(b_src + i * row32, dB + i * 32 * 8);
        a_src += 32; b_src += 32;
    };
    auto split = [](const v4u lo4, const v4u hi4, bf16x8& h, bf16x8& m) {
        const v4u hh = {__builtin_amdgcn_perm(lo4[1], lo4[0], 0x05040100u), __builtin_amdgcn_perm(lo4[3], lo4[2], 0x05040100u),
                        __builtin_amdgcn_perm(hi4[1], hi4[0], 0x05040100u), __builtin_amdgcn_perm(hi4[3], hi4[2], 0x05040100u)};
        const v4u mm = {__builtin_amdgcn_perm(lo4[1], lo4[0], 0x07060302u), __builtin_amdgcn_perm(lo4[3], lo4[2], 0x07060302u),
                        __builtin_amdgcn_perm(hi4[1], hi4[0], 0x07060302u), __builtin_amdgcn_perm(hi4[3], hi4[2], 0x07060302u)};
        h = __builtin_bit_cast(bf16x8, hh); m = __builtin_bit_cast(bf16x8, mm);
    };
    v16f acc[TN];
#pragma unroll
    for (int j = 0; j < TN; ++j)
#pragma unroll
        for (int e = 0; e < 16; ++e) acc[j][e] = 0.f;
    load_chunk(0);
    __syncthreads();
    for (int kc = 0; kc < chunks; ++kc) {
        const int buf = kc & 1;
        if (kc + 1 < chunks) load_chunk(buf ^ 1);
        const v4u* X = reinterpret_cast<const v4u*>(lds[buf]) + (wid * 32 + fr) * 8;
        const v4u* Wt = reinterpret_cast<const v4u*>(lds[buf]) + BM * 8 + fr * 8;
#pragma unroll
        for (int ks = 0; ks < 2; ++ks) {
            const int c0 = (4 * ks + 2 * fh2) ^ fsw, c1 = (4 * ks + 2 * fh2 + 1) ^ fsw;
            bf16x8 xh, xm;
            split(X[c0], X[c1], xh, xm);
#pragma unroll
            for (int j = 0; j < TN; ++j) {
                bf16x8 wh, wm;
                split(Wt[j * 32 * 8 + c0], Wt[j * 32 * 8 + c1], wh, wm);
                acc[j] = __builtin_amdgcn_mfma_f32_32x32x16_bf16(wm, xh, acc[j], 0, 0, 0);
                acc[j] = __builtin_amdgcn_mfma_f32_32x32x16_bf16(wh, xm, acc[j], 0, 0, 0);
                acc[j] = __builtin_amdgcn_mfma_f32_32x32x16_bf16(wh, xh, acc[j], 0, 0, 0);
            }
        }
        __syncthreads();
    }
    static_assert(4 * 32 * ((TN >= 2 ? 64 : 32) + 4) * sizeof(float) <= sizeof(lds), "store scratch");
    wino_store_lines<TN>(acc, reinterpret_cast<float*>(&lds[0][0]), sizeof(lds), M, N, m0, n0, wid, lane);
}

long wino_rows(long tiles) { return (tiles + 255) / 256 * 256; }

static inline int wino_grid(long n) {
    const long b = (n + 255) / 256;
    return (int)(b < 1 ? 1 : b > 256 * 16 ? 256 * 16 : b);
}

void wino_filter_transform(const double g[9], double u[36]) {
    static const double G[6][3] = {{1.0 / 4, 0, 0},          {-1.0 / 6, -1.0 / 6, -1.0 / 6}, {-1.0 / 6, 1.0 / 6, -1.0 / 6},
                                   {1.0 / 24, 1.0 / 12, 1.0 / 6}, {1.0 / 24, -1.0 / 12, 1.0 / 6},  {0, 0, 1}};
    double t[6][3];
    for (int i = 0; i < 6; ++i)
        for (int kx = 0; kx < 3; ++kx) t[i][kx] = G[i][0] * g[0 * 3 + kx] + G[i][1] * g[1 * 3 + kx] + G[i][2] * g[2 * 3 + kx];
    for (int i = 0; i < 6; ++i)
        for (int j = 0; j < 6; ++j) u[i * 6 + j] = t[i][0] * G[j][0] + t[i][1] * G[j][1] + t[i][2] * G[j][2];
}

static void wino_check(long NT, int cmax) {
    if (NT * (cmax / 4) >= (1L << 31) || 36 * (NT + 256) >= (1L << 31))
        throw std::runtime_error("winograd: batch too large for the 32-bit tile index (split the batch)");
}

void launch_wino_input(const ConvArgs& a, float* V, const float* in_scale, const float* in_shift, bool pack, hipStream_t s) {
    const int TY = (a.H + 3) / 4, TX = (a.W + 3) / 4;
    const long NT = (long)a.B * TY * TX;
    if (NT <= 0) return;
    wino_check(NT, std::max(a.Cin, a.Cout));
    KernelTimer& timer = KernelTimer::get();
    timer.begin(s);
    hipLaunchKernelGGL(wino_input_kernel, dim3(wino_grid(NT * (a.Cin >> 2))), dim3(256), 0, s, a.in, V, a.B, a.H, a.W, a.Cin, TY, TX, wino_rows(NT), in_scale,
                       in_shift, pack ? 1 : 0);
    timer.end(s, 8, 0.0, 0.0);
}

bool wino_gemm_ok_bf16x2(int Cin, int Cout) { return Cout % 64 == 0 && Cin % 32 == 0; }

static int g_wino_slots_override = 0;
void wino_debug_slots(int slots) { g_wino_slots_override = slots > 0 ? (slots + 7) / 8 * 8 : 0; }
static long wino_slots(int occ, int cus) {
    if (g_wino_slots_override) return g_wino_slots_override;
    const long s = (long)occ * (cus > 0 ? cus : 256) / 8 * 8;
    return s < 8 ? 8 : s;
}

static int wino_pers_enabled() {
    static int v = -1;
    if (v < 0) { const char* e = getenv("FACEHIP_WINO_PERS"); v = e ? atoi(e) : 0; }
    return v || g_wino_slots_override;
}

static int wino_mix_enabled() {
    static int v = -1;
    if (v < 0) { const char* e = getenv("FACEHIP_WINO_MIX"); v = e ? atoi(e) : 1; }
    return v;
}

static bool wino_bn128(bool mixed) {
    static int v = -1;
    if (v < 0) { const char* e = getenv("FACEHIP_WINO_BN128"); v = e ? atoi(e) : 1; }
    return v == 2 || (v == 1 && mixed);
}

static bool wino_pick_bn128(long row_tiles, int Cout, bool mixed, int cus) {
    static const int force = [] { const char* e = getenv("FACEHIP_WINO_BN128"); return e ? atoi(e) : -1; }();
    if (force >= 0) return wino_bn128(mixed);
    const long sw = wino_slots(2, cus), sn = wino_slots(3, cus);
    const long wide = (row_tiles * (Cout / 128) + sw - 1) / sw * 4, narrow = (row_tiles * (Cout / 64) + sn - 1) / sn * 3;
    if (wide != narrow) return wide < narrow;
    return wino_bn128(mixed);
}

bool wino_mix_layout(int B, int H, int W, int Cin, int Cout, WinoPlanes* out) {
    const int TY = (H + 3) / 4, TX = (W + 3) / 4;
    const int my = (H & 3) == 1 || (H & 3) == 2, mx = (W & 3) == 1 || (W & 3) == 2;
    if (!wino_mix_enabled() || !(my || mx) || TY * TX != 16 || Cin % 64 || Cout % 64 || B < 64) return false;
    if ((size_t)H * W * 16 * sizeof(v4f) > 64 * 1024) return false;
    WinoPlanes pl{};
    const int n[4] = {(TY - my) * (TX - mx), (TY - my) * mx, my * (TX - mx), my * mx};
    int tile = 0, row = 0, planes = 0;
    for (int c = 0; c < 4; ++c) {
        const int nfr = (c & 2) ? 4 : 6, nfc = (c & 1) ? 4 : 6;
        pl.n[c] = n[c]; pl.nfc[c] = nfc; pl.f2[c] = c;
        pl.rows[c] = (B * n[c] + 127) / 128 * 128;
        pl.t[c] = pl.rows[c] / 128;
        pl.e[c] = tile; pl.base[c] = row;
        tile += nfr * nfc * pl.t[c]; row += nfr * nfc * pl.rows[c];
        if (n[c]) planes += nfr * nfc;
    }
    if ((long)row * std::max(Cin, Cout) * 4 >= (1L << 31)) return false;
    pl.total_tiles = tile; pl.planes = planes;
    if (out) *out = pl;
    return true;
}

void launch_wino_gemm(const ConvArgs& a, const float* wt36, const float* V, float* M, int cfg, bool bf16x2, hipStream_t s, const WinoPlanes* mix) {
    const int TY = (a.H + 3) / 4, TX = (a.W + 3) / 4;
    const long NT = (long)a.B * TY * TX;
    if (NT <= 0) return;
    const long NTp = wino_rows(NT);
    KernelTimer& timer = KernelTimer::get();
    ConvArgs g{};
    g.in = V; g.wt = wt36; g.out1 = M; g.slabs = a.slabs; g.sk_err = a.sk_err; g.sk_enable = a.sk_enable; g.cus = a.cus;
    g.B = (int)(36 * NTp); g.H = g.W = g.Ho = g.Wo = 1; g.Cin = a.Cin; g.Cout = a.Cout; g.ks = 1; g.stride = 1; g.pad = 0; g.Kpad = a.Cin;
    g.act = (int)Act::NONE; g.res_mode = (int)ResMode::NONE;
    g.wt_group_rows = (int)NTp; g.wt_gs = (long)conv_wt_rows(a.Cout) * a.Cin;
    g.t_flops = 2.0 * 36.0 * (double)NT * a.Cin * a.Cout; g.t_bytes = a.t_flops;
    WinoPlanes pl{};
    if (mix) {
        if (!(a.Cout % 32 == 0 && cfg == 2)) throw std::runtime_error("winograd: the mixed tiling runs on the lean GEMM kernel only");
        pl = *mix;
        double real_rows = 0;
        for (int c = 0; c < 4; ++c) real_rows += (double)((c & 2) ? 4 : 6) * pl.nfc[c] * a.B * pl.n[c];
        g.t_flops = 2.0 * real_rows * a.Cin * a.Cout;
    } else {
        pl.e[0] = 0; pl.e[1] = pl.e[2] = pl.e[3] = (int)(36 * NTp / 128); pl.t[0] = (int)(NTp / 128); pl.nfc[0] = 6;
        pl.total_tiles = pl.e[1];
    }
    if (a.Cout % 32 == 0 && cfg == 2) {
        const long rows = 128L * pl.total_tiles;
        const int chunks = a.Cin / 32;
        const bool wide = a.Cout % 64 == 0;
        timer.begin(s);
        if (bf16x2) {
            if (!wino_gemm_ok_bf16x2(a.Cin, a.Cout)) throw std::runtime_error("winograd: this layer has no split-bf16 GEMM");
            hipLaunchKernelGGL((wino_gemm_bf16x2_kernel<64, 3>), dim3((unsigned)((rows / 128) * (a.Cout / 64))), dim3(256), 0, s, V, wt36, M, a.Cin,
                               a.Cout, pl, g.wt_gs, a.Cout / 64, chunks);
        } else if (wide && a.Cout % 128 == 0 && wino_pick_bn128(rows / 128, a.Cout, mix != nullptr, a.cus)) {
            const long nt = (rows / 128) * (a.Cout / 128), slots = wino_slots(2, a.cus);
            if (wino_pers_enabled() && nt > slots)
                hipLaunchKernelGGL((wino_gemm_pers_kernel<128, 2>), dim3((unsigned)slots), dim3(256), 0, s, V, wt36, M, a.Cin, a.Cout, pl, g.wt_gs,
                                   a.Cout / 128, chunks, (int)nt);
            else
                hipLaunchKernelGGL((wino_gemm_kernel<128, 2>), dim3((unsigned)nt), dim3(256), 0, s, V, wt36, M, a.Cin, a.Cout, pl, g.wt_gs, a.Cout / 128,
                                   chunks);
        } else if (wide && wino_pers_enabled() && (rows / 128) * (a.Cout / 64) > wino_slots(3, a.cus)) {
            const long nt = (rows / 128) * (a.Cout / 64), slots = wino_slots(3, a.cus);
            hipLaunchKernelGGL((wino_gemm_pers_kernel<64, 3>), dim3((unsigned)slots), dim3(256), 0, s, V, wt36, M, a.Cin, a.Cout, pl, g.wt_gs, a.Cout / 64,
                               chunks, (int)nt);
        } else if (wide) {
#ifdef FACEHIP_WINO_ABL
            static const int abl = [] { const char* e = getenv("FACEHIP_WINO_ABL"); return e ? atoi(e) : 0; }();
            const dim3 grid((unsigned)((rows / 128) * (a.Cout / 64)));
#define WABL(X) case X: hipLaunchKernelGGL((wino_gemm_kernel<64, 3, X>), grid, dim3(256), 0, s, V, wt36, M, a.Cin, a.Cout, pl, g.wt_gs, a.Cout / 64, chunks); break;
            switch (abl) { WABL(1) WABL(2) WABL(3) WABL(4) WABL(5) WABL(6) WABL(7) WABL(8) WABL(15) WABL(16) WABL(17) WABL(24)
                default: hipLaunchKernelGGL((wino_gemm_kernel<64, 3>), grid, dim3(256), 0, s, V, wt36, M, a.Cin, a.Cout, pl, g.wt_gs, a.Cout / 64, chunks); }
#undef WABL
#else
            hipLaunchKernelGGL((wino_gemm_kernel<64, 3>), dim3((unsigned)((rows / 128) * (a.Cout / 64))), dim3(256), 0, s, V, wt36, M, a.Cin, a.Cout,
                                   pl, g.wt_gs, a.Cout / 64, chunks);
#endif
        }
        else
            hipLaunchKernelGGL((wino_gemm_kernel<32, 4>), dim3((unsigned)((rows / 128) * (a.Cout / 32))), dim3(256), 0, s, V, wt36, M, a.Cin, a.Cout,
                               pl, g.wt_gs, a.Cout / 32, chunks);
        timer.end(s, 7, g.t_flops, g.t_bytes);
    } else {
        if (bf16x2) throw std::runtime_error("winograd: this layer has no split-bf16 GEMM");
        launch_conv(g, cfg, s);
    }
}

static WinoOutArgs wino_out_args(const ConvArgs& a, const float* M) {
    const int TY = (a.H + 3) / 4, TX = (a.W + 3) / 4;
    WinoOutArgs o{};
    o.M = M; o.bias = a.bias; o.slope = a.slope; o.res = a.res; o.out1 = a.out1; o.out2 = a.out2; o.s2 = a.s2; o.t2 = a.t2;
    o.B = a.B; o.H = a.H; o.W = a.W; o.C = a.Cout; o.TY = TY; o.TX = TX; o.act = a.act; o.NTp = wino_rows((long)a.B * TY * TX);
    return o;
}

void launch_wino_output(const ConvArgs& a, const float* M, hipStream_t s) {
    const WinoOutArgs o = wino_out_args(a, M);
    const long NT = (long)a.B * o.TY * o.TX;
    if (NT <= 0) return;
    KernelTimer& timer = KernelTimer::get();
    timer.begin(s);
    hipLaunchKernelGGL(wino_output_kernel, dim3(wino_grid(NT * (a.Cout >> 2))), dim3(256), 0, s, o);
    timer.end(s, 8, 0.0, 0.0);
}

static bool wino_fuse_shape(int H, int W, int C, int* csl4, int* pitch, int* img) {
    const int tpi = ((H + 3) / 4) * ((W + 3) / 4);
    int c = 0, pt = 0, im = 0;
    if (C % 64 == 0 && tpi <= 16 && (tpi & (tpi - 1)) == 0) { c = 16; pt = 16; im = 16 / tpi; }
    else if (C % 16 == 0 && tpi <= 64) { c = 4; pt = 5; im = 64 / tpi; }
    else return false;
    if ((size_t)im * H * W * pt * sizeof(v4f) > 64 * 1024) return false;
    if (csl4) { *csl4 = c; *pitch = pt; *img = im; }
    return true;
}
bool wino_can_fuse(int H, int W, int C, bool touches_memory) {
    if (wino_slice_shape(H, W, C)) return true;
    int csl4 = 0, pitch = 0, img = 0;
    if (!wino_fuse_shape(H, W, C, &csl4, &pitch, &img)) return false;
    return csl4 == 16 || !touches_memory;
}

void launch_wino_fused(const ConvArgs& a, const float* M, float* Vnext, int feed_aff, bool pack_next, hipStream_t s) {
    WinoFuseArgs f{};
    if (wino_slice_shape(a.H, a.W, a.Cout)) {
        f.o = wino_out_args(a, M);
        f.V = Vnext; f.feed_aff = feed_aff; f.pack = pack_next ? 1 : 0; f.csl4 = 8; f.pitch = 8; f.img = wino_slice_enabled() == 2 ? 2 : 1;
        if (a.B <= 0) return;
        wino_check((long)a.B * f.o.TY * f.o.TX, a.Cout);
        const size_t lds = (size_t)a.H * 32 * 8 * sizeof(v4f);
        static const bool attr = [] {
            FH_HIP(hipFuncSetAttribute(reinterpret_cast<const void*>(&wino_slice_kernel), hipFuncAttributeMaxDynamicSharedMemorySize, 160 * 1024));
            return true;
        }();
        (void)attr;
        KernelTimer& timer = KernelTimer::get();
        timer.begin(s);
        hipLaunchKernelGGL(wino_slice_kernel, dim3((unsigned)(a.B * (a.Cout / 32))), dim3(kSliceThreads), lds, s, f);
        timer.end(s, 8, 0.0, 0.0);
        return;
    }
    if (!wino_fuse_shape(a.H, a.W, a.Cout, &f.csl4, &f.pitch, &f.img)) throw std::runtime_error("winograd: this map cannot take the fused transform");
    f.o = wino_out_args(a, M);
    f.V = Vnext; f.feed_aff = feed_aff; f.pack = pack_next ? 1 : 0;
    const long NT = (long)a.B * f.o.TY * f.o.TX;
    if (NT <= 0) return;
    wino_check(NT, a.Cout);
    const size_t lds = (size_t)f.img * a.H * a.W * f.pitch * sizeof(v4f);
    KernelTimer& timer = KernelTimer::get();
    timer.begin(s);
    hipLaunchKernelGGL(wino_fused_kernel, dim3((unsigned)(((a.B + f.img - 1) / f.img) * (a.Cout / (4 * f.csl4)))), dim3(256), lds, s, f);
    timer.end(s, 8, 0.0, 0.0);
}

struct WinoMixArgs {
    WinoOutArgs o;
    WinoPlanes pl;
    const float* in; const float* in_s; const float* in_t;
    float* V;
    unsigned plane_bytes;
    int feed_aff, pack;
};

__device__ __forceinline__ void wino_bt2s(const v4f (&d)[6], v4f (&t)[6]) {
    t[0] = 4.f * (d[0] - d[2]);
    t[1] = -3.f * (d[1] + d[2]);
    t[2] = 3.f * (d[1] - d[2]);
    t[3] = d[1] - d[3];
    t[4] = v4f{0.f, 0.f, 0.f, 0.f};
    t[5] = t[4];
}

__global__ __launch_bounds__(256, 2) void wino_mix_kernel(const WinoMixArgs a) {
    const WinoOutArgs& p = a.o;
    extern __shared__ v4f act[];
    const int C = p.C, HW = p.H * p.W;
    const int tid = threadIdx.x, c4l = tid & 15, tile = tid >> 4;
    const int cslices = C >> 6;
    const int cs = blockIdx.x % cslices, b = blockIdx.x / cslices;
    const int ty = tile / p.TX, tx = tile - ty * p.TX;
    const int my = a.pl.n[2] + a.pl.n[3] > 0, mx = a.pl.n[1] + a.pl.n[3] > 0;
    const bool rF2 = my && ty == p.TY - 1, cF2 = mx && tx == p.TX - 1;
    const int nfr = rF2 ? 4 : 6, nfc = cF2 ? 4 : 6;
    const int n_c = rF2 ? (cF2 ? a.pl.n[3] : a.pl.n[2]) : (cF2 ? a.pl.n[1] : a.pl.n[0]);
    const int rows_c = rF2 ? (cF2 ? a.pl.rows[3] : a.pl.rows[2]) : (cF2 ? a.pl.rows[1] : a.pl.rows[0]);
    const int base_c = rF2 ? (cF2 ? a.pl.base[3] : a.pl.base[2]) : (cF2 ? a.pl.base[1] : a.pl.base[0]);
    const int lidx = rF2 ? (cF2 ? 0 : tx) : (cF2 ? ty : ty * (p.TX - mx) + tx);
    const int c4 = cs * 16 + c4l;
    const unsigned off0 = (unsigned)(((base_c + b * n_c + lidx) * C + c4 * 4) * 4);
    const unsigned pstride = (unsigned)rows_c * (unsigned)C * 4u;
    constexpr unsigned OOB = 0x80000000u;
    if (p.M) {
        const __amdgpu_buffer_rsrc_t rm = __builtin_amdgcn_make_buffer_rsrc(const_cast<float*>(p.M), 0, a.plane_bytes, 0x00020000);
        v4f t[4][6];
#pragma unroll
        for (int j = 0; j < 6; ++j) {
            v4f m[6];
#pragma unroll
            for (int i = 0; i < 6; ++i) {
                const bool ok = i < nfr && j < nfc;
                m[i] = __builtin_bit_cast(v4f, __builtin_amdgcn_raw_buffer_load_b128(rm, ok ? off0 + (unsigned)(i * nfc + j) * pstride : OOB, 0, 0));
            }
            v4f y4[4];
            wino_at(m, y4);
            const v4f y20 = m[0] + m[1] + m[2], y21 = m[1] - m[2] - m[3];
            t[0][j] = rF2 ? y20 : y4[0];
            t[1][j] = rF2 ? y21 : y4[1];
            t[2][j] = y4[2];
            t[3][j] = y4[3];
        }
        const v4f b4 = p.bias ? *reinterpret_cast<const v4f*>(p.bias + c4 * 4) : v4f{0.f, 0.f, 0.f, 0.f};
        v4f rs[4][4];
        if (p.res) {
#pragma unroll
            for (int r = 0; r < 4; ++r)
#pragma unroll
                for (int x = 0; x < 4; ++x) {
                    const int oy = 4 * ty + r, ox = 4 * tx + x;
                    rs[r][x] = *reinterpret_cast<const v4f*>(p.res + (((size_t)b * p.H + min(oy, p.H - 1)) * p.W + min(ox, p.W - 1)) * C + c4 * 4);
                }
        }
        v4f sl = {0.f, 0.f, 0.f, 0.f}, s2 = {1.f, 1.f, 1.f, 1.f}, t2 = {0.f, 0.f, 0.f, 0.f};
        if (p.act == (int)Act::PRELU) sl = *reinterpret_cast<const v4f*>(p.slope + c4 * 4);
        if (p.s2) { s2 = *reinterpret_cast<const v4f*>(p.s2 + c4 * 4); t2 = *reinterpret_cast<const v4f*>(p.t2 + c4 * 4); }
#pragma unroll
        for (int r = 0; r < 4; ++r) {
            const int oy = 4 * ty + r;
            if (oy >= p.H) continue;
            v4f y[4];
            wino_at(t[r], y);
            if (cF2) { y[0] = t[r][0] + t[r][1] + t[r][2]; y[1] = t[r][1] - t[r][2] - t[r][3]; }
#pragma unroll
            for (int x = 0; x < 4; ++x) {
                const int ox = 4 * tx + x;
                if (ox >= p.W) continue;
                v4f v = y[x] + b4;
#pragma unroll
                for (int e = 0; e < 4; ++e) {
                    float u = v[e];
                    if (p.act == (int)Act::RELU) u = u > 0.f ? u : 0.f;
                    else if (p.act == (int)Act::PRELU) u = u >= 0.f ? u : u * sl[e];
                    else if (p.act == (int)Act::SIGMOID) u = 1.0f / (1.0f + expf(-u));
                    v[e] = u;
                }
                const size_t o = (((size_t)b * p.H + oy) * p.W + ox) * C + c4 * 4;
                if (p.res) v += rs[r][x];
                if (p.out1) *reinterpret_cast<v4f*>(p.out1 + o) = v;
                const v4f vb = v * s2 + t2;
                if (p.out2) *reinterpret_cast<v4f*>(p.out2 + o) = vb;
                act[(oy * p.W + ox) * 16 + c4l] = a.feed_aff ? vb : v;
            }
        }
    } else {
        v4f as4 = {1.f, 1.f, 1.f, 1.f}, at4 = {0.f, 0.f, 0.f, 0.f};
        if (a.in_s) { as4 = *reinterpret_cast<const v4f*>(a.in_s + c4 * 4); at4 = *reinterpret_cast<const v4f*>(a.in_t + c4 * 4); }
        const float* src = a.in + (size_t)b * HW * C + c4 * 4;
        for (int px = tile; px < HW; px += 16) act[px * 16 + c4l] = *reinterpret_cast<const v4f*>(src + (size_t)px * C) * as4 + at4;
    }
    if (!a.V) return;
    __syncthreads();
    const __amdgpu_buffer_rsrc_t rv = __builtin_amdgcn_make_buffer_rsrc(a.V, 0, a.plane_bytes, 0x00020000);
    const v4f* img = act + c4l;
    const int iy0 = 4 * ty - 1, ix0 = 4 * tx - 1;
    v4f tt[6][6];
#pragma unroll
    for (int c = 0; c < 6; ++c) {
        const int ix = ix0 + c;
        v4f d[6];
#pragma unroll
        for (int r = 0; r < 6; ++r) {
            const int iy = iy0 + r;
            const bool ok = (unsigned)iy < (unsigned)p.H && (unsigned)ix < (unsigned)p.W;
            d[r] = ok ? img[(iy * p.W + ix) * 16] : v4f{0.f, 0.f, 0.f, 0.f};
        }
        v4f t4[6], t2s[6];
        wino_bt(d, t4);
        wino_bt2s(d, t2s);
#pragma unroll
        for (int i = 0; i < 6; ++i) tt[i][c] = rF2 ? t2s[i] : t4[i];
    }
#pragma unroll
    for (int i = 0; i < 6; ++i) {
        v4f o4[6], o2[6];
        wino_bt(tt[i], o4);
        wino_bt2s(tt[i], o2);
#pragma unroll
        for (int j = 0; j < 6; ++j) {
            const bool ok = i < nfr && j < nfc;
            const v4f o = cF2 ? o2[j] : o4[j];
            __builtin_amdgcn_raw_buffer_store_b128(__builtin_bit_cast(v4u, a.pack ? wino_pack_bf16x2(o) : o), rv,
                                                   ok ? off0 + (unsigned)(i * nfc + j) * pstride : OOB, 0, 0);
        }
    }
}

void launch_wino_mix(const ConvArgs& a, const WinoPlanes& pl, const float* M, float* Vnext, int feed_aff, const float* in_scale,
                     const float* in_shift, bool pack_next, hipStream_t s) {
    if (a.B <= 0) return;
    WinoMixArgs f{};
    f.o = wino_out_args(a, M);
    if (!M) { f.o.C = a.Cin; f.o.res = nullptr; f.o.out1 = f.o.out2 = nullptr; }
    f.pl = pl;
    f.in = a.in; f.in_s = in_scale; f.in_t = in_shift;
    f.V = Vnext; f.feed_aff = feed_aff; f.pack = pack_next ? 1 : 0;
    long rows = 0;
    for (int c = 0; c < 4; ++c) rows += (long)((c & 2) ? 4 : 6) * pl.nfc[c] * pl.rows[c];
    f.plane_bytes = (unsigned)(rows * f.o.C * 4);
    if (f.o.C % 64 || f.o.TY * f.o.TX != 16 || rows * f.o.C * 4 >= (1L << 31)) throw std::runtime_error("winograd: this map cannot take the mixed tiling");
    const size_t lds = (size_t)a.H * a.W * 16 * sizeof(v4f);
    KernelTimer& timer = KernelTimer::get();
    timer.begin(s);
    hipLaunchKernelGGL(wino_mix_kernel, dim3((unsigned)(a.B * (f.o.C / 64))), dim3(256), lds, s, f);
    timer.end(s, 8, 0.0, 0.0);
}

void launch_conv_winograd(const ConvArgs& a, const float* wt36, float* V, float* M, int cfg, const float* in_scale, const float* in_shift,
                          hipStream_t s) {
    WinoPlanes pl;
    if (cfg == 2 && wino_mix_layout(a.B, a.H, a.W, a.Cin, a.Cout, &pl)) {
        launch_wino_mix(a, pl, nullptr, V, 0, in_scale, in_shift, false, s);
        launch_wino_gemm(a, wt36, V, M, cfg, false, s, &pl);
        launch_wino_mix(a, pl, M, nullptr, 0, nullptr, nullptr, false, s);
        return;
    }
    launch_wino_input(a, V, in_scale, in_shift, false, s);
    launch_wino_gemm(a, wt36, V, M, cfg, false, s);
    launch_wino_output(a, M, s);
}

}
```

include/facehip.h:

```cpp
#ifndef FACEHIP_H_
#define FACEHIP_H_

#include <stddef.h>
#include <stdint.h>

#ifdef __cplusplus
extern "C" {
#endif

#define FH_API __attribute__((visibility("default")))

enum fh_status { FH_OK = 0, FH_ERR_ARG = -1, FH_ERR_MODEL = -2, FH_ERR_DEVICE = -3, FH_ERR_STATE = -4 };

typedef struct fh_face {
    int32_t x, y, w, h;
    float score;
    float lm[10];
} fh_face;

typedef struct fh_det fh_det;
typedef struct fh_rec fh_rec;
typedef struct fh_gallery fh_gallery;

FH_API const char* fh_version(void);
FH_API const char* fh_last_error(void);
FH_API int fh_init(int device);

FH_API int fh_plan_describe(const char* onnx_path, int default_h, int default_w, char* buf, int cap);
FH_API int fh_onnx_dump(const char* onnx_path, char* buf, int cap);

FH_API fh_det* fh_det_create(const char* onnx_path);
FH_API void fh_det_destroy(fh_det* d);
FH_API int fh_det_input_size(const fh_det* d, int* width, int* height);
FH_API int fh_det_num_anchors(const fh_det* d);
FH_API double fh_det_macs_per_frame(const fh_det* d);
FH_API double fh_det_act_bytes_per_frame(const fh_det* d);
FH_API int fh_det_detect(fh_det* d, const uint8_t* bgr, int rows, int cols, int step, float score_thr, float nms_thr,
                         fh_face* out, int max_out);
FH_API int fh_det_detect_batch_dev(fh_det* d, const uint8_t* d_frames, int n, int rows, int cols, int step,
                                   long long frame_stride, float score_thr, float nms_thr, fh_face* d_out,
                                   int max_per_frame, int* d_counts, void* stream);
FH_API int fh_det_run_network_dev(fh_det* d, const uint8_t* d_frames, int n, int rows, int cols, int step,
                                  long long frame_stride, void* stream);
FH_API int fh_det_num_outputs(const fh_det* d);
FH_API const float* fh_det_output_dev(fh_det* d, int index, int* rows, int* cols);
FH_API const float* fh_det_input_dev(fh_det* d);
FH_API int fh_det_postprocess_dev(fh_det* d, int n, float score_thr, float nms_thr, fh_face* d_out, int max_per_frame,
                                  int* d_counts, void* stream);
FH_API int fh_postprocess_rows_dev(const float* d_rows, int n, int rows_per_frame, int feat, float scale, float score_thr,
                                   float nms_thr, fh_face* d_out, int max_per_frame, int* d_counts, void* stream);

FH_API fh_rec* fh_rec_create(const char* onnx_path);
FH_API void fh_rec_destroy(fh_rec* r);
FH_API int fh_rec_input_size(const fh_rec* r, int* width, int* height);
FH_API int fh_rec_feature_dim(const fh_rec* r);
FH_API double fh_rec_macs_per_face(const fh_rec* r);
FH_API double fh_rec_act_bytes_per_face(const fh_rec* r);
FH_API int fh_rec_set_chunk(fh_rec* r, int faces_per_pass);
FH_API int fh_rec_extract(fh_rec* r, const uint8_t* bgr, int rows, int cols, int step, const fh_face* face, float* out,
                          int out_cap);
FH_API int fh_rec_extract_simple(fh_rec* r, const uint8_t* bgr, int rows, int cols, int step, float* out, int out_cap);
FH_API float fh_compare(const float* f1, int n1, const float* f2, int n2);
FH_API int fh_rec_embed_aligned_dev(fh_rec* r, const uint8_t* d_crops, int n, float* d_out, float* d_raw, void* stream);
FH_API int fh_det_sync(fh_det* d, void* stream);
FH_API int fh_rec_sync(fh_rec* r, void* stream);
FH_API int fh_rec_align_dev(fh_rec* r, const uint8_t* d_frames, int rows, int cols, int step, long long frame_stride,
                            const fh_face* d_faces, const int* d_frame_of, int n, uint8_t* d_crops, int* d_ok,
                            void* stream);
FH_API const float* fh_rec_input_dev(fh_rec* r);
FH_API int fh_rec_embed_faces_dev(fh_rec* r, const uint8_t* d_frames, int rows, int cols, int step,
                                  long long frame_stride, const fh_face* d_faces, const int* d_frame_of, int n,
                                  float* d_out, int* d_ok, void* stream);

FH_API int fh_pipeline_run_dev(fh_det* d, fh_rec* r, const uint8_t* d_frames, int n, int rows, int cols, int step,
                               long long frame_stride, float score_thr, float nms_thr, int faces_per_frame,
                               fh_face* d_faces, int* d_frame_of, float* d_emb, void* stream);

FH_API int fh_pipeline_submit_dev(fh_det* d, fh_rec* r, const uint8_t* d_frames, int n, int rows, int cols, int step,
                                  long long frame_stride, float score_thr, float nms_thr, int faces_per_frame,
                                  fh_face* d_faces, int* d_frame_of, float* d_emb, int* d_total, void* stream_det,
                                  void* stream_rec);

typedef struct fh_stream fh_stream;
FH_API fh_stream* fh_stream_create(fh_det* d, fh_rec* r, int frames_per_batch, int rows, int cols, int faces_per_frame);
FH_API void fh_stream_destroy(fh_stream* s);
FH_API int fh_stream_submit(fh_stream* s, const uint8_t* host_frames, int n_frames, float score_thr, float nms_thr);
FH_API int fh_stream_collect(fh_stream* s, fh_face* faces, int* frame_of, float* emb, int cap);

FH_API fh_gallery* fh_gallery_create(int dim);
FH_API void fh_gallery_destroy(fh_gallery* g);
FH_API int fh_gallery_upload(fh_gallery* g, const float* rows, long long n, int rows_on_device, long long index_base);
FH_API int fh_gallery_topk_dev(fh_gallery* g, const float* d_queries, int nq, int k, float* d_scores, int* d_indices,
                               void* stream);
enum fh_gallery_scan { FH_GAL_SCAN_FP32 = 0, FH_GAL_SCAN_F16_RERANK = 1 };
FH_API int fh_gallery_set_scan(fh_gallery* g, int mode);
FH_API int fh_gallery_get_scan(const fh_gallery* g);
FH_API int fh_gallery_scan_stats(fh_gallery* g, long long* certified, long long* fallback);
FH_API int fh_topk_merge_dev(const float* d_part_scores, const int* d_part_idx, int nparts, int nq, int k, float* d_scores,
                             int* d_indices, void* stream);
#define FH_COMM_ID_BYTES 128
typedef struct fh_comm fh_comm;
FH_API int fh_comm_unique_id(unsigned char id[FH_COMM_ID_BYTES]);
FH_API fh_comm* fh_comm_create(int rank, int world, const unsigned char id[FH_COMM_ID_BYTES], int device);
FH_API void fh_comm_destroy(fh_comm* c);
FH_API int fh_comm_rank(const fh_comm* c);
FH_API int fh_comm_world(const fh_comm* c);
FH_API int fh_comm_allgather_f32_dev(fh_comm* c, const float* d_send, float* d_recv, long long count, void* stream);
FH_API int fh_gallery_topk_sharded_dev(fh_gallery* g, fh_comm* c, const float* d_queries_local, int nq_local, int k,
                                       float* d_scores, int* d_indices, void* stream);
FH_API long long fh_gallery_enroll(fh_gallery* g, const float* rows, long long n, int rows_on_device);
FH_API long long fh_gallery_size(fh_gallery* g);
FH_API int fh_gallery_label_dev(fh_gallery* g, const float* d_queries, int nq, float threshold, int* d_labels,
                                float* d_scores, void* stream);

FH_API int fh_timing_enable(int on);
FH_API int fh_timing_num_tags(void);
FH_API int fh_timing_collect(double* ms, double* flops, double* bytes, long long* launches, int n);
FH_API int fh_timing_collect_ops(double* ms, double* flops, int* tag, int cap);
FH_API int fh_det_set_conv_cfg(fh_det* d, int cfg, int stream_k);
FH_API int fh_rec_set_conv_cfg(fh_rec* r, int cfg, int stream_k);
FH_API int fh_det_set_winograd(fh_det* d, int on);
FH_API int fh_rec_set_winograd(fh_rec* r, int on);
FH_API int fh_rec_set_wino_fusion(fh_rec* r, int on);
FH_API int fh_rec_set_shortcut_fold(fh_rec* r, int on);
enum fh_precision { FH_PREC_FP32 = 0, FH_PREC_BF16X2 = 1 };
FH_API int fh_rec_set_precision(fh_rec* r, int mode, float* worst);
FH_API int fh_rec_get_precision(fh_rec* r);
FH_API int fh_det_set_cus(fh_det* d, int cus);
FH_API int fh_rec_set_cus(fh_rec* r, int cus);
FH_API int fh_det_set_fused_stem(fh_det* d, int on);
FH_API int fh_rec_set_fused_stem(fh_rec* r, int on);
FH_API int fh_det_set_fused_front(fh_det* d, int on);
FH_API int fh_det_set_halo_conv(fh_det* d, int on);

FH_API int fh_imread(const char* path, unsigned char** bgr, int* rows, int* cols);
FH_API int fh_image_decode(const unsigned char* bytes, size_t n, unsigned char** bgr, int* rows, int* cols);
FH_API void fh_image_free(unsigned char* bgr);

FH_API int fh_memcpy_d2h(void* host_dst, const void* dev_src, size_t bytes);
FH_API int fh_resize_u8c3_dev(const uint8_t* d_src, int sh, int sw, int sstep, uint8_t* d_dst, int dh, int dw, int dstep,
                              void* stream);
FH_API int fh_conv_forward_dev(const float* d_in, const float* d_wt_packed, const float* d_bias, float* d_out, int batch,
                               int h, int w, int cin, int cout, int ksize, int stride, int kpad, int cfg, void* stream);
FH_API int fh_conv_winograd_dev(const float* d_in, const float* w_ohwi_host, const float* d_bias, float* d_out, int batch, int h, int w,
                                int cin, int cout, void* stream);
FH_API int fh_conv_wino2_dev(const float* d_in, const float* w_ohwi_host, const float* d_bias, const float* d_slope, const float* d_res,
                             float* d_out, int batch, int h, int w, int cin, int cout, int act, int bias_cls, void* stream);
FH_API int fh_conv_wino2_ex_dev(const float* d_in, const float* w_ohwi_host, const float* d_bias, const float* d_slope, const float* d_res,
                                float* d_out, float* d_out2, const float* d_s2, const float* d_t2, int n_outs, float* const* d_outs,
                                const int* oc0, const int* oact, int batch, int h, int w, int cin, int cout, int act, int bias_cls,
                                void* stream);
FH_API double fh_debug_wino2_clock_mhz(void);
FH_API int fh_set_graph_replay(int on);
FH_API const float* fh_det_workspace_dev(fh_det* d);
FH_API int fh_det_graph_stats(fh_det* d, long long* replays);
FH_API int fh_rec_graph_stats(fh_rec* r, long long* replays);
FH_API int fh_debug_streamk(int drop_publish, int timeout_ms);
FH_API int fh_debug_wino_slots(int slots);
FH_API int fh_debug_topk_merge_strided_dev(const float* d_ps, const int* d_pi, int nparts, int nq, int k, long long part_stride,
                                           float* d_scores, int* d_indices, void* stream);
FH_API int fh_conv_wt_rows(int cout);
FH_API int fh_conv_pack_weights(const float* w_ohwi, int cout, int cin, int ksize, float* dst_packed);
FH_API int fh_conv_kpad(int ktot);

#ifdef __cplusplus
}
#endif
#endif
```

Baseline: 12540 faces/s.

## Add F(3,3) Winograd edge tiling for 7x7 maps in mixed layout

Extends the mixed Winograd tiling so 7x7 and 7x8 feature maps use a 5-point F(3,3) transform on edge tiles instead of padding to full 6x6 tiles. This cuts the transform-domain GEMM rows for the last IResNet stage. The transform kernel now packs four images per block to keep its thread layout. The path is enabled by default and taken only when it reduces GEMM work units, and it adds debug hooks, a host reference tile and workspace size checks.

```diff
diff --git a/facerecognizeonnx_amd/_lib.py b/facerecognizeonnx_amd/_lib.py
--- a/facerecognizeonnx_amd/_lib.py
+++ b/facerecognizeonnx_amd/_lib.py
@@ -121,6 +121,10 @@
     "fh_rec_set_cus": (_i, [_vp, _i]),
     "fh_debug_streamk": (_i, [_i, _i]),
     "fh_debug_wino_slots": (_i, [_i]),
+    "fh_debug_wino_f3": (_i, [_i]),
+    "fh_debug_wino_layout": (_i, [_i, _i, _i, _i, _i, _vp]),
+    "fh_debug_wino_last_gemm": (_i, [_vp]),
+    "fh_debug_wino_host_tile": (_i, [_vp, _vp, _i, _i, _vp]),
     "fh_debug_topk_merge_strided_dev": (_i, [_vp, _vp, _i, _i, _i, _ll, _vp, _vp, _vp]),
     "fh_set_graph_replay": (_i, [_i]),
     "fh_det_workspace_dev": (_vp, [_vp]),
@@ -133,6 +137,7 @@
     "fh_resize_u8c3_dev": (_i, [_vp, _i, _i, _i, _vp, _i, _i, _i, _vp]),
     "fh_conv_forward_dev": (_i, [_vp, _vp, _vp, _vp, _i, _i, _i, _i, _i, _i, _i, _i, _i, _vp]),
     "fh_conv_winograd_dev": (_i, [_vp, _vp, _vp, _vp, _i, _i, _i, _i, _i, _vp]),
+    "fh_conv_winograd_ex_dev": (_i, [_vp, _vp, _vp, _vp, _vp, _vp, _vp, _vp, _vp, _i, _i, _i, _i, _i, _i, _vp]),
     "fh_debug_wino2_clock_mhz": (_d, []),
     "fh_conv_wino2_dev": (_i, [_vp, _vp, _vp, _vp, _vp, _vp, _i, _i, _i, _i, _i, _i, _i, _vp]),
     "fh_conv_wino2_ex_dev": (_i, [_vp, _vp, _vp, _vp, _vp, _vp, _vp, _vp, _vp, _i, _vp, _vp, _vp, _i, _i, _i, _i, _i, _i, _i, _vp]),
diff --git a/facerecognizeonnx_amd/csrc/api.cpp b/facerecognizeonnx_amd/csrc/api.cpp
--- a/facerecognizeonnx_amd/csrc/api.cpp
+++ b/facerecognizeonnx_amd/csrc/api.cpp
@@ -105,6 +105,7 @@
     key.push_back((long long)fh::layout_epoch());
     key.push_back(net.config_word());
     key.push_back((long long)fh::conv_error_generation() << 32 | fh::conv_debug_generation());
+    key.push_back((long long)fh::wino_debug_generation());
 }
 constexpr int kGraphFaces = 256;
 
@@ -755,9 +756,12 @@
         return 0;
     });
 }
-int fh_conv_winograd_dev(const float* d_in, const float* w_ohwi, const float* d_bias, float* d_out, int batch, int h, int w, int cin,
-                         int cout, void* stream) {
+int fh_conv_winograd_ex_dev(const float* d_in, const float* w_ohwi, const float* d_bias, const float* d_slope, const float* d_res, float* d_out,
+                            float* d_out2, const float* d_s2, const float* d_t2, int batch, int h, int w, int cin, int cout, int act,
+                            void* stream) {
     if (!d_in || !w_ohwi || !d_out || cin % 32 || cout % 4) return arg_error("fh_conv_winograd_dev: bad argument");
+    if (d_out2 && (!d_s2 || !d_t2)) return arg_error("fh_conv_winograd_dev: a second output needs its scale and shift");
+    if (act == (int)fh::Act::PRELU && !d_slope) return arg_error("fh_conv_winograd_dev: PReLU needs its slopes");
     Owns owns(nullptr);
     return guarded([&] {
         const int rows = fh::conv_wt_rows(cout);
@@ -785,12 +789,18 @@
         if (slabs_gen != fh::conv_error_generation()) { fh::conv_workspace_reset_async(slabs.as<float>(), S(stream)); slabs_gen = fh::conv_error_generation(); }
         fh::ConvArgs a{};
         a.in = d_in; a.bias = d_bias; a.out1 = d_out; a.slabs = slabs.as<float>(); a.sk_enable = 1;
+        a.slope = d_slope; a.res = d_res; a.out2 = d_out2; a.s2 = d_s2; a.t2 = d_t2;
         a.B = batch; a.H = h; a.W = w; a.Ho = h; a.Wo = w; a.Cin = cin; a.Cout = cout; a.ks = 3; a.stride = 1; a.pad = 1;
-        a.act = (int)fh::Act::NONE; a.res_mode = (int)fh::ResMode::NONE;
+        a.act = act; a.res_mode = d_res ? (int)fh::ResMode::SAME : (int)fh::ResMode::NONE;
         fh::launch_conv_winograd(a, dU.as<float>(), dV.as<float>(), dM.as<float>(), 2, nullptr, nullptr, S(stream));
         FH_HIP(hipStreamSynchronize(S(stream)));
         return 0;
     });
+}
+int fh_conv_winograd_dev(const float* d_in, const float* w_ohwi, const float* d_bias, float* d_out, int batch, int h, int w, int cin,
+                         int cout, void* stream) {
+    return fh_conv_winograd_ex_dev(d_in, w_ohwi, d_bias, nullptr, nullptr, d_out, nullptr, nullptr, nullptr, batch, h, w, cin, cout,
+                                   (int)fh::Act::NONE, stream);
 }
 int fh_conv_wino2_ex_dev(const float* d_in, const float* w_ohwi, const float* d_bias, const float* d_slope, const float* d_res, float* d_out,
                          float* d_out2, const float* d_s2, const float* d_t2, int n_outs, float* const* d_outs, const int* oc0, const int* oact,
@@ -848,6 +858,22 @@
     return (int)(r->gcall.nodes ? r->gcall.nodes : r->gcall_simple.nodes);
 }
 int fh_debug_wino_slots(int slots) { fh::wino_debug_slots(slots); return 0; }
+int fh_debug_wino_f3(int on) { fh::wino_debug_f3(on); return 0; }
+int fh_debug_wino_last_gemm(int* out4) { if (!out4) return arg_error("null argument"); fh::wino_debug_last_gemm(out4); return 0; }
+int fh_debug_wino_layout(int batch, int h, int w, int cin, int cout, int* out19) {
+    fh::WinoPlanes pl{};
+    if (!fh::wino_mix_layout(batch, h, w, cin, cout, &pl)) return 0;
+    if (out19) {
+        for (int c = 0; c < 4; ++c) { out19[c] = pl.n[c]; out19[4 + c] = pl.nfr[c]; out19[8 + c] = pl.nfc[c]; out19[12 + c] = pl.rows[c]; }
+        out19[16] = pl.total_tiles; out19[17] = pl.planes; out19[18] = pl.f3;
+    }
+    return 1;
+}
+int fh_debug_wino_host_tile(const double* g9, const double* d36, int rows_f3, int cols_f3, double* y16) {
+    if (!g9 || !d36 || !y16) return arg_error("null argument");
+    fh::wino_host_tile(g9, d36, rows_f3, cols_f3, y16);
+    return 0;
+}
 int fh_debug_streamk(int drop_publish, int timeout_ms) { fh::conv_debug_streamk(drop_publish, timeout_ms); return 0; }
 int fh_conv_forward_dev(const float* in, const float* wt, const float* bias, float* out, int batch, int h, int w, int cin, int cout,
                         int ks, int stride, int kpad, int cfg, void* stream) {
diff --git a/facerecognizeonnx_amd/csrc/engine.cpp b/facerecognizeonnx_amd/csrc/engine.cpp
--- a/facerecognizeonnx_amd/csrc/engine.cpp
+++ b/facerecognizeonnx_amd/csrc/engine.cpp
@@ -320,7 +320,7 @@
         sk_gen_ = conv_error_generation();
     }
     if (wino_elems_) {
-        const size_t pad = 36 * 256 * wino_maxc_;
+        const size_t pad = (size_t)std::max(36 * 256, 121 * 128) * wino_maxc_;
         wino_v_.ensure((wino_elems_ * (size_t)cap_ + pad) * sizeof(float));
         wino_m_.ensure((wino_elems_ * (size_t)cap_ + pad) * sizeof(float));
     }
@@ -459,6 +459,12 @@
                     const bool bf2 = bf16x2_ && d.bf2 && force_cfg < 0;
                     WinoPlanes pl;
                     const bool mix = wcfg == 2 && wino_mix_layout(batch, op.H, op.W, op.Cin, op.Cout, &pl);
+                    if (mix) {
+                        size_t rows = 0;
+                        for (int c = 0; c < 4; ++c) rows += (size_t)pl.nfr[c] * pl.nfc[c] * pl.rows[c];
+                        if (rows * (size_t)std::max(op.Cin, op.Cout) * sizeof(float) > wino_v_.bytes)
+                            throw std::runtime_error("winograd: the mixed tiling does not fit the transform workspace");
+                    }
                     if (!v_ready) {
                         const float* in_s = nullptr; const float* in_t = nullptr;
                         if (d.aff_src >= 0) {
diff --git a/facerecognizeonnx_amd/csrc/kernels.h b/facerecognizeonnx_amd/csrc/kernels.h
--- a/facerecognizeonnx_amd/csrc/kernels.h
+++ b/facerecognizeonnx_amd/csrc/kernels.h
@@ -128,19 +128,24 @@
 struct WinoPlanes {
     int e[4];
     int t[4];
+    int nfr[4];
     int nfc[4];
-    int f2[4];
     int n[4];
     int rows[4];
     int base[4];
     int total_tiles;
     int planes;
+    int f3;
 };
 bool wino_mix_layout(int B, int H, int W, int Cin, int Cout, WinoPlanes* out);
 void launch_wino_mix(const ConvArgs& a, const WinoPlanes& pl, const float* M, float* Vnext, int feed_aff, const float* in_scale,
                      const float* in_shift, bool pack_next, hipStream_t s);
 void wino_filter_transform(const double g[9], double u[36]);
 void wino_debug_slots(int slots);
+void wino_debug_f3(int on);
+unsigned wino_debug_generation();
+void wino_debug_last_gemm(int out[4]);
+void wino_host_tile(const double g[9], const double d[36], int rows_f3, int cols_f3, double y[16]);
 long wino_rows(long tiles);
 int conv_wt_rows(int Cout);
 size_t conv_slab_floats();
diff --git a/facerecognizeonnx_amd/csrc/winograd.hip b/facerecognizeonnx_amd/csrc/winograd.hip
--- a/facerecognizeonnx_amd/csrc/winograd.hip
+++ b/facerecognizeonnx_amd/csrc/winograd.hip
@@ -1,6 +1,7 @@
 #include <hip/hip_runtime.h>
 
 #include <algorithm>
+#include <atomic>
 #include <cstdlib>
 #include <stdexcept>
 
@@ -39,7 +40,8 @@
     if (n4 > 0) hipLaunchKernelGGL(pack_bf16x2_kernel, dim3((unsigned)std::min<long>((n4 + 255) / 256, 256 * 64)), dim3(256), 0, s, in, out, n4);
 }
 
-__device__ __forceinline__ void wino_bt(const v4f (&d)[6], v4f (&t)[6]) {
+template <class T>
+__host__ __device__ __forceinline__ void wino_bt(const T (&d)[6], T (&t)[6]) {
     t[0] = 4.f * d[0] - 5.f * d[2] + d[4];
     t[1] = -4.f * d[1] - 4.f * d[2] + d[3] + d[4];
     t[2] = 4.f * d[1] - 4.f * d[2] - d[3] + d[4];
@@ -47,7 +49,8 @@
     t[4] = 2.f * d[1] - d[2] - 2.f * d[3] + d[4];
     t[5] = 4.f * d[1] - 5.f * d[3] + d[5];
 }
-__device__ __forceinline__ void wino_at(const v4f (&m)[6], v4f (&y)[4]) {
+template <class T>
+__host__ __device__ __forceinline__ void wino_at(const T (&m)[6], T (&y)[4]) {
     y[0] = m[0] + m[1] + m[2] + m[3] + m[4];
     y[1] = m[1] - m[2] + 2.f * m[3] - 2.f * m[4];
     y[2] = m[1] + m[2] + 4.f * m[3] + 4.f * m[4];
@@ -395,10 +398,10 @@
 __device__ __forceinline__ int wino_plane_freq(const WinoPlanes& pl, const int tile_m) {
     const int c = tile_m >= pl.e[3] ? 3 : tile_m >= pl.e[2] ? 2 : tile_m >= pl.e[1] ? 1 : 0;
     const int pln = (tile_m - pl.e[c]) / pl.t[c];
-    const int nfc = pl.nfc[c], f2 = pl.f2[c];
+    const int nfr = pl.nfr[c], nfc = pl.nfc[c];
     int i = pln / nfc, j = pln - i * nfc;
-    if ((f2 & 2) && i == 3) i = 5;
-    if ((f2 & 1) && j == 3) j = 5;
+    if (i == nfr - 1) i = 5;
+    if (j == nfc - 1) j = 5;
     return 6 * i + j;
 }
 
@@ -777,17 +780,37 @@
     return wino_bn128(mixed);
 }
 
+static int g_wino_f3_override = -1;
+static std::atomic<unsigned> g_wino_debug_gen{0};
+void wino_debug_f3(int on) { g_wino_f3_override = on < 0 ? -1 : on != 0; g_wino_debug_gen.fetch_add(1, std::memory_order_relaxed); }
+unsigned wino_debug_generation() { return g_wino_debug_gen.load(std::memory_order_relaxed); }
+static int wino_f3_enabled() {
+    static const int env = [] { const char* e = getenv("FACEHIP_WINO_F3"); return e ? atoi(e) : 1; }();
+    return g_wino_f3_override >= 0 ? g_wino_f3_override : env;
+}
+
+static long wino_round_units(long row_tiles, int Cout) {
+    const long sw = 2 * 256, sn = 3 * 256;
+    const long narrow = (row_tiles * (Cout / 64) + sn - 1) / sn * 3;
+    if (Cout % 128) return narrow;
+    return std::min(narrow, (row_tiles * (Cout / 128) + sw - 1) / sw * 4);
+}
+
 bool wino_mix_layout(int B, int H, int W, int Cin, int Cout, WinoPlanes* out) {
     const int TY = (H + 3) / 4, TX = (W + 3) / 4;
-    const int my = (H & 3) == 1 || (H & 3) == 2, mx = (W & 3) == 1 || (W & 3) == 2;
-    if (!wino_mix_enabled() || !(my || mx) || TY * TX != 16 || Cin % 64 || Cout % 64 || B < 64) return false;
-    if ((size_t)H * W * 16 * sizeof(v4f) > 64 * 1024) return false;
+    int my = (H & 3) == 1 || (H & 3) == 2, mx = (W & 3) == 1 || (W & 3) == 2;
+    const bool f3 = TY == 2 && TX == 2 && (H == 7 || H == 8) && (W == 7 || W == 8) && (H == 7 || W == 7);
+    if (f3) { my = H == 7; mx = W == 7; }
+    const int nshort = f3 ? 5 : 4;
+    if (!wino_mix_enabled() || !(my || mx) || TY * TX != (f3 ? 4 : 16) || Cin % 64 || Cout % 64 || B < 64) return false;
+    if (f3 && !wino_f3_enabled()) return false;
+    if ((size_t)(f3 ? 4 : 1) * H * W * 16 * sizeof(v4f) > 64 * 1024) return false;
     WinoPlanes pl{};
     const int n[4] = {(TY - my) * (TX - mx), (TY - my) * mx, my * (TX - mx), my * mx};
     int tile = 0, row = 0, planes = 0;
     for (int c = 0; c < 4; ++c) {
-        const int nfr = (c & 2) ? 4 : 6, nfc = (c & 1) ? 4 : 6;
-        pl.n[c] = n[c]; pl.nfc[c] = nfc; pl.f2[c] = c;
+        const int nfr = (c & 2) ? nshort : 6, nfc = (c & 1) ? nshort : 6;
+        pl.n[c] = n[c]; pl.nfr[c] = nfr; pl.nfc[c] = nfc;
         pl.rows[c] = (B * n[c] + 127) / 128 * 128;
         pl.t[c] = pl.rows[c] / 128;
         pl.e[c] = tile; pl.base[c] = row;
@@ -795,10 +818,14 @@
         if (n[c]) planes += nfr * nfc;
     }
     if ((long)row * std::max(Cin, Cout) * 4 >= (1L << 31)) return false;
-    pl.total_tiles = tile; pl.planes = planes;
+    if (f3 && !(wino_round_units(tile, Cout) < wino_round_units(36 * wino_rows((long)B * TY * TX) / 128, Cout))) return false;
+    pl.total_tiles = tile; pl.planes = planes; pl.f3 = f3 ? 1 : 0;
     if (out) *out = pl;
     return true;
 }
+
+static int g_wino_last_gemm[4] = {0, 0, 0, 0};
+void wino_debug_last_gemm(int out[4]) { for (int i = 0; i < 4; ++i) out[i] = g_wino_last_gemm[i]; }
 
 void launch_wino_gemm(const ConvArgs& a, const float* wt36, const float* V, float* M, int cfg, bool bf16x2, hipStream_t s, const WinoPlanes* mix) {
     const int TY = (a.H + 3) / 4, TX = (a.W + 3) / 4;
@@ -817,16 +844,17 @@
         if (!(a.Cout % 32 == 0 && cfg == 2)) throw std::runtime_error("winograd: the mixed tiling runs on the lean GEMM kernel only");
         pl = *mix;
         double real_rows = 0;
-        for (int c = 0; c < 4; ++c) real_rows += (double)((c & 2) ? 4 : 6) * pl.nfc[c] * a.B * pl.n[c];
+        for (int c = 0; c < 4; ++c) real_rows += (double)pl.nfr[c] * pl.nfc[c] * a.B * pl.n[c];
         g.t_flops = 2.0 * real_rows * a.Cin * a.Cout;
     } else {
-        pl.e[0] = 0; pl.e[1] = pl.e[2] = pl.e[3] = (int)(36 * NTp / 128); pl.t[0] = (int)(NTp / 128); pl.nfc[0] = 6;
+        pl.e[0] = 0; pl.e[1] = pl.e[2] = pl.e[3] = (int)(36 * NTp / 128); pl.t[0] = (int)(NTp / 128); pl.nfr[0] = pl.nfc[0] = 6;
         pl.total_tiles = pl.e[1];
     }
     if (a.Cout % 32 == 0 && cfg == 2) {
         const long rows = 128L * pl.total_tiles;
         const int chunks = a.Cin / 32;
         const bool wide = a.Cout % 64 == 0;
+        int bn = 64;
         timer.begin(s);
         if (bf16x2) {
             if (!wino_gemm_ok_bf16x2(a.Cin, a.Cout)) throw std::runtime_error("winograd: this layer has no split-bf16 GEMM");
@@ -834,6 +862,7 @@
                                a.Cout, pl, g.wt_gs, a.Cout / 64, chunks);
         } else if (wide && a.Cout % 128 == 0 && wino_pick_bn128(rows / 128, a.Cout, mix != nullptr, a.cus)) {
             const long nt = (rows / 128) * (a.Cout / 128), slots = wino_slots(2, a.cus);
+            bn = 128;
             if (wino_pers_enabled() && nt > slots)
                 hipLaunchKernelGGL((wino_gemm_pers_kernel<128, 2>), dim3((unsigned)slots), dim3(256), 0, s, V, wt36, M, a.Cin, a.Cout, pl, g.wt_gs,
                                    a.Cout / 128, chunks, (int)nt);
@@ -857,10 +886,14 @@
                                    pl, g.wt_gs, a.Cout / 64, chunks);
 #endif
         }
-        else
+        else {
+            bn = 32;
             hipLaunchKernelGGL((wino_gemm_kernel<32, 4>), dim3((unsigned)((rows / 128) * (a.Cout / 32))), dim3(256), 0, s, V, wt36, M, a.Cin, a.Cout,
                                pl, g.wt_gs, a.Cout / 32, chunks);
+        }
         timer.end(s, 7, g.t_flops, g.t_bytes);
+        g_wino_last_gemm[0] = bn; g_wino_last_gemm[1] = (int)((rows / 128) * (a.Cout / bn)); g_wino_last_gemm[2] = pl.total_tiles;
+        g_wino_last_gemm[3] = mix ? pl.planes : 0;
     } else {
         if (bf16x2) throw std::runtime_error("winograd: this layer has no split-bf16 GEMM");
         launch_conv(g, cfg, s);
@@ -951,18 +984,41 @@
     t[4] = v4f{0.f, 0.f, 0.f, 0.f};
     t[5] = t[4];
 }
-
+template <class T>
+__host__ __device__ __forceinline__ void wino_bt3s(const T (&d)[6], T (&t)[6]) {
+    t[0] = 4.f * (d[0] - d[2]) + 2.f * (d[3] - d[1]);
+    t[1] = 3.f * (d[3] - d[2]) - 6.f * d[1];
+    t[2] = 2.f * d[1] - 3.f * d[2] + d[3];
+    t[3] = 4.f * (d[3] - d[1]);
+    t[4] = 2.f * (d[1] - d[3]) - d[2] + d[4];
+    t[5] = T{};
+}
+template <class T>
+__host__ __device__ __forceinline__ void wino_at3(const T (&m)[6], T (&y)[4]) {
+    y[0] = m[0] + m[1] + m[2] + m[3];
+    y[1] = m[1] - m[2] + 2.f * m[3];
+    y[2] = m[1] + m[2] + 4.f * m[3] + m[4];
+    y[3] = T{};
+}
+
+template <bool F3>
 __global__ __launch_bounds__(256, 2) void wino_mix_kernel(const WinoMixArgs a) {
     const WinoOutArgs& p = a.o;
-    extern __shared__ v4f act[];
+    extern __shared__ v4f act_all[];
+    constexpr int IMG = F3 ? 4 : 1, NSHORT = F3 ? 5 : 4;
     const int C = p.C, HW = p.H * p.W;
-    const int tid = threadIdx.x, c4l = tid & 15, tile = tid >> 4;
+    const int tid = threadIdx.x, c4l = tid & 15, slot = tid >> 4;
     const int cslices = C >> 6;
-    const int cs = blockIdx.x % cslices, b = blockIdx.x / cslices;
+    const int cs = blockIdx.x % cslices, b0 = (blockIdx.x / cslices) * IMG;
+    const int im = F3 ? slot >> 2 : 0, tile = F3 ? slot & 3 : slot;
+    const int b = b0 + im;
+    const bool live = !F3 || b < p.B;
+    const int Hb = live ? p.H : 0;
+    v4f* const act = act_all + im * HW * 16;
     const int ty = tile / p.TX, tx = tile - ty * p.TX;
     const int my = a.pl.n[2] + a.pl.n[3] > 0, mx = a.pl.n[1] + a.pl.n[3] > 0;
     const bool rF2 = my && ty == p.TY - 1, cF2 = mx && tx == p.TX - 1;
-    const int nfr = rF2 ? 4 : 6, nfc = cF2 ? 4 : 6;
+    const int nfr = !live ? 0 : rF2 ? NSHORT : 6, nfc = cF2 ? NSHORT : 6;
     const int n_c = rF2 ? (cF2 ? a.pl.n[3] : a.pl.n[2]) : (cF2 ? a.pl.n[1] : a.pl.n[0]);
     const int rows_c = rF2 ? (cF2 ? a.pl.rows[3] : a.pl.rows[2]) : (cF2 ? a.pl.rows[1] : a.pl.rows[0]);
     const int base_c = rF2 ? (cF2 ? a.pl.base[3] : a.pl.base[2]) : (cF2 ? a.pl.base[1] : a.pl.base[0]);
@@ -984,11 +1040,20 @@
             }
             v4f y4[4];
             wino_at(m, y4);
-            const v4f y20 = m[0] + m[1] + m[2], y21 = m[1] - m[2] - m[3];
-            t[0][j] = rF2 ? y20 : y4[0];
-            t[1][j] = rF2 ? y21 : y4[1];
-            t[2][j] = y4[2];
-            t[3][j] = y4[3];
+            if constexpr (F3) {
+                v4f y3[4];
+                wino_at3(m, y3);
+                t[0][j] = rF2 ? y3[0] : y4[0];
+                t[1][j] = rF2 ? y3[1] : y4[1];
+                t[2][j] = rF2 ? y3[2] : y4[2];
+                t[3][j] = y4[3];
+            } else {
+                const v4f y20 = m[0] + m[1] + m[2], y21 = m[1] - m[2] - m[3];
+                t[0][j] = rF2 ? y20 : y4[0];
+                t[1][j] = rF2 ? y21 : y4[1];
+                t[2][j] = y4[2];
+                t[3][j] = y4[3];
+            }
         }
         const v4f b4 = p.bias ? *reinterpret_cast<const v4f*>(p.bias + c4 * 4) : v4f{0.f, 0.f, 0.f, 0.f};
         v4f rs[4][4];
@@ -998,7 +1063,7 @@
 #pragma unroll
                 for (int x = 0; x < 4; ++x) {
                     const int oy = 4 * ty + r, ox = 4 * tx + x;
-                    rs[r][x] = *reinterpret_cast<const v4f*>(p.res + (((size_t)b * p.H + min(oy, p.H - 1)) * p.W + min(ox, p.W - 1)) * C + c4 * 4);
+                    rs[r][x] = *reinterpret_cast<const v4f*>(p.res + (((size_t)(F3 ? min(b, p.B - 1) : b) * p.H + min(oy, p.H - 1)) * p.W + min(ox, p.W - 1)) * C + c4 * 4);
                 }
         }
         v4f sl = {0.f, 0.f, 0.f, 0.f}, s2 = {1.f, 1.f, 1.f, 1.f}, t2 = {0.f, 0.f, 0.f, 0.f};
@@ -1007,10 +1072,16 @@
 #pragma unroll
         for (int r = 0; r < 4; ++r) {
             const int oy = 4 * ty + r;
-            if (oy >= p.H) continue;
+            if (oy >= Hb) continue;
             v4f y[4];
             wino_at(t[r], y);
-            if (cF2) { y[0] = t[r][0] + t[r][1] + t[r][2]; y[1] = t[r][1] - t[r][2] - t[r][3]; }
+            if constexpr (F3) {
+                v4f y3[4];
+                wino_at3(t[r], y3);
+                if (cF2) { y[0] = y3[0]; y[1] = y3[1]; y[2] = y3[2]; }
+            } else {
+                if (cF2) { y[0] = t[r][0] + t[r][1] + t[r][2]; y[1] = t[r][1] - t[r][2] - t[r][3]; }
+            }
 #pragma unroll
             for (int x = 0; x < 4; ++x) {
                 const int ox = 4 * tx + x;
@@ -1035,8 +1106,9 @@
     } else {
         v4f as4 = {1.f, 1.f, 1.f, 1.f}, at4 = {0.f, 0.f, 0.f, 0.f};
         if (a.in_s) { as4 = *reinterpret_cast<const v4f*>(a.in_s + c4 * 4); at4 = *reinterpret_cast<const v4f*>(a.in_t + c4 * 4); }
-        const float* src = a.in + (size_t)b * HW * C + c4 * 4;
-        for (int px = tile; px < HW; px += 16) act[px * 16 + c4l] = *reinterpret_cast<const v4f*>(src + (size_t)px * C) * as4 + at4;
+        const float* src = a.in + (size_t)b0 * HW * C + c4 * 4;
+        const int npx = min(IMG, p.B - b0) * HW;
+        for (int px = slot; px < npx; px += 16) act_all[px * 16 + c4l] = *reinterpret_cast<const v4f*>(src + (size_t)px * C) * as4 + at4;
     }
     if (!a.V) return;
     __syncthreads();
@@ -1056,7 +1128,7 @@
         }
         v4f t4[6], t2s[6];
         wino_bt(d, t4);
-        wino_bt2s(d, t2s);
+        if constexpr (F3) wino_bt3s(d, t2s); else wino_bt2s(d, t2s);
 #pragma unroll
         for (int i = 0; i < 6; ++i) tt[i][c] = rF2 ? t2s[i] : t4[i];
     }
@@ -1064,7 +1136,7 @@
     for (int i = 0; i < 6; ++i) {
         v4f o4[6], o2[6];
         wino_bt(tt[i], o4);
-        wino_bt2s(tt[i], o2);
+        if constexpr (F3) wino_bt3s(tt[i], o2); else wino_bt2s(tt[i], o2);
 #pragma unroll
         for (int j = 0; j < 6; ++j) {
             const bool ok = i < nfr && j < nfc;
@@ -1085,14 +1157,46 @@
     f.in = a.in; f.in_s = in_scale; f.in_t = in_shift;
     f.V = Vnext; f.feed_aff = feed_aff; f.pack = pack_next ? 1 : 0;
     long rows = 0;
-    for (int c = 0; c < 4; ++c) rows += (long)((c & 2) ? 4 : 6) * pl.nfc[c] * pl.rows[c];
+    for (int c = 0; c < 4; ++c) rows += (long)pl.nfr[c] * pl.nfc[c] * pl.rows[c];
     f.plane_bytes = (unsigned)(rows * f.o.C * 4);
-    if (f.o.C % 64 || f.o.TY * f.o.TX != 16 || rows * f.o.C * 4 >= (1L << 31)) throw std::runtime_error("winograd: this map cannot take the mixed tiling");
-    const size_t lds = (size_t)a.H * a.W * 16 * sizeof(v4f);
+    const int img = pl.f3 ? 4 : 1;
+    const size_t lds = (size_t)img * a.H * a.W * 16 * sizeof(v4f);
+    if (f.o.C % 64 || f.o.TY * f.o.TX != 16 / img || lds > 64 * 1024 || rows * f.o.C * 4 >= (1L << 31))
+        throw std::runtime_error("winograd: this map cannot take the mixed tiling");
+    const dim3 grid((unsigned)((a.B + img - 1) / img * (f.o.C / 64)));
     KernelTimer& timer = KernelTimer::get();
     timer.begin(s);
-    hipLaunchKernelGGL(wino_mix_kernel, dim3((unsigned)(a.B * (f.o.C / 64))), dim3(256), lds, s, f);
+    if (pl.f3) hipLaunchKernelGGL(wino_mix_kernel<true>, grid, dim3(256), lds, s, f);
+    else hipLaunchKernelGGL(wino_mix_kernel<false>, grid, dim3(256), lds, s, f);
     timer.end(s, 8, 0.0, 0.0);
+}
+
+void wino_host_tile(const double g[9], const double d[36], int rows_f3, int cols_f3, double y[16]) {
+    double u[36], t[6][6], v[6][6], m[6][6], w[4][6];
+    wino_filter_transform(g, u);
+    for (int c = 0; c < 6; ++c) {
+        double col[6], tc[6];
+        for (int r = 0; r < 6; ++r) col[r] = d[r * 6 + c];
+        if (rows_f3) wino_bt3s(col, tc); else wino_bt(col, tc);
+        for (int i = 0; i < 6; ++i) t[i][c] = tc[i];
+    }
+    const int nfr = rows_f3 ? 5 : 6, nfc = cols_f3 ? 5 : 6;
+    for (int i = 0; i < 6; ++i) {
+        if (cols_f3) wino_bt3s(t[i], v[i]); else wino_bt(t[i], v[i]);
+        for (int j = 0; j < 6; ++j)
+            m[i][j] = i < nfr && j < nfc ? v[i][j] * u[6 * (i == nfr - 1 ? 5 : i) + (j == nfc - 1 ? 5 : j)] : 0.0;
+    }
+    for (int j = 0; j < 6; ++j) {
+        double col[6], yc[4];
+        for (int i = 0; i < 6; ++i) col[i] = m[i][j];
+        if (rows_f3) wino_at3(col, yc); else wino_at(col, yc);
+        for (int r = 0; r < 4; ++r) w[r][j] = yc[r];
+    }
+    for (int r = 0; r < 4; ++r) {
+        double yr[4];
+        if (cols_f3) wino_at3(w[r], yr); else wino_at(w[r], yr);
+        for (int x = 0; x < 4; ++x) y[r * 4 + x] = yr[x];
+    }
 }
 
 void launch_conv_winograd(const ConvArgs& a, const float* wt36, float* V, float* M, int cfg, const float* in_scale, const float* in_shift,
diff --git a/include/facehip.h b/include/facehip.h
--- a/include/facehip.h
+++ b/include/facehip.h
@@ -144,6 +144,9 @@
                                int h, int w, int cin, int cout, int ksize, int stride, int kpad, int cfg, void* stream);
 FH_API int fh_conv_winograd_dev(const float* d_in, const float* w_ohwi_host, const float* d_bias, float* d_out, int batch, int h, int w,
                                 int cin, int cout, void* stream);
+FH_API int fh_conv_winograd_ex_dev(const float* d_in, const float* w_ohwi_host, const float* d_bias, const float* d_slope, const float* d_res,
+                                   float* d_out, float* d_out2, const float* d_s2, const float* d_t2, int batch, int h, int w, int cin,
+                                   int cout, int act, void* stream);
 FH_API int fh_conv_wino2_dev(const float* d_in, const float* w_ohwi_host, const float* d_bias, const float* d_slope, const float* d_res,
                              float* d_out, int batch, int h, int w, int cin, int cout, int act, int bias_cls, void* stream);
 FH_API int fh_conv_wino2_ex_dev(const float* d_in, const float* w_ohwi_host, const float* d_bias, const float* d_slope, const float* d_res,
@@ -157,6 +160,10 @@
 FH_API int fh_rec_graph_stats(fh_rec* r, long long* replays);
 FH_API int fh_debug_streamk(int drop_publish, int timeout_ms);
 FH_API int fh_debug_wino_slots(int slots);
+FH_API int fh_debug_wino_f3(int on);
+FH_API int fh_debug_wino_layout(int batch, int h, int w, int cin, int cout, int* out19);
+FH_API int fh_debug_wino_last_gemm(int* out4);
+FH_API int fh_debug_wino_host_tile(const double* g9, const double* d36, int rows_f3, int cols_f3, double* y16);
 FH_API int fh_debug_topk_merge_strided_dev(const float* d_ps, const int* d_pi, int nparts, int nq, int k, long long part_stride,
                                            float* d_scores, int* d_indices, void* stream);
 FH_API int fh_conv_wt_rows(int cout);
```

Result: no change. 12610 faces/s, median of 6 (+0.6%).
